# Piletskii-Oleg/chunkfs

Measured on AMD Instinct MI355X. Metric: GiB/s chunked device-resident, FastCDC 4/8/16 KiB avg, at 1/2/4/8 MI355X, higher is better.
Workload: dtype u8

## Files before the change

### chunkfs_amd/build.py

```python
import os
import subprocess
import sys

HERE = os.path.dirname(os.path.abspath(__file__))
ROOT = os.path.dirname(HERE)
CSRC = os.path.join(HERE, "csrc")
BUILD = os.path.join(HERE, "_build")
LIB = os.path.join(HERE, "libchunkfs_amd.so")
SOURCES = ["fastcdc.hip", "fastcdc_ovl.hip", "small.hip", "walk.hip", "util_kernels.hip", "sha256.hip", "index.hip", "engine.cpp", "hostpath.cpp", "capi.cpp",
           "index_host.cpp"]
HEADERS = ["fastcdc.hpp", "small.hpp", "walk.hpp", "cdc_kernels.hpp", "sha256.hpp", "index.hpp", "engine.hpp"]
ARCH = "gfx950"
HIPCC = os.environ.get("HIPCC", "/opt/rocm/bin/hipcc")
CFLAGS = ["-O3", "-std=c++17", "-fPIC", f"--offload-arch={ARCH}", "-Wall", "-Wno-unused-result"]


def source_digest():
    import hashlib
    h = hashlib.sha256()
    files = [os.path.join(CSRC, f) for f in SOURCES + HEADERS] + [
        os.path.join(ROOT, "include", f) for f in ("chunkfs_amd.h", "chunkfs_amd_tables.h", "chunkfs_amd_debug.h", "chunkfs_amd_cdc_params.h")]
    for f in files:
        h.update(os.path.basename(f).encode())
        with open(f, "rb") as fh:
            h.update(fh.read())
    return h.hexdigest()[:16]


def _newer(target, deps):
    if not os.path.exists(target):
        return True
    t = os.path.getmtime(target)
    return any(os.path.getmtime(d) > t for d in deps)


def _run(cmd):
    print("+", " ".join(cmd), flush=True)
    subprocess.check_call(cmd)


def build(force=False, defines=(), lib=None, build_dir=None):
    bdir = build_dir or BUILD
    out_lib = lib or LIB
    os.makedirs(bdir, exist_ok=True)
    common = [os.path.join(CSRC, h) for h in HEADERS] + [
        os.path.join(ROOT, "include", "chunkfs_amd.h"),
        os.path.join(ROOT, "include", "chunkfs_amd_tables.h"),
        os.path.join(ROOT, "include", "chunkfs_amd_debug.h"),
        os.path.join(ROOT, "include", "chunkfs_amd_cdc_params.h"),
    ]
    objs = []
    for src in SOURCES:
        s = os.path.join(CSRC, src)
        o = os.path.join(bdir, src + ".o")
        objs.append(o)
        deps = [s] + common + ([os.path.join(CSRC, "fastcdc.hip")] if src == "fastcdc_ovl.hip" else [])
        if force or _newer(o, deps):
            lang = ["-x", "hip"] if src.endswith(".hip") else []
            _run([HIPCC] + CFLAGS + [f"-D{d}" for d in defines] + lang + ["-c", s, "-o", o])
    if force or _newer(out_lib, objs):
        _run([HIPCC, f"--offload-arch={ARCH}", "-shared", "-fPIC", "-o", out_lib] + objs)
    return out_lib


if __name__ == "__main__":
    build(force="--force" in sys.argv)
```

### chunkfs_amd/csrc/engine.cpp

```cpp
#include "engine.hpp"

#include <algorithm>
#include <atomic>
#include <chrono>
#include <cmath>
#include <cstdio>
#include <cstdlib>
#include <cstring>

#include "../../include/chunkfs_amd_cdc_params.h"
#include "../../include/chunkfs_amd_tables.h"
#include "fastcdc.hpp"
#include "sha256.hpp"

namespace cdc {

namespace {
thread_local std::string g_last_error;

#ifndef CDC_MIN_SPAN_LOG2
#define CDC_MIN_SPAN_LOG2 16
#endif
constexpr uint32_t kMinSpanLog2 = CDC_MIN_SPAN_LOG2;
constexpr uint32_t kMaxSpanLog2 = 17;

constexpr uint32_t kMinimumMin = 64, kMinimumMax = 1048576;
constexpr uint32_t kAverageMin = 256, kAverageMax = 4194304;
constexpr uint32_t kMaximumMin = 1024, kMaximumMax = 16777216;

size_t align_up(size_t x, size_t a) { return (x + a - 1) / a * a; }

uint32_t ceil_log2(uint64_t x) {
    uint32_t r = 0;
    while ((1ull << r) < x) ++r;
    return r;
}
}

void set_error(const std::string &msg) { g_last_error = msg; }
const char *last_error() { return g_last_error.c_str(); }

#define HIP_TRY(expr)                                                          \
    do {                                                                       \
        hipError_t e_ = (expr);                                                \
        if (e_ != hipSuccess) {                                                \
            set_error(std::string(#expr) + ": " + hipGetErrorString(e_));      \
            return CDC_EDEVICE;                                                \
        }                                                                      \
    } while (0)

int Engine::create(cdc_algo_t algo, uint32_t min, uint32_t avg, uint32_t max,
                   int device, Engine **out) {
    if (!out) {
        set_error("cdc_create: out is NULL");
        return CDC_EINVAL;
    }
    *out = nullptr;
    if (algo == CDC_ALGO_RABIN || algo == CDC_ALGO_ULTRA || algo == CDC_ALGO_LEAP || algo == CDC_ALGO_SEQ) {
        const uint32_t seq[4] = {0, CDC_SEQ_LENGTH, CDC_SEQ_JUMP_TRIGGER, CDC_SEQ_JUMP_SIZE};
        return create_walk(algo, seq, min, avg, max, device, out);
    }
    if (algo != CDC_ALGO_FASTCDC && algo != CDC_ALGO_FIXED) {
        set_error("SuperCDC is not implemented on MI355X: its chunk records (supercdc.rs:10, 37-50) "
                  "follow cdc-chunkers 0.1.3, absent offline (SURVEY.md §8c)");
        return CDC_ENOTSUP;
    }
    Engine *e = new Engine();
    e->algo_ = algo;
    e->min_ = min;
    e->avg_ = avg;
    e->max_ = max;
    e->device_ = device;
    if (algo == CDC_ALGO_FASTCDC) {
        if (min < kMinimumMin || min > kMinimumMax || avg < kAverageMin ||
            avg > kAverageMax || max < kMaximumMin || max > kMaximumMax) {
            set_error("FastCDC sizes out of range (fastcdc v2020 asserts: min 64..1MiB, "
                      "avg 256..4MiB, max 1KiB..16MiB)");
            delete e;
            return CDC_EINVAL;
        }
        const unsigned bits = (unsigned)std::lround(std::log2((double)avg));
        FastParams &fp = e->fp_;
        fp.min = min;
        fp.avg = avg;
        fp.max = max;
        fp.mask_s = CHUNKFS_AMD_MASKS[bits + 1];
        fp.mask_l = CHUNKFS_AMD_MASKS[bits - 1];
        fp.cmask = fp.mask_s & fp.mask_l;
        const uint64_t all = fp.mask_s | fp.mask_l;
        const uint32_t top = 63 - (uint32_t)__builtin_clzll(all);
        if (top > 47) {
            set_error("mask tests bit >= 48: unsupported");
            delete e;
            return CDC_EINVAL;
        }
        fp.trunc = top;
        const uint32_t wlo = (uint32_t)__builtin_ctzll(all);
        fp.cm_align = (wlo <= 32 && (all >> wlo) <= 0xFFFFFFFFull) ? 1u : 0u;
        fp.tshift = fp.cm_align ? 32 - wlo : 0;
        fp.cm32 = (uint32_t)((fp.cmask << fp.tshift) >> 32);
        fp.cm_lo = (uint32_t)fp.cmask;
        fp.cm_hi = (uint32_t)(fp.cmask >> 32);
        fp.mask_s_sh = fp.mask_s << fp.tshift;
        fp.mask_l_sh = fp.mask_l << fp.tshift;
        if (const char *d = std::getenv("CHUNKFS_AMD_DIAG")) fp.diag = (uint32_t)std::atoi(d);
        if (const char *v = std::getenv("CHUNKFS_AMD_EVENT_EVERY")) e->event_every_ = std::max(1, std::atoi(v));
        if (const char *v = std::getenv("CHUNKFS_AMD_OVERLAP")) {
            e->ovl_on_ = std::atoi(v) != 0;
            e->ovl_std_ = std::atoi(v) != 1;
        }
        uint32_t l2 = ceil_log2(max);
        e->span_log2_ = l2 > kMinSpanLog2 ? l2 : kMinSpanLog2;
        {
            const uint32_t pcm = (uint32_t)__builtin_popcountll(fp.cmask);
            while (e->span_log2_ < kMaxSpanLog2 && 11 * ((2ull << e->span_log2_) >> (pcm < 63 ? pcm : 63)) <= 384)
                ++e->span_log2_;
        }
        if (const char *v = std::getenv("CHUNKFS_AMD_SPAN"))
            e->span_log2_ = (uint32_t)std::max<int>(std::atoi(v), (int)std::max(l2, 14u));
        e->small_span_log2_ = l2 > 14 ? l2 : 14;
        if (const char *v = std::getenv("CHUNKFS_AMD_SMALL_SPAN")) {
            const int x = std::atoi(v);
            e->small_span_log2_ = x == 0 ? e->span_log2_ : (uint32_t)std::max<int>(x, (int)std::max(l2, 14u));
        }
        if (e->small_span_log2_ > e->span_log2_) e->small_span_log2_ = e->span_log2_;
        const uint64_t span = 1ull << e->span_log2_;
        const uint32_t pc = (uint32_t)__builtin_popcountll(fp.cmask);
        uint64_t cap = 8 * (span >> (pc < 63 ? pc : 63));
        if (cap < 64) cap = 64;
        if (cap > 256) cap = 256;
        e->cap_ = (uint32_t)cap;
        e->smax_ = (uint32_t)(span / ((min / 2) * 2) + 2);
        if (11 * (span >> (pc < 63 ? pc : 63)) > 256 && !e->ovl_std_) e->ovl_on_ = false;
        const uint32_t pmin = (uint32_t)std::min(__builtin_popcountll(fp.mask_s), __builtin_popcountll(fp.mask_l));
        e->small_on_ = pmin >= 10;
        e->small_pmin_ = pmin;
        if (const char *v = std::getenv("CHUNKFS_AMD_SMALL")) e->small_on_ = e->small_on_ && std::atoi(v) != 0;
        if (const char *v = std::getenv("CHUNKFS_AMD_SMALL_ZC")) e->small_zc_ = std::atoi(v) != 0;
        if (const char *v = std::getenv("CHUNKFS_AMD_SMALL_FEED")) e->small_feed_ = std::atoi(v);
        if (const char *v = std::getenv("CHUNKFS_AMD_SMALL_FEED_POOL")) e->small_feed_pool_ = std::atoi(v) != 0;
        char buf[256];
        std::snprintf(buf, sizeof buf,
                      "FastCDC (2020), sizes: SizeParams { min: %u, avg: %u, max: %u } "
                      "[MI355X gfx950]",
                      min, avg, max);
        e->describe_ = buf;
    } else {
        if (min == 0) {
            set_error("FSChunker chunk size must be > 0");
            delete e;
            return CDC_EINVAL;
        }
        char buf[128];
        std::snprintf(buf, sizeof buf, "Fixed size chunking, chunk size: %u [MI355X gfx950]", min);
        e->describe_ = buf;
    }
    const int rc = e->init();
    if (rc != CDC_OK) {
        delete e;
        return rc;
    }
    *out = e;
    return CDC_OK;
}

int Engine::init() {
    int count = 0;
    HIP_TRY(hipGetDeviceCount(&count));
    if (device_ < 0 || device_ >= count) {
        set_error("device index out of range");
        return CDC_EDEVICE;
    }
    HIP_TRY(hipSetDevice(device_));
    hipDeviceProp_t prop;
    HIP_TRY(hipGetDeviceProperties(&prop, device_));
    if (std::strncmp(prop.gcnArchName, "gfx950", 6) != 0) {
        set_error(std::string("chunkfs_amd kernels are built for gfx950 only; device is ") +
                  prop.gcnArchName);
        return CDC_EDEVICE;
    }
    num_cus_ = prop.multiProcessorCount;
    HIP_TRY(hipStreamCreateWithFlags(&own_stream_, hipStreamNonBlocking));
    for (auto &ev : ev_) HIP_TRY(hipEventCreate(&ev));
    for (auto &slot : tev_)
        for (auto &ev : slot) HIP_TRY(hipEventCreate(&ev));
    HIP_TRY(hipMalloc(&d_gear_, 256 * sizeof(uint64_t)));
    HIP_TRY(hipMalloc(&d_counter_, (1 + kShaBuckets) * sizeof(unsigned long long)));
    HIP_TRY(hipMemcpy(d_gear_, CHUNKFS_AMD_GEAR, 256 * sizeof(uint64_t), hipMemcpyHostToDevice));
    return CDC_OK;
}

struct Engine::WalkWorker {
    Engine *ctx = nullptr;
    int device = 0;
    std::thread th;
    std::mutex m;
    std::condition_variable cv;
    bool has_job = false, stop = false;
    bool done = true;
    bool fresh = false;
    uint64_t seq = 0;
    std::vector<const uint8_t *> ptrs;
    std::vector<uint64_t> lens;
    cdc_chunk_t *out = nullptr;
    size_t cap = 0;
    uint64_t *first = nullptr;
    int64_t rc = 0;
    std::string err;

    void loop() {
        (void)hipSetDevice(device);
        std::unique_lock<std::mutex> lk(m);
        for (;;) {
            cv.wait(lk, [&] { return stop || has_job; });
            if (has_job) {
                has_job = false;
                lk.unlock();
                const int64_t r =
                    ctx->chunk_batch_device(ptrs.size(), ptrs.data(), lens.data(), out, cap, first, nullptr);
                std::string e = r < 0 ? std::string(last_error()) : std::string();
                lk.lock();
                rc = r;
                err = std::move(e);
                done = true;
                cv.notify_all();
                continue;
            }
            return;
        }
    }
    void wait_done(std::unique_lock<std::mutex> &lk) {
        cv.wait(lk, [&] { return done; });
    }
    ~WalkWorker() {
        {
            std::lock_guard<std::mutex> g(m);
            stop = true;
        }
        cv.notify_all();
        if (th.joinable()) th.join();
        delete ctx;
    }
};

Engine::~Engine() {
    if (device_ >= 0) (void)hipSetDevice(device_);
    if (fb_any_) (void)fast_drain();
    for (auto &w : ww_) w.reset();
    if (own_stream_) (void)hipStreamSynchronize(own_stream_);
    if (res_stream_) (void)hipStreamSynchronize(res_stream_);
    (void)hipFree(ws_);
    (void)hipFree(small_mem_);
    (void)hipFree(d_gear_);
    (void)hipFree(d_data_);
    (void)hipFree(d_out_);
    (void)hipFree(d_dig_);
    (void)hipFree(d_sha_tab_);
    (void)hipHostFree(h_sha_tab_);
    (void)hipFree(d_sha_order_);
    (void)hipFree(d_counter_);
    (void)hipFree(d_wtabs_);
    (void)hipFree(wws_);
    (void)hipHostFree(h_stage_);
    if (copy_stream_) (void)hipStreamSynchronize(copy_stream_);
    (void)hipHostFree(h_ring_);
    (void)hipHostFree(h_ready_);
    (void)hipHostFree(h_out_);
    for (auto &w : ws_win_) (void)hipFree(w);
    for (auto &e : ring_ev_)
        if (e) (void)hipEventDestroy(e);
    if (copy_done_) (void)hipEventDestroy(copy_done_);
    if (ws_ev_) (void)hipEventDestroy(ws_ev_);
    if (copy_stream_) (void)hipStreamDestroy(copy_stream_);
    for (auto &ev : ev_)
        if (ev) (void)hipEventDestroy(ev);
    for (auto &slot : tev_)
        for (auto &ev : slot)
            if (ev) (void)hipEventDestroy(ev);
    if (own_stream_) (void)hipStreamDestroy(own_stream_);
    for (auto &ev : scan_ev_)
        if (ev) (void)hipEventDestroy(ev);
    if (res_ev_) (void)hipEventDestroy(res_ev_);
    for (auto &ev : res_done_)
        if (ev) (void)hipEventDestroy(ev);
    if (res_stream_) (void)hipStreamDestroy(res_stream_);
}

int Engine::set_gear(const uint64_t *gear) {
    if (!gear) {
        set_error("gear is NULL");
        return CDC_EINVAL;
    }
    if (fb_any_) {
        const int64_t r = drain_implicit();
        if (r < 0) return (int)r;
    }
    if (wr_.active) {
        set_error("cdc_set_gear: a streaming write is in progress (cdc_write_finish it first)");
        return CDC_EINVAL;
    }
    HIP_TRY(hipSetDevice(device_));
    HIP_TRY(hipMemcpy(d_gear_, gear, 256 * sizeof(uint64_t), hipMemcpyHostToDevice));
    return CDC_OK;
}

size_t Engine::estimate(size_t len) const {
    if (algo_ == CDC_ALGO_FIXED) return len / min_ + 1;
    if (algo_ == CDC_ALGO_SEQ) return len / avg_;
    return len / min_;
}

size_t Engine::batch_max_chunks(size_t n, const uint64_t *lens) const {
    size_t t = 0;
    for (size_t i = 0; i < n; ++i) t += lens[i] / min_chunk() + 1;
    return t;
}

int Engine::ensure_host_staging(size_t n) {
    if (h_stage_ && h_stage_streams_ >= n) return CDC_OK;
    if (fb_any_) {
        set_error("internal: host staging regrown with FastCDC batches in flight");
        return CDC_EINVAL;
    }
    (void)hipHostFree(h_stage_);
    h_stage_ = nullptr;
    const size_t want = n + 64;
    h_stage_per_ = 5 * want + 36 + 4 * walk::kMaxFixRounds;
    HIP_TRY(placement().host_malloc(&h_stage_, kHostSlots * h_stage_per_ * sizeof(uint64_t), hipHostMallocCoherent));
    h_stage_streams_ = want;
    for (int k = 0; k < kSlots; ++k) fs_[k].tables.clear();
    return CDC_OK;
}

int Engine::ensure_workspace(uint64_t spans, size_t n) {
    if (ws_ && spans <= ws_spans_ && n <= ws_streams_) return CDC_OK;
    const uint64_t S = spans > ws_spans_ ? spans + spans / 4 + 16 : ws_spans_;
    const size_t N = n > ws_streams_ ? n + 64 : ws_streams_;
    const uint64_t cap = algo_ == CDC_ALGO_FASTCDC ? cap_ : 0;
    const uint64_t smax = algo_ == CDC_ALGO_FASTCDC ? smax_ : 0;
    const size_t A = 256;
    size_t off = 0;
    auto take = [&](size_t bytes) {
        const size_t o = off;
        off = align_up(off + bytes, A);
        return o;
    };
    if (fb_any_) {
        set_error("internal: workspace regrown with FastCDC batches in flight");
        return CDC_EINVAL;
    }
    size_t o_count[kSlots], o_pos[kSlots], o_ptrs[kSlots], o_lens[kSlots], o_sb[kSlots], o_stats[kSlots],
        o_tails[kSlots];
    for (int k = 0; k < kSlots; ++k) {
        o_count[k] = take(S * 4);
        o_pos[k] = take(S * cap * 4);
        o_ptrs[k] = take(N * 8);
        o_lens[k] = take(N * 8);
        o_sb[k] = take((N + 1) * 8);
        o_stats[k] = take(p3::kStatWords * 8);
        o_tails[k] = take(N * 8);
    }
    const size_t o_starts = take(S * smax * 8);
    const size_t o_first = take((N + 1) * 8);
    const uint64_t nb = std::max(p3::resolve_blocks(S), p3::ovl::resolve_blocks(S)) + 2;
    const size_t o_desc = take(6 * nb * 8);
    (void)hipFree(ws_);
    ws_ = nullptr;
    ws_spans_ = 0;
    ws_streams_ = 0;
    HIP_TRY(hipMalloc(&ws_, off));
    ++ws_gen_;
    ws_bytes_ = off;
    ws_spans_ = S;
    ws_streams_ = N;
    char *b = static_cast<char *>(ws_);
    for (int k = 0; k < kSlots; ++k) {
        FastSlot &f = fs_[k];
        f.cand.cap = (uint32_t)cap;
        f.cand.count = reinterpret_cast<uint32_t *>(b + o_count[k]);
        f.cand.pos = reinterpret_cast<uint32_t *>(b + o_pos[k]);
        f.d_ptrs = reinterpret_cast<const uint8_t **>(b + o_ptrs[k]);
        f.d_lens = reinterpret_cast<uint64_t *>(b + o_lens[k]);
        f.d_sb = reinterpret_cast<uint64_t *>(b + o_sb[k]);
        f.d_tails = reinterpret_cast<uint64_t *>(b + o_tails[k]);
        f.stats = reinterpret_cast<uint64_t *>(b + o_stats[k]);
        f.tables.clear();
    }
    cand_ = fs_[0].cand;
    d_first_ = reinterpret_cast<uint64_t *>(b + o_first);
    d_ptrs_ = fs_[0].d_ptrs;
    d_lens_ = fs_[0].d_lens;
    d_span_base_ = fs_[0].d_sb;
    ch3_.smax = (uint32_t)smax;
    ch3_.starts = reinterpret_cast<uint64_t *>(b + o_starts);
    uint64_t *desc = reinterpret_cast<uint64_t *>(b + o_desc);
    rs3_ = p3::Resolve{desc, desc + nb, desc + 2 * nb, desc + 3 * nb, desc + 4 * nb, desc + 5 * nb, 0};
    HIP_TRY(hipMemset(desc, 0, 6 * nb * 8));
    d_tails_ = fs_[0].d_tails;
    return CDC_OK;
}

int64_t Engine::chunk_batch_device(size_t n, const uint8_t *const *d_streams,
                                   const uint64_t *lens, cdc_chunk_t *d_out,
                                   size_t out_cap, uint64_t *first,
                                   hipStream_t stream) {
    return batch_device(n, d_streams, lens, d_out, out_cap, first, stream, false);
}

int64_t Engine::chunk_batch_device_async(size_t n, const uint8_t *const *d_streams, const uint64_t *lens,
                                         cdc_chunk_t *d_out, size_t out_cap, uint64_t *first,
                                         hipStream_t stream) {
    return batch_device(n, d_streams, lens, d_out, out_cap, first, stream, true);
}

int64_t Engine::batch_sync() {
    HIP_TRY(hipSetDevice(device_));
    if (fb_any_) {
        held_valid_ = false;
        return fast_drain();
    }
    if (held_valid_) {
        held_valid_ = false;
        return held_;
    }
    return 0;
}

int64_t Engine::drain_implicit() {
    if (!fb_any_) return 0;
    held_ = fast_drain();
    held_valid_ = true;
    return held_;
}

int64_t Engine::walk_submit(size_t n, const uint8_t *const *d_streams, const uint64_t *lens, cdc_chunk_t *d_out,
                            size_t out_cap, uint64_t *first) {
    const int c = (int)(wk_seq_ % (uint64_t)walk_ctx_);
    if (!ww_[c]) {
        Engine *e = nullptr;
        int rc = create_walk(algo_, seq_cfg_, min_, avg_, max_, device_, &e);
        if (rc) return rc;
        e->walk_async_ = false;
        if (rabin_poly_) rc = e->set_rabin_poly(rabin_poly_);
        if (rc) {
            delete e;
            return rc;
        }
        std::unique_ptr<WalkWorker> w(new WalkWorker());
        w->ctx = e;
        w->device = device_;
        WalkWorker *wp = w.get();
        w->th = std::thread([wp] { wp->loop(); });
        ww_[c] = std::move(w);
    }
    WalkWorker &w = *ww_[c];
    {
        std::unique_lock<std::mutex> lk(w.m);
        w.wait_done(lk);
        if (w.fresh && w.rc < 0) {
            const int64_t rc = w.rc;
            const std::string msg = w.err;
            lk.unlock();
            (void)walk_drain();
            set_error(msg);
            return rc;
        }
        w.ptrs.assign(d_streams, d_streams + n);
        w.lens.assign(lens, lens + n);
        w.out = d_out;
        w.cap = out_cap;
        w.first = first;
        w.seq = wk_seq_;
        w.rc = 0;
        w.err.clear();
        w.done = false;
        w.fresh = true;
        w.has_job = true;
    }
    w.cv.notify_all();
    ++wk_seq_;
    wk_any_ = true;
    fb_any_ = true;
    return 0;
}

int64_t Engine::walk_drain() {
    int64_t res = 0, err = 0;
    std::string msg;
    uint64_t last = 0;
    bool any = false;
    for (auto &wp : ww_) {
        if (!wp) continue;
        WalkWorker &w = *wp;
        std::unique_lock<std::mutex> lk(w.m);
        w.wait_done(lk);
        if (!w.fresh) continue;
        w.fresh = false;
        if (w.rc < 0 && !err) {
            err = w.rc;
            msg = w.err;
        }
        if (!any || w.seq > last) {
            any = true;
            last = w.seq;
            res = w.rc;
            timing_ = w.ctx->timing_;
        }
    }
    wk_any_ = false;
    fb_any_ = false;
    if (err) {
        set_error(msg);
        return err;
    }
    return res;
}

int64_t Engine::batch_device(size_t n, const uint8_t *const *d_streams, const uint64_t *lens, cdc_chunk_t *d_out,
                             size_t out_cap, uint64_t *first, hipStream_t stream, bool async) {
    if (n && (!d_streams || !lens || !first)) {
        set_error("cdc_chunk_batch_device: NULL argument");
        return CDC_EINVAL;
    }
    if (n > 0xFFFFFFFEull) {
        set_error("too many streams");
        return CDC_EINVAL;
    }
    HIP_TRY(hipSetDevice(device_));
    hipStream_t s = stream ? stream : own_stream_;
    uint64_t bytes = 0, need = 0;
    for (size_t i = 0; i < n; ++i) {
        bytes += lens[i];
        need += lens[i] / min_chunk() + 1;
        if (lens[i] && !d_streams[i]) {
            set_error("NULL stream pointer with non-zero length");
            return CDC_EINVAL;
        }
        if (lens[i] && algo_ != CDC_ALGO_FIXED && (reinterpret_cast<uintptr_t>(d_streams[i]) & 15)) {
            set_error("device stream pointers must be 16-byte aligned");
            return CDC_EINVAL;
        }
    }
    if (need > out_cap) {
        set_error("out_cap < cdc_batch_max_chunks()");
        return CDC_EINVAL;
    }
    if (async && is_walk() && walk_async_ && n > 0 && bytes > kSmallBatch)
        return walk_submit(n, d_streams, lens, d_out, out_cap, first);
    const bool pipe = algo_ == CDC_ALGO_FASTCDC && n > 0 && bytes > kSmallBatch;
    if (!pipe && fb_any_) {
        const int64_t r = drain_implicit();
        if (r < 0) return r;
    }
    if (pipe) {
        const int64_t r = fast_submit(n, d_streams, lens, d_out, out_cap, first, bytes, s,
                                      !async || fb_seq_ % event_every_ == 0, async && ovl_on_);
        if (r < 0 || async) return r;
        return fast_drain();
    }
    const double hash_ms = timing_.hash_ms;
    timing_pending_ = false;
    timing_ = cdc_timing_t{};
    timing_.hash_ms = hash_ms;
    timing_.bytes = bytes;
    timing_.path = CDC_PATH_EMPTY;
    out_cap_ = out_cap;
    if (n == 0) {
        if (first) first[0] = 0;
        return 0;
    }
    int rc = ensure_host_staging(n);
    if (rc) return rc;
    if (algo_ == CDC_ALGO_FASTCDC && n == 1 && !small_skip_ && small_ok(lens[0])) {
        rc = run_small(d_streams[0], lens[0], d_out, out_cap, first, s);
        if (rc == CDC_OK) {
            timing_.path = CDC_PATH_SMALL;
            return (int64_t)first[1];
        }
        if (rc < 0) return rc;
    }
    if (algo_ == CDC_ALGO_FASTCDC) {
        const int64_t r = fast_submit(n, d_streams, lens, d_out, out_cap, first, bytes, s, true, false);
        if (r < 0) return r;
        return fast_drain();
    }
    uint64_t *h = static_cast<uint64_t *>(h_stage_);
    uint64_t *h_ptrs = h, *h_lens = h + h_stage_streams_, *h_sb = h + 2 * h_stage_streams_;
    const uint32_t sl2 = is_walk() ? seg_log2_ : 0;
    uint64_t spans = 0;
    for (size_t i = 0; i < n; ++i) {
        h_ptrs[i] = reinterpret_cast<uint64_t>(d_streams[i]);
        h_lens[i] = lens[i];
        h_sb[i] = spans;
        if (is_walk()) spans += (lens[i] + (1ull << sl2) - 1) >> sl2;
    }
    h_sb[n] = spans;
    if (algo_ != CDC_ALGO_FIXED && spans == 0) {
        for (size_t i = 0; i <= n; ++i) first[i] = 0;
        return 0;
    }
    rc = is_walk() ? ensure_walk_workspace(spans, n) : ensure_workspace(spans, n);
    if (rc) return rc;
    const bool zero_copy = bytes <= kSmallBatch && n <= kZeroCopyStreams;
    const bool same = zero_copy || (ws_gen_ == tables_gen_ && tables_.size() == 2 * n &&
                                    std::memcmp(tables_.data(), h_ptrs, n * 8) == 0 &&
                                    std::memcmp(tables_.data() + n, h_lens, n * 8) == 0);
    if (!same) {
        HIP_TRY(hipMemcpyAsync(d_ptrs_, h_ptrs, n * 8, hipMemcpyHostToDevice, s));
        HIP_TRY(hipMemcpyAsync(d_lens_, h_lens, n * 8, hipMemcpyHostToDevice, s));
        HIP_TRY(hipMemcpyAsync(d_span_base_, h_sb, (n + 1) * 8, hipMemcpyHostToDevice, s));
        tables_.assign(h_ptrs, h_ptrs + n);
        tables_.insert(tables_.end(), h_lens, h_lens + n);
        tables_gen_ = ws_gen_;
    }
    StreamTable st{};
    st.ptrs = zero_copy ? reinterpret_cast<const uint8_t *const *>(h_ptrs) : d_ptrs_;
    st.lens = zero_copy ? h_lens : d_lens_;
    st.span_base = zero_copy ? h_sb : d_span_base_;
    st.n = (uint32_t)n;
    st.span_log2 = sl2;
    st.total_spans = spans;
    rc = is_walk() ? run_walk(st, d_out, n, first, s) : run_fixed(st, n, lens, d_out, first, s);
    if (rc) return rc;
    return (int64_t)first[n];
}

int64_t Engine::fast_submit(size_t n, const uint8_t *const *d_streams, const uint64_t *lens, cdc_chunk_t *d_out,
                            size_t out_cap, uint64_t *first, uint64_t bytes, hipStream_t s, bool timed, bool ovl) {
    if (fb_any_ && (s != fb_stream_ || ovl != fb_ovl_)) {
        const int64_t r = drain_implicit();
        if (r < 0) return r;
    }
    if (ovl && !res_stream_) {
        HIP_TRY(hipStreamCreateWithFlags(&res_stream_, hipStreamNonBlocking));
        for (auto &ev : scan_ev_) HIP_TRY(hipEventCreateWithFlags(&ev, hipEventDisableTiming));
        HIP_TRY(hipEventCreateWithFlags(&res_ev_, hipEventDisableTiming));
        for (auto &ev : res_done_) HIP_TRY(hipEventCreateWithFlags(&ev, hipEventDisableTiming));
        if (!std::getenv("CHUNKFS_AMD_NO_PREWARM")) {
            void *d = nullptr;
            HIP_TRY(hipMalloc(&d, 256));
            for (int i = 0; i < 256; ++i) {
                HIP_TRY(hipMemsetAsync(d, i, 4, s));
                HIP_TRY(hipEventRecord(scan_ev_[i % kSlots], s));
                HIP_TRY(hipStreamWaitEvent(res_stream_, scan_ev_[i % kSlots], 0));
                HIP_TRY(hipMemsetAsync(static_cast<char *>(d) + 128, i, 4, res_stream_));
                HIP_TRY(hipEventRecord(res_done_[i % 3], res_stream_));
            }
            HIP_TRY(hipStreamSynchronize(res_stream_));
            HIP_TRY(hipStreamSynchronize(s));
            HIP_TRY(hipFree(d));
        }
    }
    const uint32_t sl2 = bytes <= kSmallBatch ? small_span_log2_ : span_log2_;
    uint64_t spans = 0;
    for (size_t i = 0; i < n; ++i) spans += (lens[i] + (1ull << sl2) - 1) >> sl2;
    const bool zero_copy = bytes <= kSmallBatch && n <= kZeroCopyStreams;
    const bool grow = !(h_stage_ && h_stage_streams_ >= n) || !(ws_ && spans <= ws_spans_ && n <= ws_streams_);
    if (fb_any_ && (zero_copy || grow)) {
        const int64_t r = drain_implicit();
        if (r < 0) return r;
    }
    const uint64_t seq = fb_seq_;
    if (fb_[seq % 3].live) {
        const int rc = fast_collect((int)(seq % 3));
        if (rc) {
            (void)fast_drain();
            return rc;
        }
    }
    int rc = ensure_host_staging(n);
    if (rc) return rc;
    rc = ensure_workspace(spans ? spans : 1, n);
    if (rc) return rc;
    const int slot = (int)(seq % kSlots);
    FastSlot &f = fs_[slot];
    uint64_t *hb = static_cast<uint64_t *>(h_stage_) + (seq % kHostSlots) * h_stage_per_;
    uint64_t *h_ptrs = hb, *h_lens = hb + h_stage_streams_, *h_sb = hb + 2 * h_stage_streams_;
    uint64_t *h_tails = hb + 3 * h_stage_streams_;
    bool same = !zero_copy && f.tables_gen == ws_gen_ && f.tables.size() == 2 * n;
    for (size_t i = 0; same && i < n; ++i)
        same = f.tables[i] == reinterpret_cast<uint64_t>(d_streams[i]) && f.tables[n + i] == lens[i];
    {
        uint64_t sp = 0;
        uint32_t nt = 0;
        for (size_t i = 0; i < n; ++i) {
            h_ptrs[i] = reinterpret_cast<uint64_t>(d_streams[i]);
            h_lens[i] = lens[i];
            h_sb[i] = sp;
            sp += (lens[i] + (1ull << sl2) - 1) >> sl2;
            if (lens[i] & ((1ull << sl2) - 1)) h_tails[nt++] = sp - 1;
        }
        h_sb[n] = sp;
        if (same && nt != f.n_tails) same = false;
        f.n_tails = nt;
    }
    if (!same) {
        f.tables.clear();
        if (!zero_copy) {
            HIP_TRY(hipMemcpyAsync(f.d_ptrs, h_ptrs, n * 8, hipMemcpyHostToDevice, s));
            HIP_TRY(hipMemcpyAsync(f.d_lens, h_lens, n * 8, hipMemcpyHostToDevice, s));
            HIP_TRY(hipMemcpyAsync(f.d_sb, h_sb, (n + 1) * 8, hipMemcpyHostToDevice, s));
            if (f.n_tails) HIP_TRY(hipMemcpyAsync(f.d_tails, h_tails, f.n_tails * 8, hipMemcpyHostToDevice, s));
            f.tables.assign(h_ptrs, h_ptrs + n);
            f.tables.insert(f.tables.end(), h_lens, h_lens + n);
            f.tables_gen = ws_gen_;
        }
    }
    StreamTable st{};
    st.ptrs = zero_copy ? reinterpret_cast<const uint8_t *const *>(h_ptrs) : f.d_ptrs;
    st.lens = zero_copy ? h_lens : f.d_lens;
    st.span_base = zero_copy ? h_sb : f.d_sb;
    st.n = (uint32_t)n;
    st.span_log2 = sl2;
    st.total_spans = spans;
    uint64_t *h_misc = hb + 4 * h_stage_streams_;
    const p3::Compact cp{f.stats, h_misc, h_misc + p3::kStatWords};
    h_misc[p3::kStatDone] = ~0ull;
    if (!spans) {
        h_misc[p3::kStatDone] = 1;
        h_misc[p3::kStatError] = 0;
        for (size_t i = 0; i <= n; ++i) cp.h_first[i] = 0;
    }
    p3::Resolve rs = rs3_;
    rs.gen = ++res_gen_;
    FastBatch &rec = fb_[seq % 3];
    rec = FastBatch{};
    rec.resolved = true;
    rec.ovl = ovl;
    rec.slot = slot;
    rec.h = hb;
    rec.n = n;
    rec.first = first;
    rec.seq = seq;
    rec.bytes = bytes;
    rec.spans = spans;
    hipEvent_t *ev = tev_[seq % kTimeRing];
    tev_timed_[seq % kTimeRing] = timed;
    rec.timed = timed;
    if (timed) HIP_TRY(hipEventRecord(ev[0], s));
    if (!ovl) {
        if (spans)
            HIP_TRY(p3::launch_scan(st, fp_, d_gear_, f.cand, cp, zero_copy ? h_tails : f.d_tails, f.n_tails,
                                    num_cus_, s));
        if (timed) HIP_TRY(hipEventRecord(ev[1], s));
        if (spans) HIP_TRY(p3::launch_resolve(st, fp_, d_gear_, f.cand, ch3_, cp, rs, d_out, out_cap, s));
        if (timed) HIP_TRY(hipEventRecord(ev[2], s));
    } else {
        static_assert(kSlots > kHostSlots, "device slots must outlast the host blocks");
        if (spans && ovl_std_)
            HIP_TRY(p3::launch_scan(st, fp_, d_gear_, f.cand, cp, zero_copy ? h_tails : f.d_tails, f.n_tails,
                                    num_cus_, s));
        else if (spans)
            HIP_TRY(p3::ovl::launch_scan(st, fp_, d_gear_, f.cand, cp, zero_copy ? h_tails : f.d_tails, f.n_tails,
                                         num_cus_, s));
        if (timed) HIP_TRY(hipEventRecord(ev[1], s));
        HIP_TRY(hipEventRecord(scan_ev_[slot], s));
        HIP_TRY(hipStreamWaitEvent(res_stream_, scan_ev_[slot], 0));
        if (spans && ovl_std_)
            HIP_TRY(p3::launch_resolve(st, fp_, d_gear_, f.cand, ch3_, cp, rs, d_out, out_cap, res_stream_));
        else if (spans)
            HIP_TRY(p3::ovl::launch_resolve(st, fp_, d_gear_, f.cand, ch3_, cp, rs, d_out, out_cap, res_stream_));
        if (timed) HIP_TRY(hipEventRecord(ev[2], res_stream_));
        else HIP_TRY(hipEventRecord(res_done_[seq % 3], res_stream_));
    }
    rec.live = true;
    fb_seq_ = seq + 1;
    fast_batches_ = fb_seq_;
    fb_any_ = true;
    fb_stream_ = s;
    fb_ovl_ = ovl;
    cand_ = f.cand;
    last_spans_ = spans;
    return 0;
}

int64_t Engine::fast_drain() {
    if (!fb_any_) return 0;
    if (wk_any_) return walk_drain();
    const uint64_t last = fb_seq_ - 1;
    int rc = CDC_OK;
    int64_t total = 0;
    for (uint64_t q = last >= 2 ? last - 2 : 0; q <= last; ++q) {
        FastBatch &b = fb_[q % 3];
        if (!b.live || b.seq != q) continue;
        const int r = rc ? rc : fast_collect((int)(q % 3));
        b.live = false;
        if (r && !rc) rc = r;
        if (q == last && !rc) total = (int64_t)b.first[b.n];
    }
    if (fb_ovl_) {
        if (!rc && hipEventRecord(res_ev_, res_stream_) == hipSuccess)
            (void)hipStreamWaitEvent(fb_stream_, res_ev_, 0);
        else
            (void)hipStreamSynchronize(res_stream_);
    }
    if (rc) (void)hipStreamSynchronize(fb_stream_);
    fb_any_ = false;
    return rc ? rc : total;
}

int Engine::fast_collect(int k) {
    FastBatch &b = fb_[k];
    if (!b.resolved) {
        set_error("internal: FastCDC batch collected before its resolve was enqueued");
        return CDC_EDEVICE;
    }
    uint64_t *h_misc = b.h + 4 * h_stage_streams_;
    {
        const volatile uint64_t *done = h_misc + p3::kStatDone;
        const uint64_t us = b.ovl ? std::min<uint64_t>(4000, std::max<uint64_t>(200, b.bytes / 1000000))
                                  : std::min<uint64_t>(2000, std::max<uint64_t>(100, b.bytes / 2000000));
        const auto budget = std::chrono::microseconds(us);
        const auto t_spin = std::chrono::steady_clock::now();
        while (*done == ~0ull && std::chrono::steady_clock::now() - t_spin < budget) __builtin_ia32_pause();
    }
    if (h_misc[p3::kStatDone] == ~0ull) {
        if (b.timed) HIP_TRY(hipEventSynchronize(tev_[b.seq % kTimeRing][2]));
        else if (b.ovl) HIP_TRY(hipEventSynchronize(res_done_[b.seq % 3]));
        else HIP_TRY(hipStreamSynchronize(fb_stream_));
    }
    b.live = false;
    if (h_misc[p3::kStatDone] != 1 || h_misc[p3::kStatError] != 0) {
        set_error(h_misc[p3::kStatDone] != 1 ? "resolve kernel did not report back"
                                             : "chain overflow, output bound or look-back timeout (internal error)");
        return CDC_EDEVICE;
    }
    if (fp_.diag & 64) {
        const uint64_t *d = h_misc + p3::kStatDiag0;
        const uint64_t s0 = ~d[0], s1 = d[1], e1 = d[2], e0 = ~d[3];
        const double blocks =
            (double)(b.ovl && !ovl_std_ ? p3::ovl::resolve_blocks(b.spans) : p3::resolve_blocks(b.spans));
        std::fprintf(stderr, "resolve blocks, us: scan's last block end -> first start %.2f  starts spread %.2f  "
                             "first start -> first end %.2f  -> last end %.2f  longest block %.2f  mean block %.2f\n",
                     ((double)s0 - (double)d[6]) / 100.0, (s1 - s0) / 100.0, (e0 - s0) / 100.0, (e1 - s0) / 100.0,
                     d[4] / 100.0, d[5] / 100.0 / (blocks ? blocks : 1.0));
    } else if (fp_.diag & 128) {
        const double waves = b.ovl && !ovl_std_ ? (double)p3::ovl::resolve_blocks(b.spans) * 4
                                                : (double)p3::resolve_blocks(b.spans) * 8;
        std::fprintf(stderr, (fp_.diag & 8192) ? "resolve link passes, us per wave (records: issue trunc link; "
                                                 "virtual: issue trunc link; -; -):"
                                               : "resolve phases, us per wave (meta recs settle+wait virtual-links "
                                                 "record-links walk lookback(w0) out):");
        for (int i = 0; i < p3::kStatDiagN; ++i)
            std::fprintf(stderr, " %.2f", (double)h_misc[p3::kStatDiag0 + i] / 100.0 / (waves ? waves : 1.0));
        std::fprintf(stderr, "\n");
    }
    const uint64_t *lens = b.h + h_stage_streams_;
    uint64_t *hf = h_misc + p3::kStatWords;
    for (size_t i = b.n; i-- > 0;)
        if (lens[i] == 0) hf[i] = hf[i + 1];
    std::memcpy(b.first, hf, (b.n + 1) * 8);
    const double hash_ms = timing_.hash_ms;
    timing_ = cdc_timing_t{};
    timing_.hash_ms = hash_ms;
    timing_.bytes = b.bytes;
    timing_.candidates = h_misc[p3::kStatCand];
    timing_.overflow_spans = (uint32_t)h_misc[p3::kStatOvf];
    timing_.fixup_iterations = (uint32_t)h_misc[p3::kStatRewalk];
    timing_.walk_fallback_steps = h_misc[p3::kStatOnDemand];
    timing_.path = CDC_PATH_PIPELINE;
    timing_.timed = b.timed ? 1u : 0u;
    timing_pending_ = true;
    timing_seq_ = b.seq;
    return CDC_OK;
}

bool Engine::small_ok(uint64_t len) const {
    return small_on_ && len > 0 && len <= small::kMaxBytes && (len >> small_pmin_) <= small::kRecCap * 5 / 8;
}

int Engine::run_small(const uint8_t *data, uint64_t len, cdc_chunk_t *d_out, size_t out_cap, uint64_t *first,
                      hipStream_t s, bool host_input, const uint8_t *feed_src, uint8_t *feed_dst,
                      uint32_t feed_slot) {
    if (!small_mem_) {
        HIP_TRY(hipMalloc(&small_mem_, small::scratch_bytes() + small::copy_bytes() + small::bstamp_bytes()));
        HIP_TRY(hipMemset(small_mem_, 0, small::scratch_bytes()));
        uint32_t *b = static_cast<uint32_t *>(small_mem_);
        small_ws_.brec = reinterpret_cast<uint64_t *>(b);
        small_ws_.bcnt = b + 2 * small::kMaxBlocks * small::kBlockRecCap;
        small_ws_.ticket = small_ws_.bcnt + small::kMaxBlocks;
        small_ws_.stamp = reinterpret_cast<uint64_t *>(static_cast<char *>(small_mem_) + small::scratch_bytes() - 64);
        small_ws_.bpub = small_ws_.stamp - small::kMaxBlocks;
        small_ws_.copy = static_cast<uint8_t *>(small_mem_) + small::scratch_bytes();
        small_ws_.bstamp = reinterpret_cast<uint64_t *>(small_ws_.copy + small::copy_bytes());
    }
    uint64_t *h = static_cast<uint64_t *>(h_stage_);
    uint64_t *h_misc = h + 4 * h_stage_streams_;
    uint64_t *h_first = h_misc + p3::kStatWords;
    volatile uint64_t *done = h_misc + small::kWordDone;
    *done = 0;
    small_seq_ = small_seq_ % 0xFFFFFFFEull + 1;
    const small::Feed feed{feed_src ? h_ready_dev_ + (size_t)feed_slot * small::kFeedPieces : nullptr, small_seq_};
    auto feed_copy = [&]() {
        const auto tc = std::chrono::steady_clock::now();
        volatile uint64_t *ready = h_ready_ + (size_t)feed_slot * small::kFeedPieces;
        if (small_feed_pool_) {
            pool_->copy_feed(feed_dst, feed_src, len, size_t(1) << small::kFeedLog2, ready, small_seq_);
        } else {
            const uint64_t piece = 1ull << small::kFeedLog2;
            for (uint64_t off = 0; off < len; off += piece) {
                std::memcpy(feed_dst + off, feed_src + off, std::min(piece, len - off));
                std::atomic_thread_fence(std::memory_order_release);
                ready[off >> small::kFeedLog2] = small_seq_;
            }
        }
        small_copy_s_ = std::chrono::duration<double>(std::chrono::steady_clock::now() - tc).count();
    };
    if (feed_src && small_feed_ == 2) feed_copy();
    HIP_TRY(small::launch_small(data, len, fp_, d_gear_, small_ws_, d_out, out_cap, h_misc, h_first, host_input,
                                feed, s));
    ++small_calls_;
    if (feed_src && small_feed_ != 2) {
        feed_copy();
    }
    const auto t_spin = std::chrono::steady_clock::now();
    while (*done == 0 && std::chrono::steady_clock::now() - t_spin < std::chrono::microseconds(2000))
        __builtin_ia32_pause();
    if (*done == 0) HIP_TRY(hipStreamSynchronize(s));
    if (*done != 1) {
        set_error("small FastCDC kernel did not report back");
        return CDC_EDEVICE;
    }
    timing_pending_ = false;
    timing_.candidates = h_misc[small::kWordRecords];
    timing_.overflow_spans = 0;
    timing_.fixup_iterations = 0;
    timing_.walk_fallback_steps = 0;
    if (fp_.diag & small::kDiagStamps) {
        const uint64_t *t = h_misc + small::kWordStamp0;
        std::fprintf(stderr, "small: %llu B, us from block 0's start: last block %.2f, records %.2f, links %.2f "
                             "(%llu rounds), walk %.2f, output %.2f\n",
                     (unsigned long long)len, (t[1] - t[0]) / 100.0, (t[2] - t[0]) / 100.0, (t[3] - t[0]) / 100.0,
                     (unsigned long long)t[7], (t[4] - t[0]) / 100.0, (t[5] - t[0]) / 100.0);
        std::fprintf(stderr, "  round 0 max cycles per lane: load+trunc %llu, link %llu, successor %llu; rounds end at",
                     (unsigned long long)(t[6] & 0x1FFFFF), (unsigned long long)((t[6] >> 21) & 0x1FFFFF),
                     (unsigned long long)(t[6] >> 42));
        for (int k = 0; k < 4; ++k)
            if (h_first[2 + k]) std::fprintf(stderr, " %.2f", (h_first[2 + k] - t[0]) / 100.0);
        if (feed_src) std::fprintf(stderr, "; block 0 fed at %.2f; host copy %.2f us", (h_first[6] - t[0]) / 100.0,
                                   small_copy_s_ * 1e6);
        std::fprintf(stderr, "; round 0 added %llu entries, round 1 worked on %llu", (unsigned long long)(h_first[7] & 0xFFFF),
                     (unsigned long long)(h_first[7] >> 16));
        std::fprintf(stderr, "\n");
        const uint32_t G = (uint32_t)((len + small::kBlockBytes - 1) / small::kBlockBytes);
        std::vector<uint64_t> bs((size_t)G * 8);
        HIP_TRY(hipStreamSynchronize(s));
        HIP_TRY(hipMemcpy(bs.data(), small_ws_.bstamp, bs.size() * 8, hipMemcpyDeviceToHost));
        const char *nm[6] = {"fed", "loaded", "hashed(w0)", "tinfo(w0)", "drained", "ticket"};
        std::fprintf(stderr, "  blocks (%u):", G);
        for (int k = 0; k < 6; ++k) {
            std::vector<double> v;
            for (uint32_t b = 0; b < G; ++b) v.push_back(((double)bs[b * 8 + k] - (double)t[0]) / 100.0);
            std::sort(v.begin(), v.end());
            std::fprintf(stderr, " %s %.2f/%.2f/%.2f", nm[k], v.front(), v[v.size() / 2], v.back());
        }
        std::fprintf(stderr, "\n");
    }
    if (h_misc[small::kWordFallback]) {
        ++small_fallbacks_;
        return kSmallFallback;
    }
    first[0] = 0;
    first[1] = h_first[1];
    return CDC_OK;
}

const cdc_timing_t &Engine::timing() {
    if (fb_any_) (void)drain_implicit();
    if (timing_pending_) {
        timing_pending_ = false;
        (void)timing_back((uint32_t)(fast_batches_ - 1 - timing_seq_), timing_);
    }
    return timing_;
}

int Engine::timing_back(uint32_t back, cdc_timing_t &out) {
    if (fb_any_) (void)drain_implicit();
    if (algo_ != CDC_ALGO_FASTCDC || back >= kTimeRing || back >= fast_batches_) {
        set_error("cdc_debug_timing_back: no such FastCDC batch in the event ring");
        return CDC_EINVAL;
    }
    if (&out != &timing_) out = timing_;
    hipEvent_t *ev = tev_[(fast_batches_ - 1 - back) % kTimeRing];
    float t01 = 0, t12 = 0, t02 = 0;
    HIP_TRY(hipSetDevice(device_));
    out.path = CDC_PATH_PIPELINE;
    out.timed = tev_timed_[(fast_batches_ - 1 - back) % kTimeRing] ? 1u : 0u;
    if (!out.timed) {
        out.scan_ms = out.resolve_ms = out.total_ms = 0;
        return CDC_OK;
    }
    HIP_TRY(hipEventSynchronize(ev[2]));
    HIP_TRY(hipEventElapsedTime(&t01, ev[0], ev[1]));
    HIP_TRY(hipEventElapsedTime(&t12, ev[1], ev[2]));
    HIP_TRY(hipEventElapsedTime(&t02, ev[0], ev[2]));
    out.scan_ms = t01;
    out.resolve_ms = t12;
    out.total_ms = t02;
    return CDC_OK;
}

int Engine::run_fixed(const StreamTable &st, size_t n, const uint64_t *lens,
                      cdc_chunk_t *d_out, uint64_t *first, hipStream_t s) {
    uint64_t *h = static_cast<uint64_t *>(h_stage_);
    uint64_t *h_first = h + 4 * h_stage_streams_;
    uint64_t t = 0;
    for (size_t i = 0; i < n; ++i) {
        h_first[i] = t;
        t += (lens[i] + min_ - 1) / min_;
    }
    h_first[n] = t;
    HIP_TRY(hipEventRecord(ev_[0], s));
    HIP_TRY(hipMemcpyAsync(d_first_, h_first, (n + 1) * 8, hipMemcpyHostToDevice, s));
    HIP_TRY(launch_fixed(st, min_, d_first_, d_out, t, s));
    HIP_TRY(hipEventRecord(ev_[3], s));
    HIP_TRY(hipStreamSynchronize(s));
    std::memcpy(first, h_first, (n + 1) * 8);
    float t03 = 0;
    HIP_TRY(hipEventElapsedTime(&t03, ev_[0], ev_[3]));
    timing_.total_ms = t03;
    timing_.scan_ms = t03;
    timing_.path = CDC_PATH_FIXED;
    timing_.timed = 1;
    return CDC_OK;
}

int64_t Engine::fs_write(const uint8_t *data, size_t len, size_t seg_size, std::vector<uint64_t> &spans,
                         double *seconds) {
    spans.clear();
    if (seg_size == 0) {
        set_error("cdc_fs_write: seg_size must be > 0");
        return CDC_EINVAL;
    }
    if (len && !data) {
        set_error("cdc_fs_write: data is NULL");
        return CDC_EINVAL;
    }
    int rc = write_begin();
    if (rc) return rc;
    for (size_t off = 0; !rc && off < len; off += seg_size)
        rc = write_segment(data + off, std::min(seg_size, len - off));
    if (rc) {
        wr_.active = false;
        return rc;
    }
    return write_finish(spans, seconds);
}

int Engine::sha256_device(const uint8_t *d_data, const cdc_chunk_t *d_chunks, size_t n,
                          uint8_t *d_digests, hipStream_t s) {
    const uint64_t first[2] = {0, n};
    return sha256_batch(1, &d_data, first, d_chunks, d_digests, s);
}

int Engine::sha256_batch(size_t n, const uint8_t *const *d_streams, const uint64_t *first,
                         const cdc_chunk_t *d_chunks, uint8_t *d_digests, hipStream_t s) {
    if (n == 0) return CDC_OK;
    if (!d_streams || !first) {
        set_error("cdc_sha256_batch_device: NULL stream table");
        return CDC_EINVAL;
    }
    if (first[0] != 0) {
        set_error("cdc_sha256_batch_device: first[0] must be 0");
        return CDC_EINVAL;
    }
    for (size_t i = 0; i < n; ++i) {
        if (first[i + 1] < first[i]) {
            set_error("cdc_sha256_batch_device: first[] must be non-decreasing");
            return CDC_EINVAL;
        }
        if (first[i + 1] > first[i] && !d_streams[i]) {
            set_error("cdc_sha256_batch_device: NULL stream with chunks");
            return CDC_EINVAL;
        }
    }
    const uint64_t total = first[n];
    if (total >= (1ull << 32)) {
        set_error("cdc_sha256_batch_device: more than 2^32 - 1 chunks in one batch");
        return CDC_EINVAL;
    }
    if (total && (!d_chunks || !d_digests)) {
        set_error("cdc_sha256_chunks_device: NULL argument");
        return CDC_EINVAL;
    }
    HIP_TRY(hipSetDevice(device_));
    if (fb_any_) {
        const int64_t r = drain_implicit();
        if (r < 0) return (int)r;
    }
    hipStream_t st = s ? s : own_stream_;
    (void)timing();
    if (total == 0) {
        timing_.hash_ms = 0;
        return CDC_OK;
    }
    const size_t words = 2 * n + 1;
    if (sha_tab_cap_ < words) {
        (void)hipFree(d_sha_tab_);
        (void)hipHostFree(h_sha_tab_);
        d_sha_tab_ = h_sha_tab_ = nullptr;
        sha_tab_cap_ = 0;
        const size_t want = words + 64;
        HIP_TRY(hipMalloc(&d_sha_tab_, want * 8));
        HIP_TRY(hipHostMalloc(&h_sha_tab_, want * 8, hipHostMallocDefault));
        sha_tab_cap_ = want;
    }
    std::memcpy(h_sha_tab_, first, (n + 1) * 8);
    for (size_t i = 0; i < n; ++i) h_sha_tab_[n + 1 + i] = reinterpret_cast<uint64_t>(d_streams[i]);
    HIP_TRY(hipMemcpyAsync(d_sha_tab_, h_sha_tab_, words * 8, hipMemcpyHostToDevice, st));
    ShaBatch b{};
    b.chunks = reinterpret_cast<const cdc_chunk_pod *>(d_chunks);
    b.n_chunks = total;
    b.first = d_sha_tab_;
    b.base = d_sha_tab_ + n + 1;
    b.n_streams = (uint32_t)n;
    b.digests = reinterpret_cast<uint32_t *>(d_digests);
    b.counter = d_counter_;
    if (sha_order_cap_ < total) {
        (void)hipFree(d_sha_order_);
        d_sha_order_ = nullptr;
        sha_order_cap_ = 0;
        const uint64_t want = total + total / 8 + 1024;
        HIP_TRY(hipMalloc(&d_sha_order_, want * sizeof(uint32_t)));
        sha_order_cap_ = want;
    }
    b.order = d_sha_order_;
    HIP_TRY(hipEventRecord(ev_[3], st));
    HIP_TRY(launch_sha256(b, num_cus_, st));
    HIP_TRY(hipEventRecord(ev_[2], st));
    HIP_TRY(hipStreamSynchronize(st));
    float ms = 0;
    HIP_TRY(hipEventElapsedTime(&ms, ev_[3], ev_[2]));
    timing_.hash_ms = ms;
    return CDC_OK;
}

int64_t Engine::debug_copy(int what, void *out, size_t max_bytes) {
    if (fb_any_) {
        const int64_t r = drain_implicit();
        if (r < 0) return r;
    }
    if (algo_ != CDC_ALGO_FASTCDC || !ws_) {
        set_error("debug_copy: no FastCDC batch yet");
        return CDC_EINVAL;
    }
    const void *src = nullptr;
    size_t bytes = 0;
    if (what == 0) {
        src = cand_.count;
        bytes = last_spans_ * 4;
    } else if (what == 1) {
        src = cand_.pos;
        bytes = last_spans_ * cap_ * 4;
    } else {
        set_error("debug_copy: unknown array");
        return CDC_EINVAL;
    }
    if (bytes > max_bytes) bytes = max_bytes;
    HIP_TRY(hipSetDevice(device_));
    HIP_TRY(hipStreamSynchronize(own_stream_));
    if (bytes) HIP_TRY(hipMemcpy(out, src, bytes, hipMemcpyDeviceToHost));
    return (int64_t)bytes;
}

int Engine::read_bw(const uint8_t *d_buf, size_t len, int reps, double *ms) {
    HIP_TRY(hipSetDevice(device_));
    if (fb_any_) {
        const int64_t r = drain_implicit();
        if (r < 0) return (int)r;
    }
    uint64_t *d_acc = nullptr;
    const size_t words = (size_t)num_cus_ * 8;
    HIP_TRY(hipMalloc(&d_acc, words * 8));
    hipError_t e = hipMemsetAsync(d_acc, 0, words * 8, own_stream_);
    if (e == hipSuccess) e = launch_read_reduce(d_buf, len, d_acc, num_cus_, own_stream_);
    if (e == hipSuccess) e = hipEventRecord(ev_[0], own_stream_);
    for (int r = 0; e == hipSuccess && r < reps; ++r) e = launch_read_reduce(d_buf, len, d_acc, num_cus_, own_stream_);
    if (e == hipSuccess) e = hipEventRecord(ev_[3], own_stream_);
    if (e == hipSuccess) e = hipEventSynchronize(ev_[3]);
    float t = 0;
    if (e == hipSuccess) e = hipEventElapsedTime(&t, ev_[0], ev_[3]);
    (void)hipFree(d_acc);
    if (e != hipSuccess) {
        set_error(std::string("read_bw: ") + hipGetErrorString(e));
        return CDC_EDEVICE;
    }
    *ms = (double)t / reps;
    return CDC_OK;
}

int Engine::fill_splitmix64(uint8_t *d_buf, size_t len, uint64_t seed, hipStream_t s) {
    HIP_TRY(hipSetDevice(device_));
    hipStream_t st = s ? s : own_stream_;
    HIP_TRY(launch_fill_splitmix64(d_buf, len, seed, st));
    HIP_TRY(hipStreamSynchronize(st));
    return CDC_OK;
}


namespace {
uint64_t gf2_mod(uint64_t x, uint64_t p) {
    const int dp = 63 - __builtin_clzll(p);
    while (x) {
        const int dx = 63 - __builtin_clzll(x);
        if (dx < dp) break;
        x ^= p << (dx - dp);
    }
    return x;
}

uint64_t splitmix_word(uint64_t z) {
    z = (z ^ (z >> 30)) * 0xBF58476D1CE4E5B9ull;
    z = (z ^ (z >> 27)) * 0x94D049BB133111EBull;
    return z ^ (z >> 31);
}
}

int Engine::create_seq(const uint32_t seq[4], uint32_t min, uint32_t avg, uint32_t max, int device,
                       Engine **out) {
    if (!seq) {
        set_error("cdc_create_seq: config is NULL");
        return CDC_EINVAL;
    }
    return create_walk(CDC_ALGO_SEQ, seq, min, avg, max, device, out);
}

int Engine::create_walk(cdc_algo_t algo, const uint32_t seq[4], uint32_t min, uint32_t avg, uint32_t max,
                        int device, Engine **out) {
    if (!out) {
        set_error("cdc_create: out is NULL");
        return CDC_EINVAL;
    }
    *out = nullptr;
    if (min == 0 || min > avg || avg > max || (algo == CDC_ALGO_ULTRA && min < 8) ||
        (algo == CDC_ALGO_LEAP && min < 32) || (algo == CDC_ALGO_RABIN && avg < 2)) {
        set_error("invalid sizes: need 0 < min <= avg <= max (UltraCDC min >= 8, LeapCDC min >= 32)");
        return CDC_EINVAL;
    }
    if (algo == CDC_ALGO_SEQ && (seq[0] > 1 || seq[1] == 0 || seq[2] == 0 || seq[3] == 0)) {
        set_error("invalid SeqCDC config: mode 0/1, seq_length > 0, jump_trigger > 0, jump_size > 0");
        return CDC_EINVAL;
    }
    Engine *e = new Engine();
    e->algo_ = algo;
    e->min_ = min;
    e->avg_ = avg;
    e->max_ = max;
    e->device_ = device;
    const char *name = algo == CDC_ALGO_RABIN ? "RabinCDC" : algo == CDC_ALGO_ULTRA ? "UltraCDC"
                     : algo == CDC_ALGO_LEAP ? "LeapCDC" : "SeqCDC";
    char buf[256];
    if (algo == CDC_ALGO_SEQ)
        std::snprintf(buf, sizeof buf, "%s, sizes: SizeParams { min: %u, avg: %u, max: %u }, mode: %s [MI355X gfx950]",
                      name, min, avg, max, seq[0] ? "Decreasing" : "Increasing");
    else
        std::snprintf(buf, sizeof buf, "%s, sizes: SizeParams { min: %u, avg: %u, max: %u } [MI355X gfx950]", name,
                      min, avg, max);
    e->describe_ = buf;
    for (int i = 0; i < 4; ++i) e->seq_cfg_[i] = seq[i];
    if (const char *v = std::getenv("CHUNKFS_AMD_WALK_ASYNC")) e->walk_async_ = std::atoi(v) != 0;
    if (const char *v = std::getenv("CHUNKFS_AMD_WALK_CTX")) e->walk_ctx_ = std::max(2, std::min(kWalkCtxMax, std::atoi(v)));
    int rc = e->init();
    if (rc == CDC_OK) rc = e->init_walk(seq);
    if (rc != CDC_OK) {
        delete e;
        return rc;
    }
    *out = e;
    return CDC_OK;
}

int Engine::init_walk(const uint32_t *seq) {
    walk::WalkParams &wp = wp_;
    wp.algo = (uint32_t)algo_;
    wp.min = min_;
    wp.avg = avg_;
    wp.max = max_;
    wp.rabin_mask = (1ull << cdc_log2_round(avg_)) - 1;

    const uint64_t lspan = avg_ > min_ ? (uint64_t)(avg_ - min_) : 1;
    const uint32_t lb = cdc_log2_round(lspan);
    wp.leap_thr = CDC_LEAP_THRESHOLD[lb > 32 ? 32 : lb];
    wp.seq_mode = seq[0];
    wp.seq_len = seq[1];
    wp.seq_trig = seq[2];
    wp.seq_jump = seq[3];
    wp.nbm = algo_ == CDC_ALGO_RABIN ? (min_ >= CDC_RABIN_WINDOW ? 1u : 0u)
           : algo_ == CDC_ALGO_ULTRA ? 3u : algo_ == CDC_ALGO_LEAP ? 2u
           : (wp.seq_len <= 63 ? 1u : 0u);
    if (const char *b = std::getenv("CHUNKFS_AMD_WALK_BYTES"))
        if (std::atoi(b) != 0) wp.nbm = 0;
    wp.wave = wp.nbm ? 1u : 0u;
    if (const char *v = std::getenv("CHUNKFS_AMD_WAVE")) wp.wave = wp.wave && std::atoi(v) != 0;
    uint64_t warm_mult = !wp.wave ? (algo_ == CDC_ALGO_SEQ ? 16 : 8)
                       : algo_ == CDC_ALGO_RABIN ? 8 : algo_ == CDC_ALGO_LEAP ? 24 : 16;
    seg_log2_ = !wp.wave ? 15 : algo_ == CDC_ALGO_RABIN ? 17 : 18;
    if (wp.wave) {
        const uint32_t wl = ceil_log2(warm_mult * avg_);
        if (wl > seg_log2_) seg_log2_ = wl < 22 ? wl : 22;
    }
    const uint32_t lmin = 63 - (uint32_t)__builtin_clzll((uint64_t)min_) + 12;
    if (seg_log2_ > lmin) seg_log2_ = lmin < 12 ? 12 : lmin;
    if (const char *w = std::getenv("CHUNKFS_AMD_WALK")) {
        unsigned a = 0, b = 0;
        if (std::sscanf(w, "%u,%u", &a, &b) == 2 && a >= 10 && a <= 30) {
            seg_log2_ = a;
            warm_mult = b;
        }
    }
    wp.warm = warm_mult * avg_;
    if (const char *a = std::getenv("CHUNKFS_AMD_AHEAD")) {
        unsigned x = 0, y = 0;
        if (std::sscanf(a, "%u,%u", &x, &y) == 2 && y >= 1) {
            ahead_after_ = x;
            ahead_max_ = y;
        }
    }
    wp.ahead = 1;
    wp.bits_fine = 1;
    if (const char *f = std::getenv("CHUNKFS_AMD_BITS_FINE")) wp.bits_fine = std::atoi(f) != 0 ? 1u : 0u;
    if (const char *f = std::getenv("CHUNKFS_AMD_WALK_FUSED")) walk_fused_ = std::atoi(f) != 0;
    wp.cap = (uint32_t)((1ull << seg_log2_) / min_ + 2);
    const bool linkable = algo_ == CDC_ALGO_RABIN || algo_ == CDC_ALGO_ULTRA || algo_ == CDC_ALGO_LEAP;
    wp.links = algo_ == CDC_ALGO_ULTRA ? 1u : 0u;
    if (const char *l = std::getenv("CHUNKFS_AMD_LINKS")) wp.links = std::atoi(l) != 0 && linkable;
    {
        const uint32_t dens = algo_ == CDC_ALGO_RABIN ? cdc_log2_round(avg_) : algo_ == CDC_ALGO_ULTRA ? 10u : lb;
        const uint64_t expect = ((1ull << seg_log2_) >> dens) + 1;
        uint64_t cc = 16;
        while (cc < 4 * expect && cc < 1024) cc <<= 1;
        wp.ccap = (uint32_t)cc;
    }
    if (!wp.nbm) wp.links = 0;
    if (wp.wave) wp.links = 0;
    wp.seg_words = (uint32_t)((1ull << seg_log2_) / 64);
    wp.piece_log2 = seg_log2_ < 15 ? seg_log2_ : 15;
    wp.bm = nullptr;
    HIP_TRY(hipMalloc(&d_wtabs_, 768 * sizeof(uint64_t)));
    wp.tabs = d_wtabs_;
    return load_walk_tables(CDC_RABIN_POLY);
}

int Engine::load_walk_tables(uint64_t P) {
    uint64_t t[768];
    const int deg = 63 - __builtin_clzll(P);
    for (uint64_t b = 0; b < 256; ++b) {
        t[b] = gf2_mod(b << deg, P) | (b << deg);
        uint64_t h = b;
        for (uint32_t i = 1; i < CDC_RABIN_WINDOW; ++i) h = gf2_mod(h << 8, P);
        t[256 + b] = h;
        t[512 + b] = splitmix_word(CDC_LEAP_SEED + (b + 1) * 0x9E3779B97F4A7C15ull);
    }
    HIP_TRY(hipSetDevice(device_));
    HIP_TRY(hipMemcpy(d_wtabs_, t, sizeof t, hipMemcpyHostToDevice));
    wp_.rabin_shift = (uint32_t)deg - 8;
    return CDC_OK;
}

int Engine::set_rabin_poly(uint64_t P) {
    if (algo_ != CDC_ALGO_RABIN) {
        set_error("cdc_set_rabin_poly: not a RabinChunker handle");
        return CDC_EINVAL;
    }
    const int deg = P ? 63 - __builtin_clzll(P) : -1;
    if (deg < 9 || deg > 56) {
        set_error("cdc_set_rabin_poly: polynomial degree must be 9..56");
        return CDC_EINVAL;
    }
    if (wr_.active) {
        set_error("cdc_set_rabin_poly: a streaming write is in progress (cdc_write_finish it first)");
        return CDC_EINVAL;
    }
    HIP_TRY(hipSetDevice(device_));
    if (fb_any_) {
        const int64_t r = drain_implicit();
        if (r < 0) return (int)r;
    }
    HIP_TRY(hipStreamSynchronize(own_stream_));
    rabin_poly_ = P;
    for (auto &w : ww_) w.reset();
    (void)hipFree(wws_);
    wws_ = nullptr;
    wws_segs_ = 0;
    wws_streams_ = 0;
    return load_walk_tables(P);
}

int Engine::ensure_walk_workspace(uint64_t segs, size_t n) {
    if (wws_ && segs <= wws_segs_ && n <= wws_streams_) return CDC_OK;
    const uint64_t S = segs > wws_segs_ ? segs + segs / 4 + 16 : wws_segs_;
    const size_t N = n > wws_streams_ ? n + 64 : wws_streams_;
    const uint64_t nb = S / walk::kScanBlock + 2;
    const size_t A = 256;
    size_t off = 0;
    auto take = [&](size_t bytes) {
        const size_t o = off;
        off = align_up(off + bytes, A);
        return o;
    };
    const size_t oE = take(S * 8), oX = take(S * 8), oXs = take(S * 8), oEs = take(S * 8), oP = take((S + 1) * 8);
    const size_t oN = take(S * 4), oL = take(S * (size_t)wp_.cap * 8), oB = take((nb + 1) * 8);
    const size_t oF = take((N + 1) * 8), oG = take((4 + 4 * walk::kMaxFixRounds) * 8), oGo = take(16);
    const size_t oBM = take(S * (size_t)wp_.seg_words * wp_.nbm * 8);
    const bool jt = algo_ == CDC_ALGO_LEAP && wp_.wave;
    const size_t oJT = take(jt ? S * (size_t)wp_.seg_words * 24 : 0);
    const size_t oJ8 = take(jt ? S * (size_t)wp_.seg_words * 6 : 0);
    bool rsum = walk::bits_write_summary(wp_);
    if (const char *q = std::getenv("CHUNKFS_AMD_QUIET")) rsum = rsum && std::atoi(q) != 0;
    const size_t oRS = take(rsum ? S * (size_t)wp_.seg_words / 8 * (algo_ == CDC_ALGO_RABIN ? 2 : 1) : 0);
    const size_t oQS = take(rsum ? S : 0);
    const size_t cc = wp_.links ? wp_.ccap : 0;
    const size_t oCN = take(S * 4), oCP = take(S * cc * 4), oLN = take(S * cc * 8), oLI = take(S * cc * 4);
    const size_t vc = wp_.links ? S * 8 : 0;
    const size_t oVC = take((2 * walk::kVirtRounds + 2) * 8), oVP = take(vc * 8), oVS = take(vc * 4),
                 oVN = take(vc * 8), oVI = take(vc * 4);
    const size_t o_ptrs = take(N * 8), o_lens = take(N * 8), o_sb = take((N + 1) * 8);
    (void)hipFree(wws_);
    wws_ = nullptr;
    wws_segs_ = 0;
    wws_streams_ = 0;
    HIP_TRY(hipMalloc(&wws_, off));
    ++ws_gen_;
    wws_segs_ = S;
    wws_streams_ = N;
    char *b = static_cast<char *>(wws_);
    wst_.E = reinterpret_cast<uint64_t *>(b + oE);
    wst_.X = reinterpret_cast<uint64_t *>(b + oX);
    wst_.Xs = reinterpret_cast<uint64_t *>(b + oXs);
    wst_.Es = reinterpret_cast<uint64_t *>(b + oEs);
    wst_.P = reinterpret_cast<uint64_t *>(b + oP);
    wst_.N = reinterpret_cast<uint32_t *>(b + oN);
    wst_.list = reinterpret_cast<uint64_t *>(b + oL);
    wst_.bsum = reinterpret_cast<uint64_t *>(b + oB);
    wst_.first = reinterpret_cast<uint64_t *>(b + oF);
    wst_.flags = reinterpret_cast<unsigned long long *>(b + oG);
    walk_go_ = reinterpret_cast<uint64_t *>(b + oGo);
    walk_flags_clean_ = false;
    wp_.bm = wp_.nbm ? reinterpret_cast<uint64_t *>(b + oBM) : nullptr;
    wp_.jt = jt ? reinterpret_cast<uint8_t *>(b + oJT) : nullptr;
    wp_.jt8 = jt ? reinterpret_cast<uint16_t *>(b + oJ8) : nullptr;
    wp_.rsum = rsum ? reinterpret_cast<uint64_t *>(b + oRS) : nullptr;
    wp_.qseg = rsum ? reinterpret_cast<uint8_t *>(b + oQS) : nullptr;
    wp_.ccnt = reinterpret_cast<uint32_t *>(b + oCN);
    wp_.cpos = reinterpret_cast<uint32_t *>(b + oCP);
    wp_.lnext = reinterpret_cast<uint64_t *>(b + oLN);
    wp_.lidx = reinterpret_cast<uint32_t *>(b + oLI);
    wp_.vcap = (uint32_t)vc;
    wp_.vcnt = reinterpret_cast<unsigned long long *>(b + oVC);
    wp_.vpos = reinterpret_cast<uint64_t *>(b + oVP);
    wp_.vseg = reinterpret_cast<uint32_t *>(b + oVS);
    wp_.vnext = reinterpret_cast<uint64_t *>(b + oVN);
    wp_.vidx = reinterpret_cast<uint32_t *>(b + oVI);
    d_ptrs_ = reinterpret_cast<const uint8_t **>(b + o_ptrs);
    d_lens_ = reinterpret_cast<uint64_t *>(b + o_lens);
    d_span_base_ = reinterpret_cast<uint64_t *>(b + o_sb);
    return CDC_OK;
}

int Engine::run_walk(const StreamTable &st, cdc_chunk_t *d_out, size_t n, uint64_t *first, hipStream_t s) {
    uint64_t *h = static_cast<uint64_t *>(h_stage_);
    uint64_t *h_first = h + 4 * h_stage_streams_ + 4;
    uint64_t *h_flags = h + 5 * h_stage_streams_ + 32;
    uint64_t *h_rf = h_flags + 4;
    const uint32_t R = max_rounds_ < walk::kMaxFixRounds ? max_rounds_ : walk::kMaxFixRounds;
    HIP_TRY(hipEventRecord(ev_[0], s));
    if (!walk_flags_clean_) HIP_TRY(walk::launch_flags_init(wst_.flags, R, s));
    walk_flags_clean_ = false;
    static const bool diag = std::getenv("CHUNKFS_AMD_WALKDIAG") != nullptr;
    auto lap = [&](const char *what) -> int {
        if (!diag) return CDC_OK;
        static auto t_last = std::chrono::steady_clock::now();
        HIP_TRY(hipStreamSynchronize(s));
        const auto t = std::chrono::steady_clock::now();
        std::fprintf(stderr, "  walkdiag %-6s %9.3f ms\n", what,
                     std::chrono::duration<double, std::milli>(t - t_last).count());
        t_last = t;
        return CDC_OK;
    };
    (void)lap("start");
    HIP_TRY(walk::launch_bits(st, wp_, s));
    (void)lap("bits");
    HIP_TRY(walk::launch_links(st, wp_, s));
    (void)lap("links");
    if (diag && wp_.links) {
        std::vector<uint32_t> cn(st.total_spans);
        HIP_TRY(hipMemcpy(cn.data(), wp_.ccnt, cn.size() * 4, hipMemcpyDeviceToHost));
        uint64_t tot = 0, ovf = 0, mx = 0;
        for (uint32_t c : cn) {
            tot += c;
            ovf += c > wp_.ccap;
            mx = c > mx ? c : mx;
        }
        std::fprintf(stderr, "  walkdiag candidates %llu (%.2f per segment, max %llu, cap %u, overflowed %llu of %zu)\n",
                     (unsigned long long)tot, (double)tot / cn.size(), (unsigned long long)mx, wp_.ccap,
                     (unsigned long long)ovf, cn.size());
    }
    HIP_TRY(walk::launch_walk(st, wp_, wst_, s));
    (void)lap("walk");
    HIP_TRY(hipEventRecord(ev_[1], s));
    constexpr uint32_t kGroup = 4;
    unsigned long long *rf = wst_.flags + 4;
    uint64_t rewalked = 0, round_errors = 0;
    bool settled = false, quiet_stop = false, queued = false, fused = false;
    uint32_t launched = 0, last_round = 0;
    while (launched < R && !settled) {
        const uint32_t grp = launched == 0 ? walk::kFirstGroupRounds : kGroup;
        const uint32_t end = launched + grp < R ? launched + grp : R;
        for (uint32_t r = launched; r < end; ++r) {
            wp_.ahead = r < ahead_after_ ? 1u : ahead_max_;
            walk::WalkState ws = wst_;
            ws.flags = rf + 4 * r;
            ws.gate = r ? rf + 4 * (r - 1) : nullptr;
            const auto t0 = std::chrono::steady_clock::now();
            HIP_TRY(walk::launch_fix(st, wp_, ws, s, r != 0));
            if (diag) {
                HIP_TRY(hipStreamSynchronize(s));
                std::fprintf(stderr, "  walkdiag round %u %.3f ms\n", r,
                             std::chrono::duration<double, std::milli>(std::chrono::steady_clock::now() - t0).count());
            }
        }
        queued = launched == 0 && !diag;
        launched = end;
        fused = queued && walk_fused_ && walk::finish_fits(st);
        if (fused) {
            HIP_TRY(walk::launch_finish_emit(st, wp_, wst_, d_out, out_cap_, s, rf, launched, launched, walk_go_,
                                             h_first, h_flags));
        } else {
            if (queued) {
                HIP_TRY(walk::launch_emit(st, wp_, wst_, d_out, out_cap_, s, rf, launched));
                HIP_TRY(hipMemcpyAsync(h_first, wst_.first, (n + 1) * 8, hipMemcpyDeviceToHost, s));
            }
            HIP_TRY(hipMemcpyAsync(h_flags, wst_.flags, (4 + (size_t)launched * 4) * 8, hipMemcpyDeviceToHost, s));
        }
        if (queued) HIP_TRY(hipEventRecord(ev_[2], s));
        HIP_TRY(hipStreamSynchronize(s));
        for (uint32_t r = 0; r < launched; ++r) {
            const int v = walk::round_verdict(h_rf[4 * r], h_rf[4 * r + 3] >> 32);
            if (v == walk::kRoundSettled) {
                settled = true;
                break;
            }
            if (v == walk::kRoundQuiet) {
                last_round = r;
                quiet_stop = true;
                break;
            }
        }
        if (quiet_stop) break;
    }
    for (uint32_t r = 0; r < launched; ++r) {
        round_errors += h_rf[4 * r + 1];
        rewalked += h_rf[4 * r + 3] & 0xFFFFFFFFull;
    }
    if (diag) {
        std::fprintf(stderr, "  walkdiag rounds %u settled %d:", launched, (int)settled);
        for (uint32_t r = 0; r < launched && r < 24; ++r)
            std::fprintf(stderr, " %llu/%llu", (unsigned long long)h_rf[4 * r + 3], (unsigned long long)h_rf[4 * r]);
        std::fprintf(stderr, "\n");
    }
    if (!settled) {
        const uint32_t lr = quiet_stop ? last_round : launched - 1;
        HIP_TRY(hipMemcpyAsync(wst_.flags + 2, rf + 4 * lr + 2, 8, hipMemcpyDeviceToDevice, s));
        HIP_TRY(walk::launch_serial(st, wp_, wst_, s));
    }
    (void)lap("fixup");
    const bool gated_ran = queued && settled && launched == walk::kFirstGroupRounds;
    walk_flags_clean_ = gated_ran && fused;
    if (!gated_ran) {
        HIP_TRY(walk::launch_emit(st, wp_, wst_, d_out, out_cap_, s));
        HIP_TRY(hipMemcpyAsync(h_flags, wst_.flags, 4 * 8, hipMemcpyDeviceToHost, s));
        HIP_TRY(hipMemcpyAsync(h_first, wst_.first, (n + 1) * 8, hipMemcpyDeviceToHost, s));
        HIP_TRY(hipEventRecord(ev_[2], s));
        HIP_TRY(hipStreamSynchronize(s));
    }
    if (h_flags[1] + round_errors != 0) {
        set_error("segment walk: chunk list or output bound exceeded (internal error)");
        return CDC_EDEVICE;
    }
    std::memcpy(first, h_first, (n + 1) * 8);
    float t01 = 0, t12 = 0, t02 = 0;
    HIP_TRY(hipEventElapsedTime(&t01, ev_[0], ev_[1]));
    HIP_TRY(hipEventElapsedTime(&t12, ev_[1], ev_[2]));
    HIP_TRY(hipEventElapsedTime(&t02, ev_[0], ev_[2]));
    timing_.scan_ms = t01;
    timing_.resolve_ms = t12;
    timing_.total_ms = t02;
    timing_.fixup_iterations = (uint32_t)rewalked;
    timing_.overflow_spans = settled ? 0u : 1u;
    timing_.path = CDC_PATH_WALK;
    timing_.timed = 1;
    return CDC_OK;
}

}
```

### chunkfs_amd/csrc/engine.hpp

```cpp
#pragma once
#include <hip/hip_runtime.h>

#include <atomic>
#include <condition_variable>
#include <memory>
#include <mutex>
#include <string>
#include <thread>
#include <vector>

#include "../../include/chunkfs_amd.h"
#include "cdc_kernels.hpp"
#include "fastcdc.hpp"
#include "small.hpp"
#include "walk.hpp"

namespace cdc {

struct HostPlacement {
    std::string pci, link, link_max;
    int node = -1;
    int allowed = 0;
    std::vector<int> cpus;
    bool enabled = false;
    static HostPlacement probe(int device);
    hipError_t host_malloc(void **ptr, size_t bytes, unsigned flags) const;
    static int node_of(const void *addr);
};

class CopyPool {
  public:
    CopyPool(unsigned threads, unsigned spin_us, const std::vector<int> &cpus);
    ~CopyPool();
    static CopyPool &for_node(int node, const std::vector<int> &cpus);
    void copy(void *dst, const void *src, size_t n);
    void copy_feed(void *dst, const void *src, size_t n, size_t piece, volatile uint64_t *ready, uint64_t seq);
    unsigned threads() const { return (unsigned)th_.size() + 1; }
    unsigned pinned() const { return pinned_; }

  private:
    void run(unsigned id);
    void work();
    void job(void *dst, const void *src, size_t n, size_t piece, volatile uint64_t *ready, uint64_t seq);
    std::vector<std::thread> th_;
    std::mutex m_, job_m_;
    std::condition_variable cv_;
    unsigned spin_us_ = 200;
    unsigned pinned_ = 0;
    std::atomic<uint64_t> gen_{0};
    std::atomic<bool> stop_{false}, open_{false};
    std::atomic<unsigned> active_{0};
    std::atomic<size_t> next_{0}, done_{0};
    uint8_t *dst_ = nullptr;
    const uint8_t *src_ = nullptr;
    size_t n_ = 0, piece_ = 0, np_ = 0;
    volatile uint64_t *ready_ = nullptr;
    uint64_t seq_ = 0;
};

class Engine {
  public:
    static int create(cdc_algo_t algo, uint32_t min, uint32_t avg, uint32_t max,
                      int device, Engine **out);
    static int create_seq(const uint32_t seq[4], uint32_t min, uint32_t avg, uint32_t max,
                          int device, Engine **out);
    ~Engine();

    int64_t chunk_host(const uint8_t *data, size_t len, cdc_chunk_t *out, size_t cap,
                       uint8_t *digests = nullptr);
    int64_t fs_write(const uint8_t *data, size_t len, size_t seg_size, std::vector<uint64_t> &spans,
                     double *seconds);
    int write_begin();
    int write_segment(const uint8_t *data, size_t len);
    int64_t write_finish(std::vector<uint64_t> &spans, double *seconds);
    int64_t write_drain(uint64_t *out, size_t cap);
    int host_stats(double *v, size_t n) const;
    int64_t host_placement_json(char *out, size_t cap);
    int sha256_device(const uint8_t *d_data, const cdc_chunk_t *d_chunks, size_t n,
                      uint8_t *d_digests, hipStream_t s);
    int sha256_batch(size_t n, const uint8_t *const *d_streams, const uint64_t *first, const cdc_chunk_t *d_chunks,
                     uint8_t *d_digests, hipStream_t s);
    int64_t chunk_batch_device(size_t n, const uint8_t *const *d_streams,
                               const uint64_t *lens, cdc_chunk_t *d_out,
                               size_t out_cap, uint64_t *first, hipStream_t stream);
    int64_t chunk_batch_device_async(size_t n, const uint8_t *const *d_streams, const uint64_t *lens,
                                     cdc_chunk_t *d_out, size_t out_cap, uint64_t *first, hipStream_t stream);
    int64_t batch_sync();
    size_t estimate(size_t len) const;
    size_t min_chunk() const { return algo_ == CDC_ALGO_FASTCDC ? (min_ / 2) * 2 : min_; }
    size_t max_chunks(size_t len) const { return len / min_chunk() + 1; }
    size_t batch_max_chunks(size_t n, const uint64_t *lens) const;
    int set_gear(const uint64_t *gear);
    int set_rabin_poly(uint64_t poly);
    const char *describe() const { return describe_.c_str(); }
    const cdc_timing_t &timing();
    int timing_back(uint32_t back, cdc_timing_t &out);
    cdc_algo_t algo() const { return algo_; }
    int device() const { return device_; }
    int fill_splitmix64(uint8_t *d_buf, size_t len, uint64_t seed, hipStream_t s);
    int read_bw(const uint8_t *d_buf, size_t len, int reps, double *ms);
    int64_t debug_copy(int what, void *out, size_t max_bytes);
    uint32_t record_cap() const { return cap_; }
    int pipeline() const { return 3; }

  private:
    Engine() = default;
    static int create_walk(cdc_algo_t algo, const uint32_t seq[4], uint32_t min, uint32_t avg, uint32_t max,
                           int device, Engine **out);
    int init();
    int ensure_workspace(uint64_t spans, size_t n);
    int ensure_host_staging(size_t n);
    int64_t batch_device(size_t n, const uint8_t *const *d_streams, const uint64_t *lens, cdc_chunk_t *d_out,
                         size_t out_cap, uint64_t *first, hipStream_t stream, bool async);
    int64_t fast_submit(size_t n, const uint8_t *const *d_streams, const uint64_t *lens, cdc_chunk_t *d_out,
                        size_t out_cap, uint64_t *first, uint64_t bytes, hipStream_t s, bool timed, bool ovl);
    int fast_collect(int rec);
    int64_t fast_drain();
    int64_t drain_implicit();
    int64_t walk_submit(size_t n, const uint8_t *const *d_streams, const uint64_t *lens, cdc_chunk_t *d_out,
                        size_t out_cap, uint64_t *first);
    int64_t walk_drain();
    struct WalkWorker;
    static constexpr int kWalkCtxMax = 4;
    std::unique_ptr<WalkWorker> ww_[kWalkCtxMax];
    int walk_ctx_ = 2;
    bool wk_any_ = false;
    uint64_t wk_seq_ = 0;
    bool walk_async_ = true;
    uint32_t seq_cfg_[4] = {0, 0, 0, 0};
    uint64_t rabin_poly_ = 0;
    static constexpr int kSmallFallback = 1;
    bool small_ok(uint64_t len) const;
    int run_small(const uint8_t *data, uint64_t len, cdc_chunk_t *d_out, size_t out_cap, uint64_t *first,
                  hipStream_t s, bool host_input = false, const uint8_t *feed_src = nullptr,
                  uint8_t *feed_dst = nullptr, uint32_t feed_slot = 0);
    int run_fixed(const StreamTable &st, size_t n, const uint64_t *lens,
                  cdc_chunk_t *d_out, uint64_t *first, hipStream_t s);
    bool is_walk() const { return algo_ != CDC_ALGO_FASTCDC && algo_ != CDC_ALGO_FIXED; }
    int init_walk(const uint32_t *seq);
    int load_walk_tables(uint64_t rabin_poly);
    int ensure_walk_workspace(uint64_t segs, size_t n);
    int run_walk(const StreamTable &st, cdc_chunk_t *d_out, size_t n, uint64_t *first, hipStream_t s);
    int ensure_ring();
    int ensure_host_out(size_t chunks);
    int ensure_device_data(size_t len);
    int upload(const uint8_t *src, size_t len, uint8_t *dst, hipStream_t s, size_t piece);
    int write_window(bool final);

    cdc_algo_t algo_ = CDC_ALGO_FASTCDC;
    uint32_t min_ = 0, avg_ = 0, max_ = 0;
    int device_ = 0;
    int num_cus_ = 256;
    FastParams fp_{};
    uint32_t span_log2_ = 16;
    uint32_t small_span_log2_ = 16;
    static constexpr uint64_t kSmallBatch = uint64_t(8) << 20;
    static constexpr size_t kZeroCopyStreams = 64;
    uint32_t cap_ = 0, smax_ = 0;
    std::string describe_;

    hipStream_t own_stream_ = nullptr;
    hipEvent_t ev_[4] = {nullptr, nullptr, nullptr, nullptr};
    static constexpr uint32_t kTimeRing = 64;
    hipEvent_t tev_[kTimeRing][3] = {};
    uint64_t fast_batches_ = 0;
    uint64_t *d_gear_ = nullptr;

    void *ws_ = nullptr;
    size_t ws_bytes_ = 0;
    uint64_t ws_spans_ = 0;
    size_t ws_streams_ = 0;
    Candidates cand_{};
    p3::Chains ch3_{};
    p3::Resolve rs3_{};
    uint64_t res_gen_ = 0;
    uint64_t *d_tails_ = nullptr;
    static constexpr int kSlots = 4, kHostSlots = 3;
    struct FastSlot {
        Candidates cand{};
        const uint8_t **d_ptrs = nullptr;
        uint64_t *d_lens = nullptr, *d_sb = nullptr, *d_tails = nullptr, *stats = nullptr;
        std::vector<uint64_t> tables;
        uint64_t tables_gen = ~0ull;
        uint32_t n_tails = 0;
    } fs_[kSlots];
    struct FastBatch {
        bool live = false, resolved = false, timed = true, ovl = false;
        int slot = 0;
        uint64_t *h = nullptr;
        size_t n = 0;
        uint64_t *first = nullptr;
        uint64_t seq = 0, bytes = 0, spans = 0;
    } fb_[3];
    int event_every_ = 4;
    bool tev_timed_[kTimeRing] = {};
    uint64_t timing_seq_ = 0;
    uint64_t fb_seq_ = 0;
    hipStream_t fb_stream_ = nullptr;
    bool fb_any_ = false;
    bool fb_ovl_ = false;
    bool ovl_on_ = true;
    bool ovl_std_ = true;
    hipStream_t res_stream_ = nullptr;
    hipEvent_t scan_ev_[kSlots] = {};
    hipEvent_t res_ev_ = nullptr;
    hipEvent_t res_done_[3] = {};
    int64_t held_ = 0;
    bool held_valid_ = false;
    const uint64_t *cur_tails_ = nullptr;
    uint32_t n_tails_ = 0;
    uint64_t *d_first_ = nullptr;
    const uint8_t **d_ptrs_ = nullptr;
    uint64_t *d_lens_ = nullptr;
    uint64_t *d_span_base_ = nullptr;

    void *h_stage_ = nullptr;
    size_t h_stage_streams_ = 0, h_stage_per_ = 0;

    static constexpr uint32_t kRingSlots = 4;
    static constexpr size_t kRingSlot = size_t(4) << 20;
    static constexpr size_t kWriteWindow = size_t(256) << 20;
    static constexpr size_t kRingDirect = size_t(16) << 20;
    void *h_ring_ = nullptr;
    uint8_t *h_ring_dev_ = nullptr;
    CopyPool *pool_ = nullptr;
    HostPlacement place_;
    bool place_probed_ = false;
    const HostPlacement &placement();
    hipEvent_t ring_ev_[kRingSlots] = {};
    uint32_t ring_next_ = 0;
    uint64_t *h_ready_ = nullptr, *h_ready_dev_ = nullptr;
    hipStream_t copy_stream_ = nullptr;
    hipEvent_t copy_done_ = nullptr, ws_ev_ = nullptr;
    cdc_chunk_t *h_out_ = nullptr, *d_hout_ = nullptr;
    size_t h_out_cap_ = 0;
    uint8_t *ws_win_[2] = {nullptr, nullptr};
    struct WriteState {
        bool active = false, failed = false;
        int cur = 0;
        size_t drained = 0;
        size_t reserve = 0, carry = 0, fill = 0;
        uint64_t bytes = 0, segments = 0;
        double t0 = 0, chunk_s = 0;
        std::vector<uint64_t> spans;
    } wr_;
    struct HostStats {
        uint64_t calls = 0;
        double upload_s = 0, total_s = 0;
    } host_;
    uint8_t *d_data_ = nullptr;
    size_t d_data_bytes_ = 0;
    cdc_chunk_t *d_out_ = nullptr;
    size_t d_out_cap_ = 0;
    uint8_t *d_dig_ = nullptr;
    size_t d_dig_cap_ = 0;
    unsigned long long *d_counter_ = nullptr;
    uint64_t *d_sha_tab_ = nullptr, *h_sha_tab_ = nullptr;
    size_t sha_tab_cap_ = 0;
    uint32_t *d_sha_order_ = nullptr;
    uint64_t sha_order_cap_ = 0;

    cdc_timing_t timing_{};
    bool timing_pending_ = false;

    std::vector<uint64_t> tables_;
    uint64_t ws_gen_ = 0, tables_gen_ = ~0ull;
    bool small_on_ = false, small_zc_ = true;
    int small_feed_ = 1;
    bool small_feed_pool_ = true;
    uint32_t small_pmin_ = 0;
    bool small_skip_ = false;
    void *small_mem_ = nullptr;
    small::Scratch small_ws_{};
    uint64_t small_calls_ = 0, small_fallbacks_ = 0;
    uint64_t small_seq_ = 0;
    double small_copy_s_ = 0;
    uint64_t last_spans_ = 0;
    uint64_t out_cap_ = 0;

    walk::WalkParams wp_{};
    uint32_t seg_log2_ = 14;
    uint32_t max_rounds_ = 16;
    uint32_t ahead_after_ = 8;
    uint32_t ahead_max_ = 64;
    uint64_t *d_wtabs_ = nullptr;
    void *wws_ = nullptr;
    uint64_t wws_segs_ = 0;
    size_t wws_streams_ = 0;
    walk::WalkState wst_{};
    uint64_t *walk_go_ = nullptr;
    bool walk_flags_clean_ = false;
    bool walk_fused_ = true;
};

void set_error(const std::string &msg);
const char *last_error();

}
```

### chunkfs_amd/csrc/fastcdc.hip

```cpp
#include "fastcdc.hpp"

#include <cstdlib>
#include <type_traits>

namespace cdc {
namespace p3 {
namespace {


constexpr uint32_t kCandPosMask = 0x00FFFFFFu;
constexpr uint32_t kCandHitL = 1u << 30;
constexpr uint32_t kCandHitS = 1u << 31;

typedef unsigned int u32x4 __attribute__((ext_vector_type(4)));
typedef const __attribute__((address_space(1))) u32x4 g_u32x4;
typedef const __attribute__((address_space(1))) uint8_t g_u8;
typedef const __attribute__((address_space(1))) uint32_t g_u32;
typedef __attribute__((address_space(1))) uint64_t g_u64;
__device__ __forceinline__ g_u32x4 *as_global4(const void *p) { return (g_u32x4 *)(p); }
__device__ __forceinline__ g_u8 *as_global1(const void *p) { return (g_u8 *)(p); }
__device__ __forceinline__ uint4 ld16(g_u32x4 *p) {
    const u32x4 v = *p;
    return make_uint4(v.x, v.y, v.z, v.w);
}
__device__ __forceinline__ uint4 ld16_nt(g_u32x4 *p) {
    const u32x4 v = __builtin_nontemporal_load(p);
    return make_uint4(v.x, v.y, v.z, v.w);
}

#ifndef CDC_SCAN_NOFENCE
#define SCHED_FENCE() __builtin_amdgcn_sched_barrier(0)
#else
#define SCHED_FENCE() do {} while (0)
#endif
#ifndef CDC_SCAN_WAVES
#define CDC_SCAN_WAVES 12
#endif
#ifndef CDC_SCAN_NT_ODD
#define CDC_SCAN_NT_ODD 1
#endif
#ifndef CDC_SCAN_WAVE_MAJOR
#define CDC_SCAN_WAVE_MAJOR 1
#endif
#ifndef CDC_SCAN_LOOK
#define CDC_SCAN_LOOK 1
#endif
#ifndef CDC_SCAN_TRUNC
#define CDC_SCAN_TRUNC 0
#endif

__device__ __forceinline__ void wave_sync_lds() {
    __builtin_amdgcn_fence(__ATOMIC_RELEASE, "wavefront");
    __builtin_amdgcn_wave_barrier();
    __builtin_amdgcn_fence(__ATOMIC_ACQUIRE, "wavefront");
}

__device__ __forceinline__ void locate(const StreamTable &st, uint64_t g, uint32_t &si, uint64_t &off) {
    uint32_t lo = 0, hi = st.n;
    while (hi - lo > 1) {
        const uint32_t mid = (lo + hi) >> 1;
        if (st.span_base[mid] <= g) lo = mid; else hi = mid;
    }
    si = lo;
    off = (g - st.span_base[lo]) << st.span_log2;
}

template <bool kAlign>
__device__ __forceinline__ uint32_t cand_test(uint64_t h, const FastParams &fp) {
    if constexpr (kAlign) {
        return (uint32_t)(h >> 32) & fp.cm32;
    } else {
        return ((uint32_t)h & fp.cm_lo) | ((uint32_t)(h >> 32) & fp.cm_hi);
    }
}

__device__ __forceinline__ uint64_t shl1_add(uint64_t h, uint64_t g) {
    return (h << 1) + g;
}

__device__ __forceinline__ uint64_t wave_shr1(uint64_t v, uint64_t fill) {
    const uint32_t lo = (uint32_t)__builtin_amdgcn_update_dpp(
        (int)(uint32_t)fill, (int)(uint32_t)v, 0x138, 0xF, 0xF, false);
    const uint32_t hi = (uint32_t)__builtin_amdgcn_update_dpp(
        (int)(uint32_t)(fill >> 32), (int)(uint32_t)(v >> 32), 0x138, 0xF, 0xF, false);
    return ((uint64_t)hi << 32) | lo;
}

__device__ __forceinline__ uint64_t readlane_u64(uint64_t v, int l) {
    const uint32_t lo = (uint32_t)__builtin_amdgcn_readlane((int)(uint32_t)v, l);
    const uint32_t hi = (uint32_t)__builtin_amdgcn_readlane((int)(uint32_t)(v >> 32), l);
    return ((uint64_t)hi << 32) | lo;
}

__device__ __forceinline__ uint64_t gear_prefix(uint64_t g, uint32_t lane) {
#pragma unroll
    for (int k = 1; k < 64; k <<= 1) {
        const uint64_t t = __shfl_up(g, k);
        if (lane >= (uint32_t)k) g += t << k;
    }
    return g;
}

constexpr uint32_t kTruncMax = 47;
constexpr uint32_t kTruncNone = 63;
constexpr uint32_t kTruncUnknown = 62;
constexpr int kRecTShift = 24;

struct Regime {
    uint64_t rem, a0, ce, re, tl;
};

__device__ __forceinline__ Regime regime(const FastParams &fp, uint64_t s, uint64_t n) {
    Regime R;
    uint64_t rem = n - s, center = fp.avg;
    if (rem > fp.max) rem = fp.max; else if (rem < center) center = rem;
    R.rem = rem;
    R.a0 = (fp.min / 2) * 2;
    R.ce = (center / 2) * 2;
    R.re = (rem / 2) * 2;
    R.tl = min(R.a0 + (uint64_t)fp.trunc, R.re);
    return R;
}


constexpr int kCopies = 32;
constexpr uint32_t kEntCap = 64;
constexpr uint32_t kStep = 64;

__device__ __forceinline__ uint64_t gear_of(const uint64_t *tab, uint32_t rep_off, uint32_t w, int b) {
    const uint32_t addr = __builtin_amdgcn_perm(rep_off, w, 0x0c0c0004u | ((uint32_t)b << 8));
    return *reinterpret_cast<const uint64_t *>(reinterpret_cast<const char *>(tab) + addr);
}

struct G4 {
    uint64_t v[4];
};

__device__ __forceinline__ void look4(G4 &g, const uint64_t *tab, uint32_t rep, uint32_t w) {
#pragma unroll
    for (int b = 0; b < 4; ++b) g.v[b] = gear_of(tab, rep, w, b);
}

template <bool kAlign>
__device__ __forceinline__ void chain4_test(uint64_t &h, uint32_t &acc, const G4 &g, const FastParams &fp) {
#pragma unroll
    for (int i = 0; i < 4; ++i) {
        h = shl1_add(h, g.v[i]);
        acc = min(acc, cand_test<kAlign>(h, fp));
    }
}

__device__ __forceinline__ uint32_t word_of(const uint4 &v, int w) {
    return w == 0 ? v.x : w == 1 ? v.y : w == 2 ? v.z : v.w;
}

__device__ __forceinline__ uint4 ld16_guarded(const uint8_t *base, uint32_t p, uint32_t limit) {
    if (p + 16 <= limit) return ld16(as_global4(base + p));
    uint32_t w[4] = {0, 0, 0, 0};
    if (p < limit) {
        g_u8 *gb = as_global1(base);
        for (uint32_t j = 0; p + j < limit; ++j) w[j >> 2] |= (uint32_t)gb[p + j] << (8 * j);
    }
    return make_uint4(w[0], w[1], w[2], w[3]);
}

struct EntryList {
    uint32_t *pos, *hlo, *hhi, *cnt;
};

constexpr uint32_t kEntFix = 1u << 31;
constexpr uint32_t kEntPos = kEntFix - 1;

__device__ __forceinline__ void append_hits(bool hit, uint32_t pos, uint64_t h0, uint32_t &ne,
                                            const EntryList &E) {
    const uint64_t m = __ballot(hit);
    if (m) {
        if (hit) {
            const uint32_t below = __builtin_amdgcn_mbcnt_hi((uint32_t)(m >> 32),
                                                             __builtin_amdgcn_mbcnt_lo((uint32_t)m, 0u));
            const uint32_t slot = ne + below;
            if (slot < kEntCap) {
                E.pos[slot] = pos;
                E.hlo[slot] = (uint32_t)h0;
                E.hhi[slot] = (uint32_t)(h0 >> 32);
            }
        }
        ne += (uint32_t)__popcll(m);
    }
}

__device__ __forceinline__ void append_hits_d(bool hit, uint32_t pos, uint64_t h0, const uint4 &q, uint32_t &ne,
                                              const EntryList &E, uint4 *edat) {
    const uint64_t m = __ballot(hit);
    if (m) {
        if (hit) {
            const uint32_t below = __builtin_amdgcn_mbcnt_hi((uint32_t)(m >> 32),
                                                             __builtin_amdgcn_mbcnt_lo((uint32_t)m, 0u));
            const uint32_t slot = ne + below;
            if (slot < kEntCap) {
                E.pos[slot] = pos;
                E.hlo[slot] = (uint32_t)h0;
                E.hhi[slot] = (uint32_t)(h0 >> 32);
                edat[slot] = q;
            }
        }
        ne += (uint32_t)__popcll(m);
    }
}

template <bool kAlign>
__device__ __forceinline__ uint32_t quarter(uint64_t &h, const uint4 &v, const uint64_t *tab, uint32_t rep,
                                            const FastParams &fp) {
    G4 ga, gb;
    uint32_t acc = 0xffffffffu;
    look4(ga, tab, rep, v.x);
    SCHED_FENCE();
    look4(gb, tab, rep, v.y);
    SCHED_FENCE();
    chain4_test<kAlign>(h, acc, ga, fp);
    SCHED_FENCE();
    look4(ga, tab, rep, v.z);
    SCHED_FENCE();
    chain4_test<kAlign>(h, acc, gb, fp);
    SCHED_FENCE();
    look4(gb, tab, rep, v.w);
    SCHED_FENCE();
    chain4_test<kAlign>(h, acc, ga, fp);
    SCHED_FENCE();
    chain4_test<kAlign>(h, acc, gb, fp);
    SCHED_FENCE();
    return acc;
}

struct Q4 {
    uint4 q[4];
};

template <bool kAlign, int kLook>
__device__ __forceinline__ void process_step(const Q4 &C, uint64_t &h, uint32_t pos0, uint32_t &ne,
                                             const EntryList &E, const uint64_t *tab, uint32_t rep,
                                             const FastParams &fp) {
    if constexpr (kLook == 1) {
        G4 ga, gb;
        look4(ga, tab, rep, C.q[0].x);
        SCHED_FENCE();
#pragma unroll
        for (int q = 0; q < 4; ++q) {
            const uint64_t h0 = h;
            uint32_t acc = 0xffffffffu;
#pragma unroll
            for (int w = 0; w < 4; w += 2) {
                look4(gb, tab, rep, word_of(C.q[q], w + 1));
                SCHED_FENCE();
                chain4_test<kAlign>(h, acc, ga, fp);
                SCHED_FENCE();
                if (q < 3 || w < 2) {
                    look4(ga, tab, rep, w < 2 ? word_of(C.q[q], w + 2) : word_of(C.q[q + 1], 0));
                    SCHED_FENCE();
                }
                chain4_test<kAlign>(h, acc, gb, fp);
                SCHED_FENCE();
            }
            append_hits(acc == 0, pos0 + 16 * q, h0, ne, E);
        }
    } else {
        G4 ga0, ga1, gb0, gb1;
        look4(ga0, tab, rep, C.q[0].x);
        look4(ga1, tab, rep, C.q[0].y);
        SCHED_FENCE();
#pragma unroll
        for (int q = 0; q < 4; ++q) {
            const uint64_t h0 = h;
            uint32_t acc = 0xffffffffu;
            look4(gb0, tab, rep, C.q[q].z);
            look4(gb1, tab, rep, C.q[q].w);
            SCHED_FENCE();
            chain4_test<kAlign>(h, acc, ga0, fp);
            chain4_test<kAlign>(h, acc, ga1, fp);
            SCHED_FENCE();
            if (q < 3) {
                look4(ga0, tab, rep, C.q[q + 1].x);
                look4(ga1, tab, rep, C.q[q + 1].y);
                SCHED_FENCE();
            }
            chain4_test<kAlign>(h, acc, gb0, fp);
            chain4_test<kAlign>(h, acc, gb1, fp);
            SCHED_FENCE();
            append_hits(acc == 0, pos0 + 16 * q, h0, ne, E);
        }
    }
}

template <bool kAlign>
__device__ __forceinline__ void process_step_d(const Q4 &C, uint64_t &h, uint32_t pos0, uint32_t &ne,
                                               const EntryList &E, uint4 *edat, const uint64_t *tab, uint32_t rep,
                                               const FastParams &fp) {
    G4 ga, gb;
    look4(ga, tab, rep, C.q[0].x);
    SCHED_FENCE();
#pragma unroll
    for (int q = 0; q < 4; ++q) {
        const uint64_t h0 = h;
        uint32_t acc = 0xffffffffu;
#pragma unroll
        for (int w = 0; w < 4; w += 2) {
            look4(gb, tab, rep, word_of(C.q[q], w + 1));
            SCHED_FENCE();
            chain4_test<kAlign>(h, acc, ga, fp);
            SCHED_FENCE();
            if (q < 3 || w < 2) {
                look4(ga, tab, rep, w < 2 ? word_of(C.q[q], w + 2) : word_of(C.q[q + 1], 0));
                SCHED_FENCE();
            }
            chain4_test<kAlign>(h, acc, gb, fp);
            SCHED_FENCE();
        }
        append_hits_d(acc == 0, pos0 + 16 * q, h0, C.q[q], ne, E, edat);
    }
}

template <bool kNt = false>
__device__ __forceinline__ void gload_step(Q4 &X, const uint8_t *gp, uint64_t istride, uint32_t t) {
#pragma unroll
    for (int i = 0; i < 4; ++i)
        X.q[i] = kNt ? ld16_nt(as_global4(gp + i * istride + t * kStep)) : ld16(as_global4(gp + i * istride + t * kStep));
}

__device__ __forceinline__ void stage_step(Q4 &C, const Q4 &X, uint4 *wrow, const uint4 *rrow) {
#pragma unroll
    for (int i = 0; i < 4; ++i) wrow[i * 16 * 5] = X.q[i];
    __builtin_amdgcn_wave_barrier();
#pragma unroll
    for (int k = 0; k < 4; ++k) C.q[k] = rrow[k];
    __builtin_amdgcn_wave_barrier();
}

typedef const __attribute__((address_space(3))) uint64_t lds_u64;
typedef const __attribute__((address_space(3))) char lds_char;

#if CDC_SCAN_TRUNC
__device__ __noinline__ uint32_t scan_trunc(const uint8_t *base, uint32_t c, uint64_t avail, lds_u64 *ltab,
                                            uint32_t rep, uint32_t mn, uint32_t avg, uint32_t mx, uint32_t trunc,
                                            uint64_t mask_s, uint64_t mask_l) {
    const uint32_t a0 = (mn / 2) * 2, ce = (avg / 2) * 2, re = (mx / 2) * 2;
    if (avail - c < (uint64_t)mx || (uint64_t)a0 + 52 > avail - c) return kTruncUnknown;
    const uint32_t tl = min(a0 + trunc, re);
    if (tl <= a0) return kTruncNone;
    const uint32_t len = tl - a0;
    const uint64_t w0 = (uint64_t)c + a0;
    const uint64_t al = w0 & ~3ull;
    const uint32_t sh = (uint32_t)(w0 - al);
    uint32_t w[13];
#pragma unroll
    for (int i = 0; i < 13; ++i) w[i] = *(g_u32 *)(base + al + 4 * i);
    uint64_t h = 0;
    uint32_t t = kTruncNone;
#pragma unroll
    for (int k = 0; k < 12; ++k) {
        const uint32_t a = __builtin_amdgcn_alignbyte(w[k + 1], w[k], sh);
#pragma unroll
        for (int j = 0; j < 4; ++j) {
            const uint32_t d = 4 * k + j;
            if (d >= kTruncMax) break;
            const uint32_t addr = __builtin_amdgcn_perm(rep, a, 0x0c0c0004u | ((uint32_t)j << 8));
            h = shl1_add(h, *reinterpret_cast<lds_u64 *>(reinterpret_cast<lds_char *>(ltab) + addr));
            const bool hit = d < len && !(h & ((a0 + d) < ce ? mask_s : mask_l));
            t = (hit && t == kTruncNone) ? d : t;
        }
    }
    return t;
}

#endif

__device__ __forceinline__ void flush_span(uint64_t g, const uint8_t *base, uint32_t span_len, uint64_t avail,
                                           uint32_t sub_mask, uint32_t ne, const EntryList &E, const uint64_t *tab,
                                           uint32_t rep, const FastParams &fp, const Candidates &cand,
                                           uint32_t lane, const uint4 *edat = nullptr) {
    wave_sync_lds();
    uint32_t *cpos = cand.pos + g * cand.cap;
    if (ne > kEntCap) {
        if (lane == 0) cand.count[g] = cand.cap + 1;
        wave_sync_lds();
        return;
    }
    uint32_t hs = 0, hl = 0, my_pos = 0;
    const uint32_t wd = lane < ne ? E.pos[lane] : 0u;
    const bool keep = lane < ne && ((wd & kEntFix) || (wd & sub_mask) >= 48);
    if (lane < ne) E.cnt[lane] = 0;
    if (keep) {
        my_pos = wd & kEntPos;
        uint64_t hh = ((uint64_t)E.hhi[lane] << 32) | E.hlo[lane];
        const uint4 v = edat ? edat[lane] : ld16_guarded(base, my_pos, span_len);
#pragma unroll
        for (int w = 0; w < 4; ++w)
#pragma unroll
            for (int b = 0; b < 4; ++b) {
                const int j = 4 * w + b;
                hh = (hh << 1) + gear_of(tab, rep, word_of(v, w), b);
                if (my_pos + j < span_len) {
                    hs |= (uint32_t)((hh & fp.mask_s_sh) == 0) << j;
                    hl |= (uint32_t)((hh & fp.mask_l_sh) == 0) << j;
                }
            }
        E.cnt[lane] = __popc(hs | hl);
    }
    wave_sync_lds();
    uint32_t slot = 0, total = 0;
    for (uint32_t k = 0; k < ne; ++k) {
        const uint32_t c = E.cnt[k];
        total += c;
        if ((E.pos[k] & kEntPos) < my_pos) slot += c;
    }
    if (keep) {
        for (uint32_t m = hs | hl; m; m &= m - 1) {
            const uint32_t j = __builtin_ctz(m);
            uint32_t t = kTruncUnknown;
#if CDC_SCAN_TRUNC
            t = scan_trunc(base, my_pos + j, avail, (lds_u64 *)tab, rep, fp.min, fp.avg, fp.max, fp.trunc,
                           fp.mask_s_sh, fp.mask_l_sh);
#endif
            if (slot < cand.cap)
                cpos[slot] = (my_pos + j) | (t << kRecTShift) | (((hs >> j) & 1u) << 31) | (((hl >> j) & 1u) << 30);
            ++slot;
        }
    }
    if (lane == 0) cand.count[g] = total;
    wave_sync_lds();
}

template <int kW>
struct ScanLds {
    uint64_t tab[256 * kCopies];
    uint4 stage[kW][64 * 5];
    uint32_t epos[kW][kEntCap];
    uint32_t ehlo[kW][kEntCap];
    uint32_t ehhi[kW][kEntCap];
    uint32_t ecnt[kW][kEntCap];
};

#ifndef CDC_SCAN_DYN
#define CDC_SCAN_DYN 0
#endif
#ifdef CDC_SCAN_MAXW
#define CDC_SCAN_VGPR_ATTR __attribute__((amdgpu_flat_work_group_size(1, kW * 64), amdgpu_waves_per_eu(CDC_SCAN_MAXW)))
#else
#define CDC_SCAN_VGPR_ATTR __launch_bounds__(kW * 64, 1)
#endif
template <bool kAlign, int kW, int kLook, int kMode>
__global__ CDC_SCAN_VGPR_ATTR void scan_kernel(const StreamTable st, const FastParams fp,
                                                           const uint64_t *__restrict__ gear,
                                                           const Candidates cand, const Compact cp) {
#if CDC_SCAN_DYN
    extern __shared__ uint4 scan_dyn[];
    ScanLds<kW> &L = *reinterpret_cast<ScanLds<kW> *>(scan_dyn);
#else
    __shared__ ScanLds<kW> L;
#endif
    const uint64_t *tab = L.tab;
    for (int i = threadIdx.x; i < 256 * kCopies; i += kW * 64)
        L.tab[i] = gear[i / kCopies] << fp.tshift;
    if (blockIdx.x == 0 && threadIdx.x < kStatWords) cp.stats[threadIdx.x] = 0;
    __syncthreads();

    const uint32_t lane = threadIdx.x & 63;
    const uint32_t wave = threadIdx.x >> 6;
    const uint32_t rep = (lane & 31) * 8;
    const uint64_t span = 1ull << st.span_log2;
    const uint32_t sub_log2 = st.span_log2 - 6;
    const uint32_t sub = 1u << sub_log2;
    const uint32_t steps = sub / kStep;
    const uint32_t lo = lane << sub_log2;
    const uint64_t istride = 16ull * sub;
    const EntryList E{L.epos[wave], L.ehlo[wave], L.ehhi[wave], L.ecnt[wave]};
    const uint32_t rsel = ((lane >> 3) & 3) + 8 * (lane >> 5) + 4 * ((lane >> 2) & 1);
    uint4 *wrow = &L.stage[wave][rsel * 5 + (lane & 3)];
    const uint4 *rrow = &L.stage[wave][lane * 5];

    const uint64_t gstride = (uint64_t)gridDim.x * kW;
    auto next_full = [&](uint64_t g, uint32_t &si, uint64_t &off) {
        for (; g < st.total_spans; g += gstride) {
            locate(st, g, si, off);
            if (st.lens[si] - off >= span) break;
        }
        return g;
    };
    Q4 A, B, C;
    uint32_t si, wb = 0;
    uint64_t off;
    uint64_t g = next_full(CDC_SCAN_WAVE_MAJOR ? (uint64_t)wave * gridDim.x + blockIdx.x
                                               : (uint64_t)blockIdx.x * kW + wave, si, off);
    const uint8_t *base = nullptr, *gp = nullptr;
    auto prefetch = [&]() {
        base = st.ptrs[si] + off;
        gp = base + (uint64_t)rsel * sub + (lane & 3) * 16;
        wb = 0;
        if (off != 0 && lane < 48) wb = as_global1(base)[(int)lane - 48];
        gload_step(A, gp, istride, 0);
        SCHED_FENCE();
        gload_step<(bool)CDC_SCAN_NT_ODD>(B, gp, istride, 1);
        SCHED_FENCE();
    };
    if (g < st.total_spans) prefetch();
    while (g < st.total_spans) {
        uint32_t ne = 0;
        uint64_t h = 0;
        uint4 F0, F1, F2;
        stage_step(C, A, wrow, rrow);
        F0 = C.q[0];
        F1 = C.q[1];
        F2 = C.q[2];
        gload_step(A, gp, istride, 2);
        SCHED_FENCE();
#define CDC_PROC(POS)                                                                          \
    do {                                                                                       \
        if constexpr (kMode == 1) h ^= (uint64_t)(C.q[0].x ^ C.q[1].y ^ C.q[2].z ^ C.q[3].w);   \
        else process_step<kAlign, kLook>(C, h, POS, ne, E, tab, rep, fp);                      \
    } while (0)
#define CDC_SCAN_PAIR(T, LOAD_B, STAGE_A, LOAD_A)                                              \
    do {                                                                                       \
        CDC_PROC(lo + (T) * kStep);                                                            \
        SCHED_FENCE();                                                                         \
        stage_step(C, B, wrow, rrow);                                                          \
        if (LOAD_B && kMode != 2) gload_step<(bool)CDC_SCAN_NT_ODD>(B, gp, istride, (T) + 3);  \
        SCHED_FENCE();                                                                         \
        CDC_PROC(lo + ((T) + 1) * kStep);                                                      \
        SCHED_FENCE();                                                                         \
        if (STAGE_A) stage_step(C, A, wrow, rrow);                                             \
        if (LOAD_A && kMode != 2) gload_step(A, gp, istride, (T) + 4);                         \
        SCHED_FENCE();                                                                         \
    } while (0)
        uint32_t t = 0;
        for (; t + 4 < steps; t += 2) CDC_SCAN_PAIR(t, true, true, true);
        CDC_SCAN_PAIR(t, true, true, false);
        CDC_SCAN_PAIR(t + 2, false, false, false);
#undef CDC_SCAN_PAIR
#undef CDC_PROC
        const uint64_t g_cur = g, off_cur = off;
        const uint64_t avail_cur = st.lens[si] - off;
        const uint32_t wb_cur = wb;
        const uint8_t *base_cur = base;
        g = next_full(g + gstride, si, off);
        if (g < st.total_spans) prefetch();
        const uint64_t gw = lane < 48 ? L.tab[wb_cur * kCopies + (lane & 31)] : 0;
        const uint64_t hw = readlane_u64(gear_prefix(gw, lane), 47);
        h = wave_shr1(h, off_cur != 0 ? hw : 0);
        {
            uint64_t h0 = h;
            append_hits(quarter<kAlign>(h, F0, tab, rep, fp) == 0, lo | kEntFix, h0, ne, E);
            h0 = h;
            append_hits(quarter<kAlign>(h, F1, tab, rep, fp) == 0, (lo + 16) | kEntFix, h0, ne, E);
            h0 = h;
            append_hits(quarter<kAlign>(h, F2, tab, rep, fp) == 0, (lo + 32) | kEntFix, h0, ne, E);
        }
        flush_span(g_cur, base_cur, (uint32_t)span, avail_cur, sub - 1, ne, E, tab, rep, fp, cand, lane);
    }
    if (fp.diag & 64) {
        __syncthreads();
        if (threadIdx.x == 0)
            atomicMax((unsigned long long *)&cp.stats[kStatDiag0 + 6],
                      (unsigned long long)__builtin_amdgcn_s_memrealtime());
    }
}


constexpr int kDmaW = 8;
constexpr uint32_t kDiagDmaScan = 1024;

struct ScanDmaLds {
    uint64_t tab[256 * kCopies];
    uint4 ring[kDmaW][2][256];
    uint32_t epos[kDmaW][kEntCap];
    uint32_t ehlo[kDmaW][kEntCap];
    uint32_t ehhi[kDmaW][kEntCap];
    uint32_t ecnt[kDmaW][kEntCap];
    uint4 edat[kDmaW][kEntCap];
    uint32_t carry[kDmaW][64];
    uint4 recs[kDmaW][64];
};

typedef const __attribute__((address_space(4))) uint64_t c_u64;
typedef const __attribute__((address_space(4))) uint32_t c_u32;

__device__ __forceinline__ uint64_t cld(const uint64_t *p) { return *(c_u64 *)p; }

__device__ __forceinline__ void glds16(const uint8_t *gsrc, uint32_t lds_dst) {
    uint32_t keep;
    asm volatile("s_mov_b32 %0, m0\n\ts_mov_b32 m0, %2\n\ts_nop 0\n\tglobal_load_lds_dwordx4 %1, off\n\ts_mov_b32 m0, %0"
                 : "=&s"(keep)
                 : "v"(gsrc), "s"(lds_dst)
                 : "memory");
}

template <int N>
__device__ __forceinline__ void wait_vm() {
    asm volatile("s_waitcnt vmcnt(%0)" ::"i"(N) : "memory");
}

__device__ __forceinline__ void glds4(const uint8_t *gsrc, uint32_t lds_dst) {
    uint32_t keep;
    asm volatile("s_mov_b32 %0, m0\n\ts_mov_b32 m0, %2\n\ts_nop 0\n\tglobal_load_lds_dword %1, off\n\ts_mov_b32 m0, %0"
                 : "=&s"(keep)
                 : "v"(gsrc), "s"(lds_dst)
                 : "memory");
}

template <int kCtrl, int kRowMask>
__device__ __forceinline__ uint64_t dpp64(uint64_t v) {
    const uint32_t lo = (uint32_t)__builtin_amdgcn_update_dpp(0, (int)(uint32_t)v, kCtrl, kRowMask, 0xF, false);
    const uint32_t hi = (uint32_t)__builtin_amdgcn_update_dpp(0, (int)(uint32_t)(v >> 32), kCtrl, kRowMask, 0xF, false);
    return ((uint64_t)hi << 32) | lo;
}

__device__ __forceinline__ uint64_t wave_total_dpp(uint64_t v) {
    v += dpp64<0x111, 0xF>(v);
    v += dpp64<0x112, 0xF>(v);
    v += dpp64<0x114, 0xF>(v);
    v += dpp64<0x118, 0xF>(v);
    v += dpp64<0x142, 0xA>(v);
    v += dpp64<0x143, 0xC>(v);
    return readlane_u64(v, 63);
}

__device__ __forceinline__ void flush_span_d(uint64_t g, uint32_t sub_mask, uint32_t ne, const EntryList &E,
                                             const uint4 *edat, uint4 *recs, const uint64_t *tab, uint32_t rep,
                                             const FastParams &fp, const Candidates &cand, uint32_t lane) {
    wave_sync_lds();
    uint32_t hs = 0, hl = 0, my_pos = 0xFFFFFFFFu, cnt = 0;
    const bool ovf = ne > kEntCap;
    const uint32_t wd = lane < ne && !ovf ? E.pos[lane] : 0u;
    const bool keep = lane < ne && !ovf && ((wd & kEntFix) || (wd & sub_mask) >= 48);
    if (keep) {
        my_pos = wd & kEntPos;
        uint64_t hh = ((uint64_t)E.hhi[lane] << 32) | E.hlo[lane];
        const uint4 v = edat[lane];
#pragma unroll
        for (int w = 0; w < 4; ++w)
#pragma unroll
            for (int b = 0; b < 4; ++b) {
                const int j = 4 * w + b;
                hh = (hh << 1) + gear_of(tab, rep, word_of(v, w), b);
                hs |= (uint32_t)((hh & fp.mask_s_sh) == 0) << j;
                hl |= (uint32_t)((hh & fp.mask_l_sh) == 0) << j;
            }
        cnt = __popc(hs | hl);
    }
    uint32_t slot = 0, total = 0;
    const uint32_t nk = ovf ? 0u : ne;
    for (uint32_t k = 0; k < nk; ++k) {
        const uint32_t pk = (uint32_t)__builtin_amdgcn_readlane((int)my_pos, (int)k);
        const uint32_t ck = (uint32_t)__builtin_amdgcn_readlane((int)cnt, (int)k);
        total += ck;
        slot += pk < my_pos ? ck : 0u;
    }
    uint32_t *const rec = reinterpret_cast<uint32_t *>(recs);
    if (keep) {
        for (uint32_t m = hs | hl; m; m &= m - 1) {
            const uint32_t j = __builtin_ctz(m);
            if (slot < cand.cap)
                rec[slot] = (my_pos + j) | (kTruncUnknown << kRecTShift) | (((hs >> j) & 1u) << 31) |
                            (((hl >> j) & 1u) << 30);
            ++slot;
        }
    }
    wave_sync_lds();
    if (lane < cand.cap / 4)
        *reinterpret_cast<uint4 *>(cand.pos + g * cand.cap + 4 * lane) = recs[lane];
    if (lane == 0) cand.count[g] = ovf ? cand.cap + 1 : total;
    wave_sync_lds();
}

__device__ __forceinline__ void locate_c(const StreamTable &st, uint64_t g, uint32_t &si, uint64_t &off) {
    uint32_t lo = 0, hi = st.n;
    while (hi - lo > 1) {
        const uint32_t mid = (lo + hi) >> 1;
        if (cld(st.span_base + mid) <= g) lo = mid; else hi = mid;
    }
    si = lo;
    off = (g - cld(st.span_base + lo)) << st.span_log2;
}

template <bool kAlign>
__global__ __launch_bounds__(kDmaW * 64, 1) void scan_dma_kernel(const StreamTable st, const FastParams fp,
                                                                 const uint64_t *__restrict__ gear,
                                                                 const Candidates cand, const Compact cp) {
    __shared__ ScanDmaLds L;
    const uint64_t *tab = L.tab;
    for (int i = threadIdx.x; i < 256 * kCopies; i += kDmaW * 64)
        L.tab[i] = gear[i / kCopies] << fp.tshift;
    if (blockIdx.x == 0 && threadIdx.x < kStatWords) cp.stats[threadIdx.x] = 0;
    __syncthreads();

    const uint32_t lane = threadIdx.x & 63;
    const uint32_t wave = __builtin_amdgcn_readfirstlane(threadIdx.x >> 6);
    const uint32_t rep = (lane & 31) * 8;
    const uint64_t span = 1ull << st.span_log2;
    const uint32_t sub_log2 = st.span_log2 - 6;
    const uint32_t sub = 1u << sub_log2;
    const uint32_t steps = sub / kStep;
    const uint32_t lo = lane << sub_log2;
    const EntryList E{L.epos[wave], L.ehlo[wave], L.ehhi[wave], L.ecnt[wave]};
    uint4 *const edat = L.edat[wave];
    const uint64_t src_lane = (uint64_t)(lane & 15) * sub + (lane >> 4) * 16;
    const uint64_t istride = 16ull * sub;
    const uint32_t ring0 = (uint32_t)(uintptr_t)&L.ring[wave][0][0];
    const uint4 *rd0 = &L.ring[wave][0][(lane >> 4) * 64 + (lane & 15)];
    const uint64_t gstride = (uint64_t)gridDim.x * kDmaW;
    auto next_full = [&](uint64_t g, uint32_t &si, uint64_t &off) {
        for (; g < st.total_spans; g += gstride) {
            locate_c(st, g, si, off);
            if (cld(st.lens + si) - off >= span) break;
        }
        return g;
    };
    auto stream_ptr = [&](uint32_t si) {
        return reinterpret_cast<const uint8_t *>(cld(reinterpret_cast<const uint64_t *>(st.ptrs) + si));
    };
    auto issue = [&](const uint8_t *src, uint32_t slot) {
#pragma unroll
        for (int i = 0; i < 4; ++i) glds16(src + i * istride, ring0 + slot * 4096 + i * 1024);
    };
    const uint32_t carry0 = (uint32_t)(uintptr_t)&L.carry[wave][0];
    auto issue_carry = [&](const uint8_t *b, uint64_t o) {
        glds4(o != 0 ? b - 48 + 4 * (lane % 12) : b, carry0);
    };
    uint32_t si;
    uint64_t off;
    uint64_t g = next_full(CDC_SCAN_WAVE_MAJOR ? (uint64_t)wave * gridDim.x + blockIdx.x
                                               : (uint64_t)blockIdx.x * kDmaW + wave, si, off);
    const uint8_t *base = nullptr;
    if (g < st.total_spans) {
        base = stream_ptr(si) + off;
        issue_carry(base, off);
        issue(base + src_lane, 0);
        issue(base + src_lane + kStep, 1);
    }
    uint32_t slot = 0;
    bool first = true;
    while (g < st.total_spans) {
        const uint64_t g_cur = g, off_cur = off;
        const uint8_t *const base_cur = base;
        g = next_full(g + gstride, si, off);
        const bool more = g < st.total_spans;
        const uint8_t *const base_next = more ? stream_ptr(si) + off : base_cur;
        const uint64_t off_next = more ? off : 0;
        uint32_t ne = 0;
        uint64_t h = 0;
        uint32_t wb = 0;
        uint4 F0, F1, F2;
        for (uint32_t t = 0; t < steps; ++t) {
            if (t == 0) {
                if (first) wait_vm<4>(); else wait_vm<6>();
            } else if (t + 1 == steps) {
                wait_vm<5>();
            } else {
                wait_vm<4>();
            }
            Q4 C;
            const uint4 *rd = rd0 + slot * 256;
#pragma unroll
            for (int k = 0; k < 4; ++k) C.q[k] = rd[k * 16];
            if (t == 0 && lane < 48) wb = L.carry[wave][lane >> 2];
            asm volatile("s_waitcnt lgkmcnt(0)" ::: "memory");
            if (t + 2 < steps) {
                issue(base_cur + src_lane + (t + 2) * kStep, slot);
            } else if (t + 2 == steps) {
                issue_carry(base_next, off_next);
                issue(base_next + src_lane, slot);
            } else {
                issue(base_next + src_lane + kStep, slot);
            }
            if (t == 0) {
                F0 = C.q[0];
                F1 = C.q[1];
                F2 = C.q[2];
            }
            process_step_d<kAlign>(C, h, lo + t * kStep, ne, E, edat, tab, rep, fp);
            slot ^= 1;
        }
        first = false;
        base = base_next;
        wb = (wb >> (8 * (lane & 3))) & 0xFFu;
        const uint64_t gw = lane < 48 ? L.tab[wb * kCopies + (lane & 31)] << (47 - lane) : 0;
        const uint64_t hw = wave_total_dpp(gw);
        h = wave_shr1(h, off_cur != 0 ? hw : 0);
        {
            uint64_t h0 = h;
            append_hits_d(quarter<kAlign>(h, F0, tab, rep, fp) == 0, lo | kEntFix, h0, F0, ne, E, edat);
            h0 = h;
            append_hits_d(quarter<kAlign>(h, F1, tab, rep, fp) == 0, (lo + 16) | kEntFix, h0, F1, ne, E, edat);
            h0 = h;
            append_hits_d(quarter<kAlign>(h, F2, tab, rep, fp) == 0, (lo + 32) | kEntFix, h0, F2, ne, E, edat);
        }
        flush_span_d(g_cur, sub - 1, ne, E, edat, L.recs[wave], tab, rep, fp, cand, lane);
    }
    wait_vm<0>();
}

template <bool kAlign>
__global__ __launch_bounds__(64) void scan_tail_kernel(const StreamTable st, const FastParams fp,
                                                       const uint64_t *__restrict__ gear, const Candidates cand,
                                                       const uint64_t *__restrict__ tails) {
    __shared__ uint64_t tab[256 * kCopies];
    __shared__ uint32_t e_pos[kEntCap], e_hlo[kEntCap], e_hhi[kEntCap], e_cnt[kEntCap];
    for (int i = threadIdx.x; i < 256 * kCopies; i += 64) tab[i] = gear[i / kCopies] << fp.tshift;
    __syncthreads();
    const uint32_t lane = threadIdx.x;
    const uint32_t rep = (lane & 31) * 8;
    const uint64_t g = tails[blockIdx.x];
    const EntryList E{e_pos, e_hlo, e_hhi, e_cnt};
    uint32_t si;
    uint64_t off;
    locate(st, g, si, off);
    const uint8_t *base = st.ptrs[si] + off;
    const uint32_t span_len = (uint32_t)(st.lens[si] - off);
    const uint32_t sub_log2 = st.span_log2 - 6;
    const uint32_t sub = 1u << sub_log2;
    const uint32_t lo = lane << sub_log2;
    uint32_t ne = 0;
    uint64_t h = 0;
    const bool active = lo < span_len;
    if (active && off + lo != 0) {
        (void)quarter<kAlign>(h, ld16(as_global4(base + lo - 48)), tab, rep, fp);
        (void)quarter<kAlign>(h, ld16(as_global4(base + lo - 32)), tab, rep, fp);
        (void)quarter<kAlign>(h, ld16(as_global4(base + lo - 16)), tab, rep, fp);
    }
    for (uint32_t it = 0; it < sub / 16; ++it) {
        const uint32_t p = lo + 16 * it;
        bool hit = false;
        const uint64_t h0 = h;
        if (active && p < span_len) hit = quarter<kAlign>(h, ld16_guarded(base, p, span_len), tab, rep, fp) == 0;
        append_hits(hit, p | kEntFix, h0, ne, E);
    }
    flush_span(g, base, span_len, span_len, 0, ne, E, tab, rep, fp, cand, lane);
}



#ifndef CDC_RES_WAVES
#define CDC_RES_WAVES 8
#endif
#ifndef CDC_WALK_SPANS
#define CDC_WALK_SPANS 8
#endif
#ifndef CDC_WIN_RECS
#define CDC_WIN_RECS 768
#endif
constexpr int kResWaves = CDC_RES_WAVES;
#ifndef CDC_RES_LINK_DIAG
#define CDC_RES_LINK_DIAG 0
#endif
#ifndef CDC_RES_HOSTREL
#define CDC_RES_HOSTREL 1
#endif
#ifndef CDC_WALK_COOP
#define CDC_WALK_COOP 1
#endif
#ifndef CDC_RES_FASTTRUNC
#define CDC_RES_FASTTRUNC 1
#endif
constexpr int kResThreads = kResWaves * 64;

__device__ __forceinline__ uint32_t trunc_words(const uint8_t *data, uint64_t w0, uint32_t len, uint64_t a0,
                                                uint64_t ce, uint64_t mask_s, uint64_t mask_l, lds_u64 *tab) {
    const uint64_t al = w0 & ~3ull;
    const uint32_t sh = (uint32_t)(w0 - al);
    uint32_t w[13];
#pragma unroll
    for (int i = 0; i < 13; ++i) w[i] = *(g_u32 *)(data + al + 4 * i);
    uint64_t h = 0;
    uint32_t t = kTruncNone;
#pragma unroll
    for (int k = 0; k < 12; ++k) {
        const uint32_t a = __builtin_amdgcn_alignbyte(w[k + 1], w[k], sh);
#pragma unroll
        for (int j = 0; j < 4; ++j) {
            const uint32_t d = 4 * k + j;
            if (d >= kTruncMax) break;
            h = shl1_add(h, tab[(a >> (8 * j)) & 255]);
            const bool hit = d < len && !(h & ((a0 + d) < ce ? mask_s : mask_l));
            t = (hit && t == kTruncNone) ? d : t;
        }
    }
    return t;
}

#ifndef CDC_RES_CALLS
#define CDC_RES_CALLS __forceinline__
#endif
__device__ CDC_RES_CALLS uint32_t trunc_at(const uint8_t *data, uint64_t n, uint64_t c, uint64_t mask_s,
                                          uint64_t mask_l, uint32_t mn, uint32_t avg, uint32_t mx, uint32_t trunc,
                                          lds_u64 *tab) {
    if (n - c <= mn) return kTruncNone;
    uint64_t rem = n - c, center = avg;
    if (rem > mx) rem = mx; else if (rem < center) center = rem;
    const uint64_t a0 = (mn / 2) * 2, ce = (center / 2) * 2, re = (rem / 2) * 2;
    const uint64_t tl = min(a0 + (uint64_t)trunc, re);
    if (tl <= a0) return kTruncNone;
    const uint32_t len = (uint32_t)(tl - a0);
    const uint64_t w0 = c + a0;
    if ((w0 & ~3ull) + 52 <= n) return trunc_words(data, w0, len, a0, ce, mask_s, mask_l, tab);
    uint64_t h = 0;
    for (uint32_t d = 0; d < len; ++d) {
        h = (h << 1) + tab[as_global1(data)[w0 + d]];
        if (!(h & ((a0 + d) < ce ? mask_s : mask_l))) return d;
    }
    return kTruncNone;
}

__device__ __forceinline__ uint32_t trunc_call(const uint8_t *data, uint64_t n, uint64_t c, const FastParams &fp,
                                               const uint64_t *tab) {
    return trunc_at(data, n, c, fp.mask_s, fp.mask_l, fp.min, fp.avg, fp.max, fp.trunc, (lds_u64 *)tab);
}

__device__ CDC_RES_CALLS uint64_t coop_next_bytes(uint32_t mn, uint32_t avg, uint32_t mx, uint64_t mask_s,
                                                 uint64_t mask_l, const uint64_t *tab, const uint8_t *data,
                                                 uint64_t n, uint64_t s, uint32_t lane) {
    if (n - s <= mn) return n;
    FastParams fp{};
    fp.min = mn;
    fp.avg = avg;
    fp.max = mx;
    const Regime R = regime(fp, s, n);
    uint64_t h = 0;
    for (uint64_t b = R.a0; b < R.re; b += 64) {
        const uint64_t p1 = min(b + 64, R.re);
        const uint64_t p = b + lane;
        const bool in = p < p1;
        const uint64_t gv = in ? tab[as_global1(data)[s + p]] : 0;
        const uint64_t x = gear_prefix(gv, lane) + ((h << lane) << 1);
        const bool hit = in && !(x & (p < R.ce ? mask_s : mask_l));
        const uint64_t m = __ballot(hit);
        if (m) return s + b + (uint64_t)(__ffsll((long long)m) - 1);
        h = __shfl(x, (int)(p1 - b - 1));
    }
    return s + R.rem;
}

__device__ __forceinline__ void load_tab1(uint64_t *tab, const uint64_t *gear) {
    for (int i = threadIdx.x; i < 256; i += blockDim.x) tab[i] = gear[i];
    __syncthreads();
}

__device__ __forceinline__ uint64_t wave_sum(uint64_t v) {
#pragma unroll
    for (int k = 1; k < 64; k <<= 1) v += __shfl_xor(v, k);
    return v;
}

__device__ __forceinline__ uint64_t lane_next_global(const StreamTable &st, const FastParams &fp,
                                                     const Candidates &cand, const uint64_t *tab,
                                                     const uint8_t *data, uint64_t n, uint64_t gbase, uint64_t s) {
    if (n - s <= fp.min) return n;
    const Regime R = regime(fp, s, n);
    const uint32_t t = trunc_call(data, n, s, fp, tab);
    if (t != kTruncNone) return s + R.a0 + t;
    if (R.tl >= R.re) return s + R.rem;
    const uint64_t lo = s + R.tl, hi = s + R.re;
    for (uint64_t sp = lo >> st.span_log2; (sp << st.span_log2) < hi; ++sp) {
        const uint64_t g = gbase + sp;
        const uint32_t cnt = cand.count[g];
        if (cnt > cand.cap) return ~0ull;
        const uint32_t *P = cand.pos + g * cand.cap;
        const uint64_t sp0 = sp << st.span_log2;
        const uint32_t lo_rel = lo > sp0 ? (uint32_t)(lo - sp0) : 0u;
        uint32_t a = 0, b = cnt;
        while (a < b) {
            const uint32_t m = (a + b) >> 1;
            if ((P[m] & kCandPosMask) < lo_rel) a = m + 1; else b = m;
        }
        for (uint32_t j = a; j < cnt; ++j) {
            const uint32_t r = P[j];
            const uint64_t c = sp0 + (r & kCandPosMask);
            if (c >= hi) return s + R.rem;
            if (r & ((c - s) < R.ce ? kCandHitS : kCandHitL)) return c;
        }
    }
    return s + R.rem;
}

struct LaneSpan {
    bool act, first;
    uint32_t si;
    uint64_t g, off, span_end, n, gbase;
    const uint8_t *data;
};

struct ChainWin;
__device__ __forceinline__ void emit_start(ChainWin &W, const Chains &ch, const LaneSpan &L, uint32_t l, uint64_t s,
                                           uint32_t &cnt, uint64_t &entry);
__device__ __forceinline__ void walk_lanes(const StreamTable &st, const FastParams &fp, const Candidates &cand,
                                           const uint64_t *tab, ChainWin &W, const Chains &ch, const LaneSpan &L,
                                           uint32_t lane, bool go, uint64_t s, uint32_t &cnt, uint64_t &entry,
                                           uint64_t &exit, uint64_t &steps) {
    cnt = 0;
    entry = ~0ull;
    go = go && s < L.span_end;
    for (;;) {
        bool need = false;
        if (go) {
            emit_start(W, ch, L, lane, s, cnt, entry);
            ++steps;
            const uint64_t nx = lane_next_global(st, fp, cand, tab, L.data, L.n, L.gbase, s);
            if (nx == ~0ull) need = true; else s = nx;
            go = !need && s < L.span_end;
        }
        for (uint64_t m = __ballot(need); m; m &= m - 1) {
            const int l = __ffsll((long long)m) - 1;
            const uint64_t sl = readlane_u64(s, l), nl = readlane_u64(L.n, l);
            const uint8_t *dl = reinterpret_cast<const uint8_t *>(readlane_u64(reinterpret_cast<uint64_t>(L.data), l));
            const uint64_t nx = coop_next_bytes(fp.min, fp.avg, fp.max, fp.mask_s, fp.mask_l, tab, dl, nl, sl, lane);
            if ((int)lane == l) {
                s = nx;
                go = s < L.span_end;
            }
        }
        if (__ballot(go) == 0) break;
    }
    if (cnt == 0) entry = s;
    exit = s;
}

constexpr int kWalkSpans = CDC_WALK_SPANS;
#ifndef CDC_WARM_SPANS
#define CDC_WARM_SPANS 2
#endif
constexpr int kWarmSpans = CDC_WARM_SPANS;
constexpr int kWinSlots = kWarmSpans + kWalkSpans + 1;
constexpr int kReach = kWarmSpans + kWalkSpans;
constexpr uint32_t kWinRecs = CDC_WIN_RECS;
constexpr uint32_t kVirt = 128;
constexpr int kBlockSpans = kResWaves * kWalkSpans;
constexpr uint64_t kNoDep = ~0ull;
constexpr uint64_t kAgg = 1, kInc = 2;
constexpr uint32_t kSpinMax = 1u << 26;

constexpr uint32_t kLdsStarts = 24;
constexpr int kKeyShift = 40;
constexpr uint64_t kKeyPos = (1ull << kKeyShift) - 1;

struct ChainWin {
    uint64_t key[kWinRecs];
    uint32_t rec[kWinRecs];
    uint32_t link[kWinRecs + kVirt];
    uint16_t lrec[kWinRecs + kVirt];
    uint8_t rslot[kWinRecs];
    uint8_t vslot[kVirt];
    uint64_t vpos[kVirt];
    uint32_t st[kWalkSpans][kLdsStarts];
    uint64_t soff[kWinSlots];
    uint64_t slen[kWinSlots];
    const uint8_t *sptr[kWinSlots];
    uint32_t ssi[kWinSlots];
    uint32_t scnt[kWinSlots];
    uint32_t pre[kWinSlots + 1];
    uint32_t wpre[kWalkSpans + 1];
    uint32_t nrec, nvirt;
};

struct BlockState {
    uint64_t E[kBlockSpans];
    uint64_t X[kBlockSpans];
    uint32_t N[kBlockSpans];
    uint8_t F[kBlockSpans];
    uint64_t b, base, pred;
    uint64_t t0;
    uint32_t rewalk;
    uint64_t stat[kResWaves][3];
    uint64_t diag[kResWaves][kStatDiagN];
};

__device__ __forceinline__ uint64_t skey(uint32_t si) { return (uint64_t)si << kKeyShift; }

__device__ __forceinline__ uint32_t win_lower(const ChainWin &W, uint64_t k) {
    uint32_t a = 0, b = W.nrec;
    while (a < b) {
        const uint32_t m = (a + b) >> 1;
        if (W.key[m] < k) a = m + 1; else b = m;
    }
    return a;
}

__device__ __forceinline__ uint32_t win_entry_at(const ChainWin &W, uint32_t si, uint64_t p) {
    const uint64_t k = skey(si) | p;
    const uint32_t f = win_lower(W, k);
    if (f < W.nrec && W.key[f] == k) return f + 1;
    for (uint32_t v = 0; v < W.nvirt; ++v)
        if (W.vpos[v] == p && W.ssi[W.vslot[v]] == si) return kWinRecs + v + 1;
    return 0;
}

__device__ __forceinline__ uint64_t win_search(const ChainWin &W, uint32_t si, uint64_t c, const Regime &R,
                                               uint32_t i0, uint32_t *lr) {
    *lr = 0;
    const uint64_t s = skey(si);
    const uint64_t lo = s | (c + R.tl), hi = s | (c + R.re), ce = s | (c + R.ce);
    for (uint32_t i = i0; i < W.nrec; ++i) {
        const uint64_t k = W.key[i];
        if (k >= hi) break;
        if (k >= lo && (W.rec[i] & (k < ce ? kCandHitS : kCandHitL))) {
            *lr = i + 1;
            return k & kKeyPos;
        }
    }
    return c + R.rem;
}

template <bool kTrKnown>
__device__ __forceinline__ uint64_t win_next(const ChainWin &W, const FastParams &fp, const uint64_t *tab,
                                             const uint8_t *data, uint64_t n, uint32_t si, uint64_t c,
                                             uint32_t i0, uint32_t tr, uint32_t *lr) {
    *lr = 0;
    if (n - c <= fp.min) return n;
    const Regime R = regime(fp, c, n);
    if (R.tl > R.a0) {
        const uint32_t t = kTrKnown ? tr : trunc_call(data, n, c, fp, tab);
        if (t != kTruncNone) return c + R.a0 + t;
    }
    if (R.tl >= R.re) return c + R.rem;
    if (fp.diag & 8) return c + R.rem;
    return win_search(W, si, c, R, i0, lr);
}

__device__ __forceinline__ uint32_t virt_alloc(bool mk, uint32_t &nv) {
    const uint64_t m = __ballot(mk);
    const uint32_t below = __builtin_amdgcn_mbcnt_hi((uint32_t)(m >> 32), __builtin_amdgcn_mbcnt_lo((uint32_t)m, 0u));
    const uint32_t v = nv + below;
    nv += (uint32_t)__popcll(m);
    return v < kVirt ? v : kVirt;
}

__device__ __forceinline__ void emit_start(ChainWin &W, const Chains &ch, const LaneSpan &L, uint32_t l, uint64_t s,
                                           uint32_t &cnt, uint64_t &entry) {
    if (s >= L.off) {
        if (cnt < kLdsStarts) W.st[l][cnt] = (uint32_t)(s - L.off);
        else if (cnt < ch.smax) ch.starts[L.g * ch.smax + cnt] = s;
        if (cnt == 0) entry = s;
        ++cnt;
    }
}

__device__ __forceinline__ void walk_window(ChainWin &W, const FastParams &fp, const uint64_t *tab,
                                            const LaneSpan &L, const Chains &ch, uint32_t lane, bool go, uint64_t s,
                                            uint32_t wr, uint32_t &cnt, uint64_t &entry, uint64_t &exit,
                                            uint64_t &steps) {
    cnt = 0;
    entry = ~0ull;
    go = go && s < L.span_end;
    for (;;) {
        while (go) {
            emit_start(W, ch, L, lane, s, cnt, entry);
            if (wr == 0) break;
            const uint32_t d = W.link[wr - 1];
            if (d == 0) break;
            wr = W.lrec[wr - 1];
            s += d;
            go = s < L.span_end;
        }
        if (!__ballot(go)) break;
#if CDC_WALK_COOP
        static_assert(kWalkSpans == 8, "walkers are lanes 0..7");
        {
            const int wl = (int)(lane & 7);
            const uint32_t jj = lane >> 3;
            const uint64_t c0 = __shfl(s, wl);
            const bool g0 = __shfl(go ? 1 : 0, wl) != 0;
            const uint64_t nw = __shfl(L.n, wl);
            const uint32_t siw = (uint32_t)__shfl((int)L.si, wl);
            const uint8_t *dw = reinterpret_cast<const uint8_t *>(__shfl(reinterpret_cast<uint64_t>(L.data), wl));
            const uint64_t cj = c0 + (uint64_t)jj * fp.max;
            uint64_t nx = 0;
            uint32_t lrj = 0;
            if (g0 && cj < nw) nx = win_next<false>(W, fp, tab, dw, nw, siw, cj, win_lower(W, skey(siw) | cj), 0, &lrj);
            bool run = go;
            uint64_t cur = s;
#pragma unroll
            for (int j = 0; j < 8; ++j) {
                const uint64_t n_j = __shfl(nx, wl + 8 * j);
                const uint32_t l_j = (uint32_t)__shfl((int)lrj, wl + 8 * j);
                if (run) {
                    ++steps;
                    const uint64_t c_next = cur + fp.max;
                    if (j < 7 && l_j == 0 && n_j == c_next && c_next < L.span_end) {
                        emit_start(W, ch, L, lane, c_next, cnt, entry);
                        cur = c_next;
                    } else {
                        s = n_j;
                        wr = l_j;
                        go = s < L.span_end;
                        run = false;
                    }
                }
            }
        }
#else
        if (go) {
            ++steps;
            uint32_t lr;
            s = win_next<false>(W, fp, tab, L.data, L.n, L.si, s, win_lower(W, skey(L.si) | s), 0, &lr);
            wr = lr;
            go = s < L.span_end;
        }
#endif
    }
    if (cnt == 0) entry = s;
    exit = s;
}

__device__ __forceinline__ void wave_settle(const StreamTable &st, const FastParams &fp, const Candidates &cand,
                                            const uint64_t *tab, const Chains &ch, ChainWin &W, bool dense,
                                            const LaneSpan &L, uint32_t lane, uint32_t k0, bool has0,
                                            uint64_t pred0, BlockState &B, uint64_t &rewalks, uint64_t &steps) {
    const bool mine = lane < kWalkSpans && L.act;
    uint64_t E = mine ? B.E[k0 + lane] : 0, X = mine ? B.X[k0 + lane] : 0;
    for (;;) {
        uint64_t pred = __shfl_up(X, 1);
        if (lane == 0) pred = pred0;
        const bool mism = mine && !L.first && (lane > 0 || has0) && E != pred;
        const uint64_t m = __ballot(mism);
        if (m == 0) break;
        const bool ready = mism && !(lane > 0 && ((m >> (lane - 1)) & 1ull));
        uint32_t cnt = 0;
        uint64_t entry = 0, exit = 0;
        if (dense)
            walk_lanes(st, fp, cand, tab, W, ch, L, lane, ready, pred, cnt, entry, exit, steps);
        else
            walk_window(W, fp, tab, L, ch, lane, ready, pred, ready ? win_entry_at(W, L.si, pred) : 0u, cnt, entry,
                        exit, steps);
        if (ready) {
            B.E[k0 + lane] = E = entry;
            B.X[k0 + lane] = X = exit;
            B.N[k0 + lane] = cnt;
            ++rewalks;
        }
    }
}

struct LinkItem {
    bool act, fast;
    int j;
    uint32_t e, i0, si, len;
    uint32_t known;
    uint64_t c, n, a0, ce, w0;
    const uint8_t *data;
};

__device__ __forceinline__ LinkItem link_item(const ChainWin &W, const FastParams &fp, bool virt, uint32_t x,
                                              uint32_t e1) {
    LinkItem it{};
    it.known = kTruncUnknown;
    it.act = x < e1;
    if (!it.act) return it;
    if (virt) {
        it.e = kWinRecs + x;
        it.j = W.vslot[x];
        it.c = W.vpos[x];
        it.i0 = win_lower(W, skey(W.ssi[it.j]) | it.c);
    } else {
        it.e = x;
        it.j = W.rslot[x];
        it.c = W.key[x] & kKeyPos;
        it.i0 = x + 1;
        it.known = (W.rec[x] >> kRecTShift) & 63u;
    }
    it.si = W.ssi[it.j];
    it.n = W.slen[it.j];
    it.data = W.sptr[it.j];
    if (it.n - it.c > fp.min) {
        const Regime R = regime(fp, it.c, it.n);
        if (R.tl > R.a0) {
            it.len = (uint32_t)(R.tl - R.a0);
            it.a0 = R.a0;
            it.ce = R.ce;
            it.w0 = it.c + R.a0;
            it.fast = (it.w0 & ~3ull) + 52 <= it.n && it.known == kTruncUnknown;
        }
    }
    return it;
}

__device__ __forceinline__ void item_load(const LinkItem &it, const void *safe, uint32_t (&w)[13]) {
    if (!__ballot(it.fast)) return;
    const uint8_t *src = it.fast ? it.data + (it.w0 & ~3ull) : static_cast<const uint8_t *>(safe);
#pragma unroll
    for (int i = 0; i < 13; ++i) w[i] = *(g_u32 *)(src + 4 * i);
}

__device__ __forceinline__ uint32_t item_trunc(const LinkItem &it, const uint32_t (&w)[13], const FastParams &fp,
                                               const uint64_t *tab, const uint64_t *tabs) {
    if (!it.act || it.len == 0) return kTruncNone;
    if (it.known != kTruncUnknown) return it.known;
    if (!it.fast) return trunc_call(it.data, it.n, it.c, fp, tab);
    const uint32_t r = (uint32_t)(it.w0 & 3);
    const uint32_t ns = it.ce > it.a0 ? (uint32_t)min(it.ce - it.a0, (uint64_t)64) : 0u;
    if (CDC_RES_FASTTRUNC && fp.cm_align && it.len == kTruncMax && ns >= kTruncMax) {
        const uint32_t ms = (uint32_t)(fp.mask_s_sh >> 32);
        uint64_t h = 0;
        uint32_t acc = 0xFFFFFFFFu;
#pragma unroll
        for (int k0 = 0; k0 < 12; k0 += 3) {
            uint64_t g[12];
#pragma unroll
            for (int k = 0; k < 3; ++k) {
                const uint32_t a = __builtin_amdgcn_alignbyte(w[k0 + k + 1], w[k0 + k], r);
#pragma unroll
                for (int b = 0; b < 4; ++b) g[4 * k + b] = tabs[(a >> (8 * b)) & 255];
            }
#pragma unroll
            for (int i = 0; i < 12; ++i) {
                if (4 * k0 + i >= (int)kTruncMax) break;
                h = shl1_add(h, g[i]);
                acc = min(acc, (uint32_t)(h >> 32) & ms);
            }
        }
        if (acc != 0) return kTruncNone;
    }
    uint64_t h = 0, hits = 0;
#pragma unroll
    for (int k0 = 0; k0 < 12; k0 += 3) {
        uint64_t g[12];
#pragma unroll
        for (int k = 0; k < 3; ++k) {
            const uint32_t a = __builtin_amdgcn_alignbyte(w[k0 + k + 1], w[k0 + k], r);
#pragma unroll
            for (int b = 0; b < 4; ++b) g[4 * k + b] = tab[(a >> (8 * b)) & 255];
        }
#pragma unroll
        for (int i = 0; i < 12; ++i) {
            const uint32_t d = 4 * k0 + i;
            if (d >= kTruncMax) break;
            h = shl1_add(h, g[i]);
            hits |= (uint64_t)((h & (d < ns ? fp.mask_s : fp.mask_l)) == 0) << d;
        }
    }
    hits &= it.len >= 64 ? ~0ull : (1ull << it.len) - 1;
    return hits ? (uint32_t)__builtin_ctzll(hits) : kTruncNone;
}

__device__ __forceinline__ void item_link(ChainWin &W, const FastParams &fp, const uint64_t *tab,
                                          const LinkItem &it, uint32_t tr, uint32_t sl2, uint32_t &nv) {
    bool mk = false;
    uint64_t nx = 0;
    uint32_t lr = 0;
    int jt = 0;
    if (it.act) {
        nx = win_next<true>(W, fp, tab, nullptr, it.n, it.si, it.c, it.i0, tr, &lr);
        W.link[it.e] = (uint32_t)(nx - it.c);
        jt = it.j + (int)((nx - W.soff[it.j]) >> sl2);
        mk = lr == 0 && nx < it.n && jt < kReach && W.ssi[jt] == it.si;
    }
    const uint32_t v = virt_alloc(mk, nv);
    if (mk && v < kVirt) {
        W.vpos[v] = nx;
        W.vslot[v] = (uint8_t)jt;
        lr = kWinRecs + v + 1;
    }
    if (it.act) W.lrec[it.e] = (uint16_t)lr;
}

__device__ __forceinline__ uint64_t ld_agent(const uint64_t *p) {
    return __hip_atomic_load((g_u64 *)const_cast<uint64_t *>(p), __ATOMIC_RELAXED, __HIP_MEMORY_SCOPE_AGENT);
}
__device__ __forceinline__ void st_agent(uint64_t *p, uint64_t v) {
    __hip_atomic_store((g_u64 *)p, v, __ATOMIC_RELAXED, __HIP_MEMORY_SCOPE_AGENT);
}

__device__ __forceinline__ void publish(const Resolve &rs, uint64_t b, uint64_t status, uint64_t cnt, uint64_t E,
                                        uint64_t X, uint32_t lane) {
    if (lane == 0) {
        if (status == kAgg) {
            st_agent(&rs.dagg[b], cnt);
            st_agent(&rs.dE[b], E);
            st_agent(&rs.dXa[b], X);
        } else {
            st_agent(&rs.dinc[b], cnt);
            st_agent(&rs.dXi[b], X);
        }
        asm volatile("s_waitcnt vmcnt(0)" ::: "memory");
        st_agent(&rs.dstat[b], (rs.gen << 2) | status);
    }
}

__device__ __forceinline__ bool wait_final(const Resolve &rs, uint64_t j) {
    const uint64_t inc = (rs.gen << 2) | kInc;
    for (uint32_t k = 0; k < kSpinMax; ++k) {
        if (ld_agent(&rs.dstat[j]) == inc) {
            __builtin_amdgcn_fence(__ATOMIC_ACQUIRE, "wavefront");
            return true;
        }
        __builtin_amdgcn_s_sleep(2);
    }
    return false;
}

constexpr int kLbGroups = 4;

__device__ int lookback(const Resolve &rs, uint64_t b, uint64_t Eb, uint32_t lane, uint64_t &acc, uint64_t &pred) {
    const uint64_t agg_w = (rs.gen << 2) | kAgg, inc_w = (rs.gen << 2) | kInc;
    for (uint32_t attempt = 0; attempt < 1024; ++attempt) {
        acc = 0;
        uint64_t expect = Eb;
        int64_t j0 = (int64_t)b - 1;
        int64_t stale = -1;
        for (;;) {
            int64_t j[kLbGroups];
            uint64_t w[kLbGroups];
#pragma unroll
            for (int k = 0; k < kLbGroups; ++k) {
                j[k] = j0 - (int64_t)lane - 64 * k;
                w[k] = j[k] >= 0 ? 0 : inc_w;
            }
            int kl = kLbGroups - 1;
            uint32_t ll = 63;
            uint64_t mi[kLbGroups];
            for (uint32_t spins = 0;; ++spins) {
#pragma unroll
                for (int k = 0; k < kLbGroups; ++k)
                    if (w[k] != agg_w && w[k] != inc_w) w[k] = ld_agent(&rs.dstat[j[k]]);
                bool ready = true, found = false;
#pragma unroll
                for (int k = 0; k < kLbGroups; ++k) {
                    mi[k] = __ballot(w[k] == inc_w);
                    const uint64_t mp = __ballot(w[k] == agg_w || w[k] == inc_w);
                    if (found) continue;
                    if (mi[k]) {
                        found = true;
                        kl = k;
                        ll = (uint32_t)__ffsll((long long)mi[k]) - 1;
                        const uint64_t need = (2ull << ll) - 1;
                        if ((mp & need) != need) ready = false;
                    } else if (mp != ~0ull) {
                        ready = false;
                    }
                }
                if (!found) {
                    kl = kLbGroups - 1;
                    ll = 63;
                }
                if (ready) break;
                if (spins >= kSpinMax) return -1;
                __builtin_amdgcn_s_sleep(2);
            }
            __builtin_amdgcn_fence(__ATOMIC_ACQUIRE, "wavefront");
            uint64_t cnt[kLbGroups], E[kLbGroups], X[kLbGroups];
#pragma unroll
            for (int k = 0; k < kLbGroups; ++k) {
                const bool in = k < kl || (k == kl && lane <= ll);
                const bool inc = w[k] == inc_w;
                cnt[k] = 0;
                E[k] = kNoDep;
                X[k] = 0;
                if (j[k] >= 0 && in) {
                    cnt[k] = ld_agent(inc ? &rs.dinc[j[k]] : &rs.dagg[j[k]]);
                    X[k] = ld_agent(inc ? &rs.dXi[j[k]] : &rs.dXa[j[k]]);
                    if (!inc) E[k] = ld_agent(&rs.dE[j[k]]);
                }
            }
            int64_t bad = -1;
#pragma unroll
            for (int k = 0; k < kLbGroups; ++k) {
                if (k > kl) break;
                uint64_t En = __shfl_up(E[k], 1);
                if (lane == 0) En = k == 0 ? expect : readlane_u64(E[k - 1], 63);
                const bool in = k < kl || lane <= ll;
                const uint64_t mb = __ballot(in && En != kNoDep && X[k] != En);
                if (mb && bad < 0) bad = 64 * k + (__ffsll((long long)mb) - 1);
            }
            if (bad >= 0) {
                stale = j0 - bad + 1;
                break;
            }
            uint64_t part = 0;
#pragma unroll
            for (int k = 0; k < kLbGroups; ++k)
                if (k < kl || (k == kl && lane <= ll)) part += cnt[k];
            acc += wave_sum(part);
            if (mi[kl]) return 1;
            expect = readlane_u64(E[kLbGroups - 1], 63);
            j0 -= 64 * kLbGroups;
        }
        if (stale == (int64_t)b) {
            if (!wait_final(rs, b - 1)) return -1;
            acc = ld_agent(&rs.dinc[b - 1]);
            pred = ld_agent(&rs.dXi[b - 1]);
            return pred == Eb ? 1 : 0;
        }
        if (!wait_final(rs, (uint64_t)stale)) return -1;
    }
    return -1;
}

__device__ __forceinline__ uint64_t ld_nt(const uint64_t *p) {
    return __builtin_nontemporal_load((const g_u64 *)p);
}

#define CDC_DIAG_T(k)                                                  \
    do {                                                               \
        if ((fp.diag & 128) && !(CDC_RES_LINK_DIAG && (fp.diag & 8192))) { \
            const uint64_t t_ = __builtin_amdgcn_s_memrealtime();       \
            dt[k] += t_ - t_prev;                                      \
            t_prev = t_;                                               \
        }                                                              \
    } while (0)

#ifndef CDC_RES_ATTR
#define CDC_RES_ATTR __launch_bounds__(kResThreads, 2)
#endif
__global__ CDC_RES_ATTR void resolve_kernel(const StreamTable st, const FastParams fp,
                                                              const uint64_t *__restrict__ gear,
                                                              const Candidates cand, const Chains ch,
                                                              const Compact cp, const Resolve rs,
                                                              cdc_chunk_pod *out, uint64_t out_cap) {
    __shared__ uint64_t tab[256];
    __shared__ uint64_t tabs[256];
    __shared__ ChainWin win[kResWaves];
    __shared__ BlockState B;
    if (threadIdx.x == 0) {
        if (fp.diag & 64) B.t0 = __builtin_amdgcn_s_memrealtime();
        B.b = atomicAdd((unsigned long long *)&cp.stats[kStatOrder], 1ull);
        B.base = B.pred = 0;
        B.rewalk = 0;
    }
    for (int i = threadIdx.x; i < 256; i += blockDim.x) tabs[i] = gear[i] << fp.tshift;
    load_tab1(tab, gear);
    const uint64_t b = B.b;
    const uint32_t lane = threadIdx.x & 63, wave = threadIdx.x >> 6;
    const uint32_t sl2 = st.span_log2;
    const uint64_t span = 1ull << sl2;
    const uint64_t g0 = b * kBlockSpans;
    const uint32_t nsp = (uint32_t)min((uint64_t)kBlockSpans, st.total_spans - g0);
    const uint32_t k0 = wave * kWalkSpans;
    const uint64_t G0 = g0 + k0;
    const uint32_t cap = cand.cap;
    ChainWin &W = win[wave];
    uint64_t t_prev = (fp.diag & 128) ? __builtin_amdgcn_s_memrealtime() : 0;
    uint64_t dt[kStatDiagN] = {};
    uint64_t steps = 0, rewalks = 0, cstat = 0;
    LaneSpan L{};
    bool dense = false;

    if (k0 < nsp) {
        const int64_t gfirst = (int64_t)G0 - kWarmSpans;
        if (lane < kWinSlots) {
            const int64_t g = gfirst + lane;
            uint32_t si = ~0u, c = 0;
            uint64_t off = 0, n = 0;
            const uint8_t *p = nullptr;
            if (g >= 0 && (uint64_t)g < st.total_spans) {
                locate(st, (uint64_t)g, si, off);
                c = cand.count[g];
                n = st.lens[si];
                p = st.ptrs[si];
            }
            W.ssi[lane] = si;
            W.soff[lane] = off;
            W.scnt[lane] = c;
            W.slen[lane] = n;
            W.sptr[lane] = p;
        }
        wave_sync_lds();
        if (lane == 0) {
            uint32_t acc = 0;
            bool dn = (fp.diag & 2) != 0;
#pragma unroll 1
            for (int j = 0; j < kWinSlots; ++j) {
                W.pre[j] = acc;
                const uint32_t c = W.scnt[j];
                if (c > cap) dn = true; else acc += c;
            }
            if (acc > kWinRecs) dn = true;
            W.pre[kWinSlots] = dn ? 0 : acc;
            W.nrec = dn ? 0 : acc;
            W.nvirt = dn ? 1u : 0u;
        }
        wave_sync_lds();
        dense = W.nvirt != 0;
        if (lane < kWalkSpans && k0 + lane < nsp) {
            const int j = kWarmSpans + (int)lane;
            L.act = true;
            L.g = G0 + lane;
            L.si = W.ssi[j];
            L.off = W.soff[j];
            L.n = W.slen[j];
            L.data = W.sptr[j];
            L.gbase = L.g - (L.off >> sl2);
            L.span_end = min(L.off + span, L.n);
            L.first = L.off == 0;
            const uint32_t c = W.scnt[j];
            cstat = c > cap ? 1ull : (uint64_t)c << 24;
        }
        CDC_DIAG_T(0);
        uint32_t cnt = 0;
        uint64_t entry = 0, exit = 0;
        if (dense) {
            uint64_t s0 = 0;
            if (L.act && !L.first) s0 = L.off > kWarmSpans * span ? L.off - kWarmSpans * span : 0;
            if (L.act && !L.first && (fp.diag & 1)) s0 = L.off;
            walk_lanes(st, fp, cand, tab, W, ch, L, lane, L.act, s0, cnt, entry, exit, steps);
        } else {
            const uint32_t nrec = W.nrec;
            {
                uint32_t v[kWinSlots];
#pragma unroll
                for (int j = 0; j < kWinSlots; ++j) {
                    const uint32_t c = W.scnt[j];
                    v[j] = cand.pos[lane < c ? (uint64_t)(gfirst + j) * cap + lane : 0];
                }
#pragma unroll 1
                for (int j = 0; j < kWinSlots; ++j) {
                    const uint64_t kb = skey(W.ssi[j]) | W.soff[j];
                    const uint32_t c = W.scnt[j], p0 = W.pre[j];
                    for (uint32_t k = lane; k < c; k += 64) {
                        const uint32_t r = k < 64 ? v[0] : cand.pos[(uint64_t)(gfirst + j) * cap + k];
                        W.rec[p0 + k] = r;
                        W.key[p0 + k] = kb + (r & kCandPosMask);
                        W.rslot[p0 + k] = (uint8_t)j;
                    }
#pragma unroll
                    for (int q = 0; q + 1 < kWinSlots; ++q) v[q] = v[q + 1];
                }
            }
            wave_sync_lds();
            CDC_DIAG_T(1);
            const uint32_t nlink = W.pre[kReach];
            for (uint32_t i = nlink + lane; i < nrec; i += 64) W.link[i] = 0;
            uint32_t nv = 0, e0 = 0, e1 = nlink;
            bool virt = false;
            for (;;) {
                LinkItem A = link_item(W, fp, virt, e0 + lane, e1);
                uint32_t wa[13];
                item_load(A, gear, wa);
                for (uint32_t base = e0; base < e1; base += 64) {
                    constexpr bool kLinkDiag = CDC_RES_LINK_DIAG;
                    uint64_t f0 = (kLinkDiag && (fp.diag & 8192)) ? __builtin_amdgcn_s_memrealtime() : 0;
                    const LinkItem B2 = link_item(W, fp, virt, base + 64 + lane, e1);
                    uint32_t wb[13];
                    item_load(B2, gear, wb);
                    uint64_t f1 = (kLinkDiag && (fp.diag & 8192)) ? __builtin_amdgcn_s_memrealtime() : 0;
                    const uint32_t tr = (fp.diag & 4) ? kTruncNone : item_trunc(A, wa, fp, tab, tabs);
                    if (kLinkDiag && (fp.diag & 8192)) __builtin_amdgcn_s_waitcnt(0);
                    uint64_t f2 = (kLinkDiag && (fp.diag & 8192)) ? __builtin_amdgcn_s_memrealtime() : 0;
                    item_link(W, fp, tab, A, tr, sl2, nv);
                    if (kLinkDiag && (fp.diag & 8192)) {
                        const uint64_t f3 = __builtin_amdgcn_s_memrealtime();
                        const int o = virt ? 3 : 0;
                        dt[o] += f1 - f0;
                        dt[o + 1] += f2 - f1;
                        dt[o + 2] += f3 - f2;
                    }
                    A = B2;
#pragma unroll
                    for (int i = 0; i < 13; ++i) wa[i] = wb[i];
                }
                wave_sync_lds();
                if (!virt) CDC_DIAG_T(4);
                const uint32_t vend = min(nv, kVirt);
                if (virt ? e1 >= vend : vend == 0) break;
                e0 = virt ? e1 : 0;
                e1 = vend;
                virt = true;
            }
            if (lane == 0) W.nvirt = min(nv, kVirt);
            wave_sync_lds();
            CDC_DIAG_T(3);
            uint64_t s = 0;
            uint32_t wr = 0;
            if (L.act && !L.first && L.off >= kWarmSpans * span) {
                const int jw = (int)lane;
                if (W.pre[jw + 1] > W.pre[jw]) {
                    wr = W.pre[jw] + 1;
                    s = W.key[W.pre[jw]] & kKeyPos;
                } else {
                    s = W.soff[jw];
                }
            }
            if (L.act && !L.first && (fp.diag & 1)) {
                s = L.off;
                wr = 0;
            }
            walk_window(W, fp, tab, L, ch, lane, L.act, s, wr, cnt, entry, exit, steps);
        }
        if (L.act) {
            B.E[k0 + lane] = entry;
            B.X[k0 + lane] = exit;
            B.N[k0 + lane] = cnt;
            B.F[k0 + lane] = L.first ? 1 : 0;
        }
        CDC_DIAG_T(5);
    }
    __syncthreads();

#pragma unroll 1
    for (int round = 0; round < 2; ++round) {
        bool need;
        if (round == 0) {
            const uint32_t k = threadIdx.x;
            need = __syncthreads_or(k > 0 && k < nsp && !B.F[k] && B.E[k] != B.X[k - 1]) != 0;
        } else {
            if (wave == 0) {
                uint64_t C = 0;
                for (uint32_t k = lane; k < nsp; k += 64) C += B.N[k];
                C = wave_sum(C);
                const uint64_t Eb = B.F[0] ? kNoDep : B.E[0];
                const uint64_t Xb = B.X[nsp - 1];
                uint64_t acc = 0, pred = 0;
                int ok = 1;
                if (b > 0) {
                    publish(rs, b, kAgg, C, Eb, Xb, lane);
                    ok = lookback(rs, b, Eb, lane, acc, pred);
                }
                if (ok != 0) publish(rs, b, kInc, acc + C, 0, Xb, lane);
                if (lane == 0) {
                    B.base = acc;
                    B.pred = pred;
                    B.rewalk = ok == 0 ? 1u : 0u;
                    if (ok < 0) atomicAdd((unsigned long long *)&cp.stats[kStatError], 1ull);
                }
                CDC_DIAG_T(6);
            }
            __syncthreads();
            need = B.rewalk != 0;
        }
        if (need) {
            for (uint32_t w2 = 0; w2 < (uint32_t)kResWaves; ++w2) {
                if (wave == w2 && k0 < nsp)
                    wave_settle(st, fp, cand, tab, ch, W, dense, L, lane, k0, w2 > 0 || round > 0,
                                w2 > 0 ? B.X[k0 - 1] : B.pred, B, rewalks, steps);
                __syncthreads();
            }
        }
    }
    CDC_DIAG_T(2);
    if (B.rewalk && wave == 0) {
        uint64_t C = 0;
        for (uint32_t k = lane; k < nsp; k += 64) C += B.N[k];
        C = wave_sum(C);
        publish(rs, b, kInc, B.base + C, 0, B.X[nsp - 1], lane);
    }

    if (k0 < nsp) {
        uint32_t wpre0 = 0;
        for (uint32_t k = 0; k < k0; ++k) wpre0 += B.N[k];
        const uint32_t myN = L.act ? B.N[k0 + lane] : 0;
        uint32_t x = myN;
#pragma unroll
        for (int o = 1; o < kWalkSpans; o <<= 1) {
            const uint32_t t = __shfl_up(x, o);
            if (lane >= (uint32_t)o) x += t;
        }
        if (lane < kWalkSpans) W.wpre[lane + 1] = x;
        if (lane == 0) W.wpre[0] = 0;
        const uint32_t wtot = (uint32_t)__shfl(x, kWalkSpans - 1);
        const uint64_t obase = B.base + wpre0;
        const bool bad = __ballot(L.act && myN > ch.smax) != 0 || obase + wtot > out_cap;
        asm volatile("s_waitcnt vmcnt(0)" ::: "memory");
        wave_sync_lds();
        if (!bad) {
            for (uint32_t i = lane; i < wtot; i += 64) {
                int k = 0;
                while (k + 1 < kWalkSpans && W.wpre[k + 1] <= i) ++k;
                const uint32_t r = i - W.wpre[k];
                const uint64_t *list = ch.starts + (G0 + k) * ch.smax;
                const uint64_t off_k = W.soff[kWarmSpans + k];
                const uint64_t s0 = r < kLdsStarts ? off_k + W.st[k][r] : ld_nt(list + r);
                const uint64_t nx = r + 1 >= B.N[k0 + k] ? B.X[k0 + k]
                                    : r + 1 < kLdsStarts ? off_k + W.st[k][r + 1] : ld_nt(list + r + 1);
                out[obase + i] = cdc_chunk_pod{s0, nx - s0};
            }
            if (L.act) {
                if (L.first) cp.h_first[L.si] = obase + x - myN;
                if (L.g + 1 == st.total_spans) cp.h_first[st.n] = obase + x;
            }
        }
        const uint64_t cs = wave_sum(cstat), rw = wave_sum(rewalks), sp = wave_sum(steps);
        if (lane == 0) {
            B.stat[wave][0] = cs;
            B.stat[wave][1] = rw;
            B.stat[wave][2] = sp + (bad ? (1ull << 40) : 0);
        }
        CDC_DIAG_T(7);
    } else if (lane == 0) {
        B.stat[wave][0] = B.stat[wave][1] = B.stat[wave][2] = 0;
    }
    if ((fp.diag & 128) && lane == 0)
        for (int k = 0; k < kStatDiagN; ++k) B.diag[wave][k] = dt[k];
#if CDC_RES_HOSTREL >= 3
    __threadfence_system();
#elif CDC_RES_HOSTREL >= 1
    asm volatile("s_waitcnt vmcnt(0)" ::: "memory");
#endif
    __syncthreads();
    if (threadIdx.x == 0) {
        uint64_t cs = 0, rw = 0, sp = 0;
        for (int w = 0; w < kResWaves; ++w) {
            cs += B.stat[w][0];
            rw += B.stat[w][1];
            sp += B.stat[w][2];
        }
        if (fp.diag & 64) {
            const uint64_t t1 = __builtin_amdgcn_s_memrealtime(), t0 = B.t0;
            unsigned long long *d = (unsigned long long *)&cp.stats[kStatDiag0];
            atomicMax(d + 0, (unsigned long long)~t0);
            atomicMax(d + 1, (unsigned long long)t0);
            atomicMax(d + 2, (unsigned long long)t1);
            atomicMax(d + 3, (unsigned long long)~t1);
            atomicMax(d + 4, (unsigned long long)(t1 - t0));
            atomicAdd(d + 5, (unsigned long long)(t1 - t0));
        } else if (fp.diag & 128)
            for (int k = 0; k < kStatDiagN; ++k) {
                uint64_t d = 0;
                for (int w = 0; w < kResWaves; ++w) d += B.diag[w][k];
                atomicAdd((unsigned long long *)&cp.stats[kStatDiag0 + k], (unsigned long long)d);
            }
        const uint64_t err = sp >> 40;
        sp &= (1ull << 40) - 1;
        if (cs) atomicAdd((unsigned long long *)&cp.stats[kStatCand], (unsigned long long)cs);
        if (rw) atomicAdd((unsigned long long *)&cp.stats[kStatRewalk], (unsigned long long)rw);
        if (sp) atomicAdd((unsigned long long *)&cp.stats[kStatOnDemand], (unsigned long long)sp);
        if (err) atomicAdd((unsigned long long *)&cp.stats[kStatError], (unsigned long long)err);
#if CDC_RES_HOSTREL >= 2
        __threadfence_system();
#else
        __threadfence();
#endif
        if (atomicAdd((unsigned long long *)&cp.stats[kStatTicket], 1ull) + 1 == gridDim.x) {
            __threadfence_system();
            for (int i = 0; i < kStatWords; ++i)
                if (i != kStatDone) cp.h_stats[i] = ld_agent(&cp.stats[i]);
            const uint64_t c = cp.h_stats[kStatCand];
            cp.h_stats[kStatCand] = c >> 24;
            cp.h_stats[kStatOvf] = c & 0xFFFFFF;
            __threadfence_system();
            cp.h_stats[kStatDone] = 1;
        }
    }
}
#undef CDC_DIAG_T

}

#ifdef CDC_OVL
namespace ovl {
#endif

template <bool kAlign, int kW, int kLook, int kMode>
static hipError_t scan_launch(unsigned grid, const StreamTable &st, const FastParams &fp, const uint64_t *d_gear,
                              const Candidates &cand, const Compact &cp, hipStream_t s) {
    size_t lds = 0;
    if (CDC_SCAN_DYN) {
        lds = sizeof(ScanLds<kW>);
        static bool attr = false;
        if (!attr) {
            const hipError_t e = hipFuncSetAttribute(reinterpret_cast<const void *>(&scan_kernel<kAlign, kW, kLook, kMode>),
                                                     hipFuncAttributeMaxDynamicSharedMemorySize, (int)lds);
            if (e != hipSuccess) return e;
            attr = true;
        }
    }
    scan_kernel<kAlign, kW, kLook, kMode><<<grid, kW * 64, lds, s>>>(st, fp, d_gear, cand, cp);
    return hipSuccess;
}

hipError_t launch_scan(const StreamTable &st, const FastParams &fp, const uint64_t *d_gear,
                       const Candidates &cand, const Compact &cp, const uint64_t *d_tails, uint32_t n_tails,
                       int num_cus, hipStream_t s) {
    if (!st.total_spans) return hipSuccess;
    if (n_tails) {
        if (fp.cm_align)
            scan_tail_kernel<true><<<n_tails, 64, 0, s>>>(st, fp, d_gear, cand, d_tails);
        else
            scan_tail_kernel<false><<<n_tails, 64, 0, s>>>(st, fp, d_gear, cand, d_tails);
    }
    constexpr int W = CDC_SCAN_WAVES, K = CDC_SCAN_LOOK;
    const uint32_t mode = (fp.diag >> 8) & 3;
    if (mode == 0 && (fp.diag & kDiagDmaScan)) {
        const uint64_t groups = (st.total_spans + kDmaW - 1) / kDmaW;
        const unsigned grid = (unsigned)(groups < (uint64_t)num_cus ? groups : (uint64_t)num_cus);
        if (fp.cm_align)
            scan_dma_kernel<true><<<grid, kDmaW * 64, 0, s>>>(st, fp, d_gear, cand, cp);
        else
            scan_dma_kernel<false><<<grid, kDmaW * 64, 0, s>>>(st, fp, d_gear, cand, cp);
        return hipGetLastError();
    }
    const uint64_t groups = (st.total_spans + W - 1) / W;
    const unsigned grid = (unsigned)(groups < (uint64_t)num_cus ? groups : (uint64_t)num_cus);
    hipError_t e;
    if (mode == 1 && fp.cm_align)
        e = scan_launch<true, W, K, 1>(grid, st, fp, d_gear, cand, cp, s);
    else if (mode == 2 && fp.cm_align)
        e = scan_launch<true, W, K, 2>(grid, st, fp, d_gear, cand, cp, s);
    else if (fp.cm_align)
        e = scan_launch<true, W, K, 0>(grid, st, fp, d_gear, cand, cp, s);
    else
        e = scan_launch<false, W, K, 0>(grid, st, fp, d_gear, cand, cp, s);
    return e != hipSuccess ? e : hipGetLastError();
}

uint64_t resolve_blocks(uint64_t spans) { return (spans + kBlockSpans - 1) / kBlockSpans; }

hipError_t launch_resolve(const StreamTable &st, const FastParams &fp, const uint64_t *d_gear,
                          const Candidates &cand, const Chains &ch, const Compact &cp, const Resolve &rs,
                          void *d_out, uint64_t out_cap, hipStream_t s) {
    if (!st.total_spans) return hipSuccess;
    resolve_kernel<<<(unsigned)resolve_blocks(st.total_spans), kResThreads, 0, s>>>(
        st, fp, d_gear, cand, ch, cp, rs, reinterpret_cast<cdc_chunk_pod *>(d_out), out_cap);
    return hipGetLastError();
}

#ifdef CDC_OVL
}
#endif
}
}
```

### chunkfs_amd/csrc/fastcdc.hpp

```cpp
#pragma once
#include "cdc_kernels.hpp"

namespace cdc {
namespace p3 {

struct Chains {
    uint32_t smax;
    uint64_t *starts;
};

struct Compact {
    uint64_t *stats;
    uint64_t *h_stats;
    uint64_t *h_first;
};

struct Resolve {
    uint64_t *dstat;
    uint64_t *dagg;
    uint64_t *dinc;
    uint64_t *dE;
    uint64_t *dXa;
    uint64_t *dXi;
    uint64_t gen;
};

constexpr int kStatCand = 0;
constexpr int kStatOvf = 1;
constexpr int kStatRewalk = 2;
constexpr int kStatError = 3;
constexpr int kStatOrder = 4;
constexpr int kStatOnDemand = 5;
constexpr int kStatTicket = 6;
constexpr int kStatDone = 7;
constexpr int kStatDiag0 = 8;
constexpr int kStatDiagN = 8;
constexpr int kStatWords = kStatDiag0 + kStatDiagN;

uint64_t resolve_blocks(uint64_t spans);

hipError_t launch_scan(const StreamTable &st, const FastParams &fp, const uint64_t *d_gear,
                       const Candidates &cand, const Compact &cp, const uint64_t *d_tails, uint32_t n_tails,
                       int num_cus, hipStream_t s);
hipError_t launch_resolve(const StreamTable &st, const FastParams &fp, const uint64_t *d_gear,
                          const Candidates &cand, const Chains &ch, const Compact &cp, const Resolve &rs,
                          void *d_out, uint64_t out_cap, hipStream_t s);

namespace ovl {
uint64_t resolve_blocks(uint64_t spans);
hipError_t launch_scan(const StreamTable &st, const FastParams &fp, const uint64_t *d_gear,
                       const Candidates &cand, const Compact &cp, const uint64_t *d_tails, uint32_t n_tails,
                       int num_cus, hipStream_t s);
hipError_t launch_resolve(const StreamTable &st, const FastParams &fp, const uint64_t *d_gear,
                          const Candidates &cand, const Chains &ch, const Compact &cp, const Resolve &rs,
                          void *d_out, uint64_t out_cap, hipStream_t s);
}

}
}
```

Measured before the change: 4304.

## Template resolve kernel geometry and add runtime-selectable waves and warm spans

```diff
diff --git a/chunkfs_amd/build.py b/chunkfs_amd/build.py
--- a/chunkfs_amd/build.py
+++ b/chunkfs_amd/build.py
@@ -10,6 +10,7 @@
 SOURCES = ["fastcdc.hip", "fastcdc_ovl.hip", "small.hip", "walk.hip", "util_kernels.hip", "sha256.hip", "index.hip", "engine.cpp", "hostpath.cpp", "capi.cpp",
            "index_host.cpp"]
 HEADERS = ["fastcdc.hpp", "small.hpp", "walk.hpp", "cdc_kernels.hpp", "sha256.hpp", "index.hpp", "engine.hpp"]
+REMARKS = ("fastcdc.hip",)
 ARCH = "gfx950"
 HIPCC = os.environ.get("HIPCC", "/opt/rocm/bin/hipcc")
 CFLAGS = ["-O3", "-std=c++17", "-fPIC", f"--offload-arch={ARCH}", "-Wall", "-Wno-unused-result"]
@@ -55,13 +56,42 @@
         o = os.path.join(bdir, src + ".o")
         objs.append(o)
         deps = [s] + common + ([os.path.join(CSRC, "fastcdc.hip")] if src == "fastcdc_ovl.hip" else [])
-        if force or _newer(o, deps):
+        remarks = o + ".remarks.txt" if src in REMARKS else None
+        if force or _newer(o, deps) or (remarks and not os.path.exists(remarks)):
             lang = ["-x", "hip"] if src.endswith(".hip") else []
-            _run([HIPCC] + CFLAGS + [f"-D{d}" for d in defines] + lang + ["-c", s, "-o", o])
+            cmd = [HIPCC] + CFLAGS + [f"-D{d}" for d in defines] + lang + ["-c", s, "-o", o]
+            if remarks:
+                print("+", " ".join(cmd), "-Rpass-analysis=kernel-resource-usage", flush=True)
+                r = subprocess.run(cmd + ["-Rpass-analysis=kernel-resource-usage"], stderr=subprocess.PIPE, text=True)
+                other = [l for l in r.stderr.splitlines() if "remark:" not in l and not l.startswith((" ", "\t"))]
+                if other:
+                    print("\n".join(other), file=sys.stderr, flush=True)
+                if r.returncode:
+                    sys.stderr.write(r.stderr)
+                    raise subprocess.CalledProcessError(r.returncode, cmd)
+                with open(remarks, "w") as fh:
+                    fh.write("\n".join(l for l in r.stderr.splitlines() if "remark:" in l) + "\n")
+            else:
+                _run(cmd)
     if force or _newer(out_lib, objs):
         _run([HIPCC, f"--offload-arch={ARCH}", "-shared", "-fPIC", "-o", out_lib] + objs)
     return out_lib
 
 
+def resource_remarks(src="fastcdc.hip"):
+    import re
+    out, cur = {}, None
+    with open(os.path.join(BUILD, src + ".o.remarks.txt")) as fh:
+        for line in fh:
+            m = re.search(r"remark: +Function Name: (\S+)", line)
+            if m:
+                cur = out.setdefault(m.group(1), {})
+                continue
+            m = re.search(r"remark: +([A-Za-z ]+?)(?: \[[^\]]*\])?: (\d+)", line)
+            if m and cur is not None:
+                cur[m.group(1)] = int(m.group(2))
+    return out
+
+
 if __name__ == "__main__":
     build(force="--force" in sys.argv)
diff --git a/chunkfs_amd/csrc/engine.cpp b/chunkfs_amd/csrc/engine.cpp
--- a/chunkfs_amd/csrc/engine.cpp
+++ b/chunkfs_amd/csrc/engine.cpp
@@ -118,6 +118,28 @@
         }
         if (const char *v = std::getenv("CHUNKFS_AMD_SPAN"))
             e->span_log2_ = (uint32_t)std::max<int>(std::atoi(v), (int)std::max(l2, 14u));
+        {
+            e->res_waves_ = 8;
+            e->res_warm_ = 2;
+            if (const char *v = std::getenv("CHUNKFS_AMD_RES_WAVES")) {
+                const int w = std::atoi(v);
+                if (w != 8 && w != 12) {
+                    set_error("CHUNKFS_AMD_RES_WAVES must be 8 or 12");
+                    delete e;
+                    return CDC_EINVAL;
+                }
+                e->res_waves_ = w;
+            }
+            if (const char *v = std::getenv("CHUNKFS_AMD_WARM_SPANS")) {
+                const int w = std::atoi(v);
+                if (w < 0 || w > 2) {
+                    set_error("CHUNKFS_AMD_WARM_SPANS must be 0, 1 or 2");
+                    delete e;
+                    return CDC_EINVAL;
+                }
+                e->res_warm_ = w;
+            }
+        }
         e->small_span_log2_ = l2 > 14 ? l2 : 14;
         if (const char *v = std::getenv("CHUNKFS_AMD_SMALL_SPAN")) {
             const int x = std::atoi(v);
@@ -362,7 +384,7 @@
     }
     const size_t o_starts = take(S * smax * 8);
     const size_t o_first = take((N + 1) * 8);
-    const uint64_t nb = std::max(p3::resolve_blocks(S), p3::ovl::resolve_blocks(S)) + 2;
+    const uint64_t nb = std::max(p3::resolve_blocks(S, res_waves_), p3::ovl::resolve_blocks(S)) + 2;
     const size_t o_desc = take(6 * nb * 8);
     (void)hipFree(ws_);
     ws_ = nullptr;
@@ -738,12 +760,14 @@
     tev_timed_[seq % kTimeRing] = timed;
     rec.timed = timed;
     if (timed) HIP_TRY(hipEventRecord(ev[0], s));
+    const int warm = res_warm_ ? res_warm_ : p3::resolve_warm_spans(sl2);
     if (!ovl) {
         if (spans)
             HIP_TRY(p3::launch_scan(st, fp_, d_gear_, f.cand, cp, zero_copy ? h_tails : f.d_tails, f.n_tails,
                                     num_cus_, s));
         if (timed) HIP_TRY(hipEventRecord(ev[1], s));
-        if (spans) HIP_TRY(p3::launch_resolve(st, fp_, d_gear_, f.cand, ch3_, cp, rs, d_out, out_cap, s));
+        if (spans)
+            HIP_TRY(p3::launch_resolve(st, fp_, d_gear_, f.cand, ch3_, cp, rs, d_out, out_cap, res_waves_, warm, s));
         if (timed) HIP_TRY(hipEventRecord(ev[2], s));
     } else {
         static_assert(kSlots > kHostSlots, "device slots must outlast the host blocks");
@@ -757,7 +781,8 @@
         HIP_TRY(hipEventRecord(scan_ev_[slot], s));
         HIP_TRY(hipStreamWaitEvent(res_stream_, scan_ev_[slot], 0));
         if (spans && ovl_std_)
-            HIP_TRY(p3::launch_resolve(st, fp_, d_gear_, f.cand, ch3_, cp, rs, d_out, out_cap, res_stream_));
+            HIP_TRY(p3::launch_resolve(st, fp_, d_gear_, f.cand, ch3_, cp, rs, d_out, out_cap, res_waves_, warm,
+                                       res_stream_));
         else if (spans)
             HIP_TRY(p3::ovl::launch_resolve(st, fp_, d_gear_, f.cand, ch3_, cp, rs, d_out, out_cap, res_stream_));
         if (timed) HIP_TRY(hipEventRecord(ev[2], res_stream_));
@@ -829,14 +854,14 @@
         const uint64_t *d = h_misc + p3::kStatDiag0;
         const uint64_t s0 = ~d[0], s1 = d[1], e1 = d[2], e0 = ~d[3];
         const double blocks =
-            (double)(b.ovl && !ovl_std_ ? p3::ovl::resolve_blocks(b.spans) : p3::resolve_blocks(b.spans));
+            (double)(b.ovl && !ovl_std_ ? p3::ovl::resolve_blocks(b.spans) : p3::resolve_blocks(b.spans, res_waves_));
         std::fprintf(stderr, "resolve blocks, us: scan's last block end -> first start %.2f  starts spread %.2f  "
                              "first start -> first end %.2f  -> last end %.2f  longest block %.2f  mean block %.2f\n",
                      ((double)s0 - (double)d[6]) / 100.0, (s1 - s0) / 100.0, (e0 - s0) / 100.0, (e1 - s0) / 100.0,
                      d[4] / 100.0, d[5] / 100.0 / (blocks ? blocks : 1.0));
     } else if (fp_.diag & 128) {
         const double waves = b.ovl && !ovl_std_ ? (double)p3::ovl::resolve_blocks(b.spans) * 4
-                                                : (double)p3::resolve_blocks(b.spans) * 8;
+                                                : (double)p3::resolve_blocks(b.spans, res_waves_) * res_waves_;
         std::fprintf(stderr, (fp_.diag & 8192) ? "resolve link passes, us per wave (records: issue trunc link; "
                                                  "virtual: issue trunc link; -; -):"
                                                : "resolve phases, us per wave (meta recs settle+wait virtual-links "
diff --git a/chunkfs_amd/csrc/engine.hpp b/chunkfs_amd/csrc/engine.hpp
--- a/chunkfs_amd/csrc/engine.hpp
+++ b/chunkfs_amd/csrc/engine.hpp
@@ -154,6 +154,8 @@
     FastParams fp_{};
     uint32_t span_log2_ = 16;
     uint32_t small_span_log2_ = 16;
+    int res_waves_ = 8;
+    int res_warm_ = 2;
     static constexpr uint64_t kSmallBatch = uint64_t(8) << 20;
     static constexpr size_t kZeroCopyStreams = 64;
     uint32_t cap_ = 0, smax_ = 0;
diff --git a/chunkfs_amd/csrc/fastcdc.hip b/chunkfs_amd/csrc/fastcdc.hip
--- a/chunkfs_amd/csrc/fastcdc.hip
+++ b/chunkfs_amd/csrc/fastcdc.hip
@@ -837,16 +837,9 @@
 
 
 
-#ifndef CDC_RES_WAVES
-#define CDC_RES_WAVES 8
-#endif
 #ifndef CDC_WALK_SPANS
 #define CDC_WALK_SPANS 8
 #endif
-#ifndef CDC_WIN_RECS
-#define CDC_WIN_RECS 768
-#endif
-constexpr int kResWaves = CDC_RES_WAVES;
 #ifndef CDC_RES_LINK_DIAG
 #define CDC_RES_LINK_DIAG 0
 #endif
@@ -859,8 +852,8 @@
 #ifndef CDC_RES_FASTTRUNC
 #define CDC_RES_FASTTRUNC 1
 #endif
-constexpr int kResThreads = kResWaves * 64;
-
+
+template <bool kLean>
 __device__ __forceinline__ uint32_t trunc_words(const uint8_t *data, uint64_t w0, uint32_t len, uint64_t a0,
                                                 uint64_t ce, uint64_t mask_s, uint64_t mask_l, lds_u64 *tab) {
     const uint64_t al = w0 & ~3ull;
@@ -870,6 +863,30 @@
     for (int i = 0; i < 13; ++i) w[i] = *(g_u32 *)(data + al + 4 * i);
     uint64_t h = 0;
     uint32_t t = kTruncNone;
+    if constexpr (kLean) {
+        const uint32_t ns = ce > a0 ? (uint32_t)min(ce - a0, (uint64_t)64) : 0u;
+#pragma unroll
+        for (int k0 = 0; k0 < 12; k0 += 3) {
+            uint64_t g[12];
+#pragma unroll
+            for (int k = 0; k < 3; ++k) {
+                const uint32_t a = __builtin_amdgcn_alignbyte(w[k0 + k + 1], w[k0 + k], sh);
+#pragma unroll
+                for (int j = 0; j < 4; ++j) g[4 * k + j] = tab[(a >> (8 * j)) & 255];
+            }
+#pragma unroll
+            for (int i = 0; i < 12; ++i) {
+                const uint32_t d = 4 * k0 + i;
+                if (d >= kTruncMax) break;
+                h = shl1_add(h, g[i]);
+                const bool hit = d < len && !(h & (d < ns ? mask_s : mask_l));
+                t = (hit && t == kTruncNone) ? d : t;
+            }
+            asm volatile("" : "+v"(h), "+v"(t));
+            __builtin_amdgcn_sched_barrier(0);
+        }
+        return t;
+    }
 #pragma unroll
     for (int k = 0; k < 12; ++k) {
         const uint32_t a = __builtin_amdgcn_alignbyte(w[k + 1], w[k], sh);
@@ -888,6 +905,7 @@
 #ifndef CDC_RES_CALLS
 #define CDC_RES_CALLS __forceinline__
 #endif
+template <bool kLean>
 __device__ CDC_RES_CALLS uint32_t trunc_at(const uint8_t *data, uint64_t n, uint64_t c, uint64_t mask_s,
                                           uint64_t mask_l, uint32_t mn, uint32_t avg, uint32_t mx, uint32_t trunc,
                                           lds_u64 *tab) {
@@ -899,7 +917,7 @@
     if (tl <= a0) return kTruncNone;
     const uint32_t len = (uint32_t)(tl - a0);
     const uint64_t w0 = c + a0;
-    if ((w0 & ~3ull) + 52 <= n) return trunc_words(data, w0, len, a0, ce, mask_s, mask_l, tab);
+    if ((w0 & ~3ull) + 52 <= n) return trunc_words<kLean>(data, w0, len, a0, ce, mask_s, mask_l, tab);
     uint64_t h = 0;
     for (uint32_t d = 0; d < len; ++d) {
         h = (h << 1) + tab[as_global1(data)[w0 + d]];
@@ -908,9 +926,10 @@
     return kTruncNone;
 }
 
+template <bool kLean>
 __device__ __forceinline__ uint32_t trunc_call(const uint8_t *data, uint64_t n, uint64_t c, const FastParams &fp,
                                                const uint64_t *tab) {
-    return trunc_at(data, n, c, fp.mask_s, fp.mask_l, fp.min, fp.avg, fp.max, fp.trunc, (lds_u64 *)tab);
+    return trunc_at<kLean>(data, n, c, fp.mask_s, fp.mask_l, fp.min, fp.avg, fp.max, fp.trunc, (lds_u64 *)tab);
 }
 
 __device__ CDC_RES_CALLS uint64_t coop_next_bytes(uint32_t mn, uint32_t avg, uint32_t mx, uint64_t mask_s,
@@ -948,12 +967,13 @@
     return v;
 }
 
+template <bool kLean>
 __device__ __forceinline__ uint64_t lane_next_global(const StreamTable &st, const FastParams &fp,
                                                      const Candidates &cand, const uint64_t *tab,
                                                      const uint8_t *data, uint64_t n, uint64_t gbase, uint64_t s) {
     if (n - s <= fp.min) return n;
     const Regime R = regime(fp, s, n);
-    const uint32_t t = trunc_call(data, n, s, fp, tab);
+    const uint32_t t = trunc_call<kLean>(data, n, s, fp, tab);
     if (t != kTruncNone) return s + R.a0 + t;
     if (R.tl >= R.re) return s + R.rem;
     const uint64_t lo = s + R.tl, hi = s + R.re;
@@ -986,13 +1006,16 @@
     const uint8_t *data;
 };
 
+template <class G>
 struct ChainWin;
-__device__ __forceinline__ void emit_start(ChainWin &W, const Chains &ch, const LaneSpan &L, uint32_t l, uint64_t s,
+template <class G>
+__device__ __forceinline__ void emit_start(ChainWin<G> &W, const Chains &ch, const LaneSpan &L, uint32_t l, uint64_t s,
                                            uint32_t &cnt, uint64_t &entry);
+template <class G>
 __device__ __forceinline__ void walk_lanes(const StreamTable &st, const FastParams &fp, const Candidates &cand,
-                                           const uint64_t *tab, ChainWin &W, const Chains &ch, const LaneSpan &L,
+                                           const uint64_t *tab, ChainWin<G> &W, const Chains &ch, const LaneSpan &L,
                                            uint32_t lane, bool go, uint64_t s, uint32_t &cnt, uint64_t &entry,
-                                           uint64_t &exit, uint64_t &steps) {
+                                           uint64_t &exit, uint32_t &steps) {
     cnt = 0;
     entry = ~0ull;
     go = go && s < L.span_end;
@@ -1001,7 +1024,7 @@
         if (go) {
             emit_start(W, ch, L, lane, s, cnt, entry);
             ++steps;
-            const uint64_t nx = lane_next_global(st, fp, cand, tab, L.data, L.n, L.gbase, s);
+            const uint64_t nx = lane_next_global<G::kLean>(st, fp, cand, tab, L.data, L.n, L.gbase, s);
             if (nx == ~0ull) need = true; else s = nx;
             go = !need && s < L.span_end;
         }
@@ -1022,15 +1045,20 @@
 }
 
 constexpr int kWalkSpans = CDC_WALK_SPANS;
-#ifndef CDC_WARM_SPANS
-#define CDC_WARM_SPANS 2
-#endif
-constexpr int kWarmSpans = CDC_WARM_SPANS;
-constexpr int kWinSlots = kWarmSpans + kWalkSpans + 1;
-constexpr int kReach = kWarmSpans + kWalkSpans;
-constexpr uint32_t kWinRecs = CDC_WIN_RECS;
 constexpr uint32_t kVirt = 128;
-constexpr int kBlockSpans = kResWaves * kWalkSpans;
+
+template <int kWaves_, uint32_t kRecs_, int kWarm_, bool kDiag_>
+struct ResGeo {
+    static constexpr int kWaves = kWaves_;
+    static constexpr int kThreads = kWaves_ * 64;
+    static constexpr int kWarm = kWarm_;
+    static constexpr int kWinSlots = kWarm_ + kWalkSpans + 1;
+    static constexpr int kReach = kWarm_ + kWalkSpans;
+    static constexpr uint32_t kRecs = kRecs_;
+    static constexpr int kBlockSpans = kWaves_ * kWalkSpans;
+    static constexpr bool kDiag = kDiag_;
+    static constexpr bool kLean = kWaves_ > 8;
+};
 constexpr uint64_t kNoDep = ~0ull;
 constexpr uint64_t kAgg = 1, kInc = 2;
 constexpr uint32_t kSpinMax = 1u << 26;
@@ -1039,7 +1067,10 @@
 constexpr int kKeyShift = 40;
 constexpr uint64_t kKeyPos = (1ull << kKeyShift) - 1;
 
+template <class G>
 struct ChainWin {
+    static constexpr uint32_t kWinRecs = G::kRecs;
+    static constexpr int kWinSlots = G::kWinSlots;
     uint64_t key[kWinRecs];
     uint32_t rec[kWinRecs];
     uint32_t link[kWinRecs + kVirt];
@@ -1058,21 +1089,23 @@
     uint32_t nrec, nvirt;
 };
 
+template <class G>
 struct BlockState {
-    uint64_t E[kBlockSpans];
-    uint64_t X[kBlockSpans];
-    uint32_t N[kBlockSpans];
-    uint8_t F[kBlockSpans];
+    uint64_t E[G::kBlockSpans];
+    uint64_t X[G::kBlockSpans];
+    uint32_t N[G::kBlockSpans];
+    uint8_t F[G::kBlockSpans];
     uint64_t b, base, pred;
     uint64_t t0;
     uint32_t rewalk;
-    uint64_t stat[kResWaves][3];
-    uint64_t diag[kResWaves][kStatDiagN];
+    uint64_t stat[G::kWaves][3];
+    uint64_t diag[G::kWaves][G::kDiag ? kStatDiagN : 1];
 };
 
 __device__ __forceinline__ uint64_t skey(uint32_t si) { return (uint64_t)si << kKeyShift; }
 
-__device__ __forceinline__ uint32_t win_lower(const ChainWin &W, uint64_t k) {
+template <class G>
+__device__ __forceinline__ uint32_t win_lower(const ChainWin<G> &W, uint64_t k) {
     uint32_t a = 0, b = W.nrec;
     while (a < b) {
         const uint32_t m = (a + b) >> 1;
@@ -1081,16 +1114,18 @@
     return a;
 }
 
-__device__ __forceinline__ uint32_t win_entry_at(const ChainWin &W, uint32_t si, uint64_t p) {
+template <class G>
+__device__ __forceinline__ uint32_t win_entry_at(const ChainWin<G> &W, uint32_t si, uint64_t p) {
     const uint64_t k = skey(si) | p;
     const uint32_t f = win_lower(W, k);
     if (f < W.nrec && W.key[f] == k) return f + 1;
     for (uint32_t v = 0; v < W.nvirt; ++v)
-        if (W.vpos[v] == p && W.ssi[W.vslot[v]] == si) return kWinRecs + v + 1;
+        if (W.vpos[v] == p && W.ssi[W.vslot[v]] == si) return G::kRecs + v + 1;
     return 0;
 }
 
-__device__ __forceinline__ uint64_t win_search(const ChainWin &W, uint32_t si, uint64_t c, const Regime &R,
+template <class G>
+__device__ __forceinline__ uint64_t win_search(const ChainWin<G> &W, uint32_t si, uint64_t c, const Regime &R,
                                                uint32_t i0, uint32_t *lr) {
     *lr = 0;
     const uint64_t s = skey(si);
@@ -1106,15 +1141,15 @@
     return c + R.rem;
 }
 
-template <bool kTrKnown>
-__device__ __forceinline__ uint64_t win_next(const ChainWin &W, const FastParams &fp, const uint64_t *tab,
+template <bool kTrKnown, class G>
+__device__ __forceinline__ uint64_t win_next(const ChainWin<G> &W, const FastParams &fp, const uint64_t *tab,
                                              const uint8_t *data, uint64_t n, uint32_t si, uint64_t c,
                                              uint32_t i0, uint32_t tr, uint32_t *lr) {
     *lr = 0;
     if (n - c <= fp.min) return n;
     const Regime R = regime(fp, c, n);
     if (R.tl > R.a0) {
-        const uint32_t t = kTrKnown ? tr : trunc_call(data, n, c, fp, tab);
+        const uint32_t t = kTrKnown ? tr : trunc_call<G::kLean>(data, n, c, fp, tab);
         if (t != kTruncNone) return c + R.a0 + t;
     }
     if (R.tl >= R.re) return c + R.rem;
@@ -1130,7 +1165,8 @@
     return v < kVirt ? v : kVirt;
 }
 
-__device__ __forceinline__ void emit_start(ChainWin &W, const Chains &ch, const LaneSpan &L, uint32_t l, uint64_t s,
+template <class G>
+__device__ __forceinline__ void emit_start(ChainWin<G> &W, const Chains &ch, const LaneSpan &L, uint32_t l, uint64_t s,
                                            uint32_t &cnt, uint64_t &entry) {
     if (s >= L.off) {
         if (cnt < kLdsStarts) W.st[l][cnt] = (uint32_t)(s - L.off);
@@ -1140,10 +1176,11 @@
     }
 }
 
-__device__ __forceinline__ void walk_window(ChainWin &W, const FastParams &fp, const uint64_t *tab,
+template <class G>
+__device__ __forceinline__ void walk_window(ChainWin<G> &W, const FastParams &fp, const uint64_t *tab,
                                             const LaneSpan &L, const Chains &ch, uint32_t lane, bool go, uint64_t s,
                                             uint32_t wr, uint32_t &cnt, uint64_t &entry, uint64_t &exit,
-                                            uint64_t &steps) {
+                                            uint32_t &steps) {
     cnt = 0;
     entry = ~0ull;
     go = go && s < L.span_end;
@@ -1207,10 +1244,11 @@
     exit = s;
 }
 
+template <class G>
 __device__ __forceinline__ void wave_settle(const StreamTable &st, const FastParams &fp, const Candidates &cand,
-                                            const uint64_t *tab, const Chains &ch, ChainWin &W, bool dense,
+                                            const uint64_t *tab, const Chains &ch, ChainWin<G> &W, bool dense,
                                             const LaneSpan &L, uint32_t lane, uint32_t k0, bool has0,
-                                            uint64_t pred0, BlockState &B, uint64_t &rewalks, uint64_t &steps) {
+                                            uint64_t pred0, BlockState<G> &B, uint32_t &rewalks, uint32_t &steps) {
     const bool mine = lane < kWalkSpans && L.act;
     uint64_t E = mine ? B.E[k0 + lane] : 0, X = mine ? B.X[k0 + lane] : 0;
     for (;;) {
@@ -1239,20 +1277,22 @@
 struct LinkItem {
     bool act, fast;
     int j;
-    uint32_t e, i0, si, len;
+    uint32_t e, i0, len;
     uint32_t known;
-    uint64_t c, n, a0, ce, w0;
-    const uint8_t *data;
+    uint32_t ce;
+    uint64_t c;
 };
-
-__device__ __forceinline__ LinkItem link_item(const ChainWin &W, const FastParams &fp, bool virt, uint32_t x,
+__device__ __forceinline__ uint64_t item_a0(const FastParams &fp) { return (fp.min / 2) * 2; }
+
+template <class G>
+__device__ __forceinline__ LinkItem link_item(const ChainWin<G> &W, const FastParams &fp, bool virt, uint32_t x,
                                               uint32_t e1) {
     LinkItem it{};
     it.known = kTruncUnknown;
     it.act = x < e1;
     if (!it.act) return it;
     if (virt) {
-        it.e = kWinRecs + x;
+        it.e = G::kRecs + x;
         it.j = W.vslot[x];
         it.c = W.vpos[x];
         it.i0 = win_lower(W, skey(W.ssi[it.j]) | it.c);
@@ -1263,36 +1303,36 @@
         it.i0 = x + 1;
         it.known = (W.rec[x] >> kRecTShift) & 63u;
     }
-    it.si = W.ssi[it.j];
-    it.n = W.slen[it.j];
-    it.data = W.sptr[it.j];
-    if (it.n - it.c > fp.min) {
-        const Regime R = regime(fp, it.c, it.n);
+    const uint64_t n = W.slen[it.j];
+    if (n - it.c > fp.min) {
+        const Regime R = regime(fp, it.c, n);
         if (R.tl > R.a0) {
             it.len = (uint32_t)(R.tl - R.a0);
-            it.a0 = R.a0;
-            it.ce = R.ce;
-            it.w0 = it.c + R.a0;
-            it.fast = (it.w0 & ~3ull) + 52 <= it.n && it.known == kTruncUnknown;
+            it.ce = (uint32_t)R.ce;
+            it.fast = ((it.c + R.a0) & ~3ull) + 52 <= n && it.known == kTruncUnknown;
         }
     }
     return it;
 }
 
-__device__ __forceinline__ void item_load(const LinkItem &it, const void *safe, uint32_t (&w)[13]) {
+template <class G>
+__device__ __forceinline__ void item_load(const ChainWin<G> &W, const FastParams &fp, const LinkItem &it,
+                                          const void *safe, uint32_t (&w)[13]) {
     if (!__ballot(it.fast)) return;
-    const uint8_t *src = it.fast ? it.data + (it.w0 & ~3ull) : static_cast<const uint8_t *>(safe);
+    const uint8_t *src = it.fast ? W.sptr[it.j] + ((it.c + item_a0(fp)) & ~3ull) : static_cast<const uint8_t *>(safe);
 #pragma unroll
     for (int i = 0; i < 13; ++i) w[i] = *(g_u32 *)(src + 4 * i);
 }
 
-__device__ __forceinline__ uint32_t item_trunc(const LinkItem &it, const uint32_t (&w)[13], const FastParams &fp,
-                                               const uint64_t *tab, const uint64_t *tabs) {
+template <class G>
+__device__ __forceinline__ uint32_t item_trunc(const ChainWin<G> &W, const LinkItem &it, const uint32_t (&w)[13],
+                                               const FastParams &fp, const uint64_t *tab, const uint64_t *tabs) {
     if (!it.act || it.len == 0) return kTruncNone;
     if (it.known != kTruncUnknown) return it.known;
-    if (!it.fast) return trunc_call(it.data, it.n, it.c, fp, tab);
-    const uint32_t r = (uint32_t)(it.w0 & 3);
-    const uint32_t ns = it.ce > it.a0 ? (uint32_t)min(it.ce - it.a0, (uint64_t)64) : 0u;
+    if (!it.fast) return trunc_call<G::kLean>(W.sptr[it.j], W.slen[it.j], it.c, fp, tab);
+    const uint64_t a0 = item_a0(fp);
+    const uint32_t r = (uint32_t)((it.c + a0) & 3);
+    const uint32_t ns = it.ce > a0 ? (uint32_t)min(it.ce - a0, (uint64_t)64) : 0u;
     if (CDC_RES_FASTTRUNC && fp.cm_align && it.len == kTruncMax && ns >= kTruncMax) {
         const uint32_t ms = (uint32_t)(fp.mask_s_sh >> 32);
         uint64_t h = 0;
@@ -1337,23 +1377,26 @@
     return hits ? (uint32_t)__builtin_ctzll(hits) : kTruncNone;
 }
 
-__device__ __forceinline__ void item_link(ChainWin &W, const FastParams &fp, const uint64_t *tab,
+template <class G>
+__device__ __forceinline__ void item_link(ChainWin<G> &W, const FastParams &fp, const uint64_t *tab,
                                           const LinkItem &it, uint32_t tr, uint32_t sl2, uint32_t &nv) {
     bool mk = false;
     uint64_t nx = 0;
     uint32_t lr = 0;
     int jt = 0;
     if (it.act) {
-        nx = win_next<true>(W, fp, tab, nullptr, it.n, it.si, it.c, it.i0, tr, &lr);
+        const uint64_t n = W.slen[it.j];
+        const uint32_t si = W.ssi[it.j];
+        nx = win_next<true>(W, fp, tab, nullptr, n, si, it.c, it.i0, tr, &lr);
         W.link[it.e] = (uint32_t)(nx - it.c);
         jt = it.j + (int)((nx - W.soff[it.j]) >> sl2);
-        mk = lr == 0 && nx < it.n && jt < kReach && W.ssi[jt] == it.si;
+        mk = lr == 0 && nx < n && jt < G::kReach && W.ssi[jt] == si;
     }
     const uint32_t v = virt_alloc(mk, nv);
     if (mk && v < kVirt) {
         W.vpos[v] = nx;
         W.vslot[v] = (uint8_t)jt;
-        lr = kWinRecs + v + 1;
+        lr = G::kRecs + v + 1;
     }
     if (it.act) W.lrec[it.e] = (uint16_t)lr;
 }
@@ -1494,18 +1537,40 @@
     return __builtin_nontemporal_load((const g_u64 *)p);
 }
 
+template <class G>
+__device__ __forceinline__ LaneSpan lane_span(const ChainWin<G> &W, uint64_t G0, uint32_t k0, uint32_t nsp,
+                                              uint32_t lane, uint32_t sl2) {
+    LaneSpan L{};
+    if (lane < kWalkSpans && k0 + lane < nsp) {
+        const int j = G::kWarm + (int)lane;
+        L.act = true;
+        L.g = G0 + lane;
+        L.si = W.ssi[j];
+        L.off = W.soff[j];
+        L.n = W.slen[j];
+        L.data = W.sptr[j];
+        L.gbase = L.g - (L.off >> sl2);
+        L.span_end = min(L.off + (1ull << sl2), L.n);
+        L.first = L.off == 0;
+    }
+    return L;
+}
+
 #define CDC_DIAG_T(k)                                                  \
     do {                                                               \
-        if ((fp.diag & 128) && !(CDC_RES_LINK_DIAG && (fp.diag & 8192))) { \
-            const uint64_t t_ = __builtin_amdgcn_s_memrealtime();       \
-            dt[k] += t_ - t_prev;                                      \
-            t_prev = t_;                                               \
+        if constexpr (G::kDiag) {                                      \
+            if ((fp.diag & 128) && !(CDC_RES_LINK_DIAG && (fp.diag & 8192))) { \
+                const uint64_t t_ = __builtin_amdgcn_s_memrealtime();   \
+                dt[k] += (uint32_t)(t_ - t_prev);                                 \
+                t_prev = t_;                                           \
+            }                                                          \
         }                                                              \
     } while (0)
 
 #ifndef CDC_RES_ATTR
-#define CDC_RES_ATTR __launch_bounds__(kResThreads, 2)
-#endif
+#define CDC_RES_ATTR __launch_bounds__(G::kThreads, G::kWaves > 8 ? G::kWaves / 4 : 2)
+#endif
+template <class G>
 __global__ CDC_RES_ATTR void resolve_kernel(const StreamTable st, const FastParams fp,
                                                               const uint64_t *__restrict__ gear,
                                                               const Candidates cand, const Chains ch,
@@ -1513,8 +1578,11 @@
                                                               cdc_chunk_pod *out, uint64_t out_cap) {
     __shared__ uint64_t tab[256];
     __shared__ uint64_t tabs[256];
-    __shared__ ChainWin win[kResWaves];
-    __shared__ BlockState B;
+    constexpr int kResWaves = G::kWaves, kBlockSpans = G::kBlockSpans, kWarmSpans = G::kWarm;
+    constexpr int kWinSlots = G::kWinSlots, kReach = G::kReach;
+    constexpr uint32_t kWinRecs = G::kRecs;
+    __shared__ ChainWin<G> win[kResWaves];
+    __shared__ BlockState<G> B;
     if (threadIdx.x == 0) {
         if (fp.diag & 64) B.t0 = __builtin_amdgcn_s_memrealtime();
         B.b = atomicAdd((unsigned long long *)&cp.stats[kStatOrder], 1ull);
@@ -1532,11 +1600,10 @@
     const uint32_t k0 = wave * kWalkSpans;
     const uint64_t G0 = g0 + k0;
     const uint32_t cap = cand.cap;
-    ChainWin &W = win[wave];
-    uint64_t t_prev = (fp.diag & 128) ? __builtin_amdgcn_s_memrealtime() : 0;
-    uint64_t dt[kStatDiagN] = {};
-    uint64_t steps = 0, rewalks = 0, cstat = 0;
-    LaneSpan L{};
+    ChainWin<G> &W = win[wave];
+    uint64_t t_prev = (G::kDiag && (fp.diag & 128)) ? __builtin_amdgcn_s_memrealtime() : 0;
+    uint32_t dt[kStatDiagN] = {};
+    uint32_t steps = 0, rewalks = 0;
     bool dense = false;
 
     if (k0 < nsp) {
@@ -1575,24 +1642,14 @@
         }
         wave_sync_lds();
         dense = W.nvirt != 0;
-        if (lane < kWalkSpans && k0 + lane < nsp) {
-            const int j = kWarmSpans + (int)lane;
-            L.act = true;
-            L.g = G0 + lane;
-            L.si = W.ssi[j];
-            L.off = W.soff[j];
-            L.n = W.slen[j];
-            L.data = W.sptr[j];
-            L.gbase = L.g - (L.off >> sl2);
-            L.span_end = min(L.off + span, L.n);
-            L.first = L.off == 0;
-            const uint32_t c = W.scnt[j];
-            cstat = c > cap ? 1ull : (uint64_t)c << 24;
-        }
         CDC_DIAG_T(0);
         uint32_t cnt = 0;
         uint64_t entry = 0, exit = 0;
+        bool act, first;
         if (dense) {
+            const LaneSpan L = lane_span(W, G0, k0, nsp, lane, sl2);
+            act = L.act;
+            first = L.first;
             uint64_t s0 = 0;
             if (L.act && !L.first) s0 = L.off > kWarmSpans * span ? L.off - kWarmSpans * span : 0;
             if (L.act && !L.first && (fp.diag & 1)) s0 = L.off;
@@ -1629,24 +1686,33 @@
             for (;;) {
                 LinkItem A = link_item(W, fp, virt, e0 + lane, e1);
                 uint32_t wa[13];
-                item_load(A, gear, wa);
+                item_load(W, fp, A, gear, wa);
+                if constexpr (G::kLean) {
+                    for (uint32_t base = e0; base < e1; base += 64) {
+                        const uint32_t tr = (fp.diag & 4) ? kTruncNone : item_trunc(W, A, wa, fp, tab, tabs);
+                        const LinkItem B2 = link_item(W, fp, virt, base + 64 + lane, e1);
+                        item_load(W, fp, B2, gear, wa);
+                        item_link(W, fp, tab, A, tr, sl2, nv);
+                        A = B2;
+                    }
+                } else
                 for (uint32_t base = e0; base < e1; base += 64) {
-                    constexpr bool kLinkDiag = CDC_RES_LINK_DIAG;
+                    constexpr bool kLinkDiag = CDC_RES_LINK_DIAG && G::kDiag;
                     uint64_t f0 = (kLinkDiag && (fp.diag & 8192)) ? __builtin_amdgcn_s_memrealtime() : 0;
                     const LinkItem B2 = link_item(W, fp, virt, base + 64 + lane, e1);
                     uint32_t wb[13];
-                    item_load(B2, gear, wb);
+                    item_load(W, fp, B2, gear, wb);
                     uint64_t f1 = (kLinkDiag && (fp.diag & 8192)) ? __builtin_amdgcn_s_memrealtime() : 0;
-                    const uint32_t tr = (fp.diag & 4) ? kTruncNone : item_trunc(A, wa, fp, tab, tabs);
+                    const uint32_t tr = (fp.diag & 4) ? kTruncNone : item_trunc(W, A, wa, fp, tab, tabs);
                     if (kLinkDiag && (fp.diag & 8192)) __builtin_amdgcn_s_waitcnt(0);
                     uint64_t f2 = (kLinkDiag && (fp.diag & 8192)) ? __builtin_amdgcn_s_memrealtime() : 0;
                     item_link(W, fp, tab, A, tr, sl2, nv);
                     if (kLinkDiag && (fp.diag & 8192)) {
                         const uint64_t f3 = __builtin_amdgcn_s_memrealtime();
                         const int o = virt ? 3 : 0;
-                        dt[o] += f1 - f0;
-                        dt[o + 1] += f2 - f1;
-                        dt[o + 2] += f3 - f2;
+                        dt[o] += (uint32_t)(f1 - f0);
+                        dt[o + 1] += (uint32_t)(f2 - f1);
+                        dt[o + 2] += (uint32_t)(f3 - f2);
                     }
                     A = B2;
 #pragma unroll
@@ -1663,6 +1729,9 @@
             if (lane == 0) W.nvirt = min(nv, kVirt);
             wave_sync_lds();
             CDC_DIAG_T(3);
+            const LaneSpan L = lane_span(W, G0, k0, nsp, lane, sl2);
+            act = L.act;
+            first = L.first;
             uint64_t s = 0;
             uint32_t wr = 0;
             if (L.act && !L.first && L.off >= kWarmSpans * span) {
@@ -1680,11 +1749,11 @@
             }
             walk_window(W, fp, tab, L, ch, lane, L.act, s, wr, cnt, entry, exit, steps);
         }
-        if (L.act) {
+        if (act) {
             B.E[k0 + lane] = entry;
             B.X[k0 + lane] = exit;
             B.N[k0 + lane] = cnt;
-            B.F[k0 + lane] = L.first ? 1 : 0;
+            B.F[k0 + lane] = first ? 1 : 0;
         }
         CDC_DIAG_T(5);
     }
@@ -1722,6 +1791,7 @@
             need = B.rewalk != 0;
         }
         if (need) {
+            const LaneSpan L = lane_span(W, G0, k0, nsp, lane, sl2);
             for (uint32_t w2 = 0; w2 < (uint32_t)kResWaves; ++w2) {
                 if (wave == w2 && k0 < nsp)
                     wave_settle(st, fp, cand, tab, ch, W, dense, L, lane, k0, w2 > 0 || round > 0,
@@ -1735,10 +1805,17 @@
         uint64_t C = 0;
         for (uint32_t k = lane; k < nsp; k += 64) C += B.N[k];
         C = wave_sum(C);
-        publish(rs, b, kInc, B.base + C, 0, B.X[nsp - 1], lane);
+        publish(rs, B.b, kInc, B.base + C, 0, B.X[nsp - 1], lane);
     }
 
     if (k0 < nsp) {
+        const uint64_t Gw = B.b * kBlockSpans + k0;
+        const LaneSpan L = lane_span(W, Gw, k0, nsp, lane, sl2);
+        uint64_t cstat = 0;
+        if (L.act) {
+            const uint32_t c = W.scnt[kWarmSpans + lane];
+            cstat = c > cap ? 1ull : (uint64_t)c << 24;
+        }
         uint32_t wpre0 = 0;
         for (uint32_t k = 0; k < k0; ++k) wpre0 += B.N[k];
         const uint32_t myN = L.act ? B.N[k0 + lane] : 0;
@@ -1760,7 +1837,7 @@
                 int k = 0;
                 while (k + 1 < kWalkSpans && W.wpre[k + 1] <= i) ++k;
                 const uint32_t r = i - W.wpre[k];
-                const uint64_t *list = ch.starts + (G0 + k) * ch.smax;
+                const uint64_t *list = ch.starts + (Gw + k) * ch.smax;
                 const uint64_t off_k = W.soff[kWarmSpans + k];
                 const uint64_t s0 = r < kLdsStarts ? off_k + W.st[k][r] : ld_nt(list + r);
                 const uint64_t nx = r + 1 >= B.N[k0 + k] ? B.X[k0 + k]
@@ -1772,7 +1849,7 @@
                 if (L.g + 1 == st.total_spans) cp.h_first[st.n] = obase + x;
             }
         }
-        const uint64_t cs = wave_sum(cstat), rw = wave_sum(rewalks), sp = wave_sum(steps);
+        const uint64_t cs = wave_sum(cstat), rw = wave_sum((uint64_t)rewalks), sp = wave_sum((uint64_t)steps);
         if (lane == 0) {
             B.stat[wave][0] = cs;
             B.stat[wave][1] = rw;
@@ -1782,8 +1859,9 @@
     } else if (lane == 0) {
         B.stat[wave][0] = B.stat[wave][1] = B.stat[wave][2] = 0;
     }
-    if ((fp.diag & 128) && lane == 0)
-        for (int k = 0; k < kStatDiagN; ++k) B.diag[wave][k] = dt[k];
+    if constexpr (G::kDiag)
+        if ((fp.diag & 128) && lane == 0)
+            for (int k = 0; k < kStatDiagN; ++k) B.diag[wave][k] = dt[k];
 #if CDC_RES_HOSTREL >= 3
     __threadfence_system();
 #elif CDC_RES_HOSTREL >= 1
@@ -1806,7 +1884,7 @@
             atomicMax(d + 3, (unsigned long long)~t1);
             atomicMax(d + 4, (unsigned long long)(t1 - t0));
             atomicAdd(d + 5, (unsigned long long)(t1 - t0));
-        } else if (fp.diag & 128)
+        } else if (G::kDiag && (fp.diag & 128))
             for (int k = 0; k < kStatDiagN; ++k) {
                 uint64_t d = 0;
                 for (int w = 0; w < kResWaves; ++w) d += B.diag[w][k];
@@ -1896,16 +1974,59 @@
     return e != hipSuccess ? e : hipGetLastError();
 }
 
-uint64_t resolve_blocks(uint64_t spans) { return (spans + kBlockSpans - 1) / kBlockSpans; }
+template <class G>
+static hipError_t resolve_launch(const StreamTable &st, const FastParams &fp, const uint64_t *d_gear,
+                                 const Candidates &cand, const Chains &ch, const Compact &cp, const Resolve &rs,
+                                 void *d_out, uint64_t out_cap, hipStream_t s) {
+    const uint64_t blocks = (st.total_spans + G::kBlockSpans - 1) / G::kBlockSpans;
+    resolve_kernel<G><<<(unsigned)blocks, G::kThreads, 0, s>>>(
+        st, fp, d_gear, cand, ch, cp, rs, reinterpret_cast<cdc_chunk_pod *>(d_out), out_cap);
+    return hipGetLastError();
+}
+
+#ifdef CDC_OVL
+using OvlGeo = ResGeo<CDC_RES_WAVES, CDC_WIN_RECS, 2, true>;
+
+uint64_t resolve_blocks(uint64_t spans) { return (spans + OvlGeo::kBlockSpans - 1) / OvlGeo::kBlockSpans; }
 
 hipError_t launch_resolve(const StreamTable &st, const FastParams &fp, const uint64_t *d_gear,
                           const Candidates &cand, const Chains &ch, const Compact &cp, const Resolve &rs,
                           void *d_out, uint64_t out_cap, hipStream_t s) {
     if (!st.total_spans) return hipSuccess;
-    resolve_kernel<<<(unsigned)resolve_blocks(st.total_spans), kResThreads, 0, s>>>(
-        st, fp, d_gear, cand, ch, cp, rs, reinterpret_cast<cdc_chunk_pod *>(d_out), out_cap);
-    return hipGetLastError();
-}
+    return resolve_launch<OvlGeo>(st, fp, d_gear, cand, ch, cp, rs, d_out, out_cap, s);
+}
+#else
+constexpr uint32_t kRecs8 = 768, kRecs12 = 512;
+
+uint32_t resolve_win_recs(int waves) { return waves == 12 ? kRecs12 : kRecs8; }
+
+uint64_t resolve_blocks(uint64_t spans, int waves) {
+    const uint64_t bs = (uint64_t)(waves == 12 ? 12 : 8) * kWalkSpans;
+    return (spans + bs - 1) / bs;
+}
+
+int resolve_warm_spans(uint32_t span_log2) { return span_log2 >= 17 ? 1 : 2; }
+
+hipError_t launch_resolve(const StreamTable &st, const FastParams &fp, const uint64_t *d_gear,
+                          const Candidates &cand, const Chains &ch, const Compact &cp, const Resolve &rs,
+                          void *d_out, uint64_t out_cap, int waves, int warm, hipStream_t s) {
+    if (!st.total_spans) return hipSuccess;
+    const bool diag = (fp.diag & 128) != 0;
+#define CDC_RES_CASE(WV, RC, WM, DG)                                                                     \
+    if (waves == WV && warm == WM && diag == DG)                                                         \
+        return resolve_launch<ResGeo<WV, RC, WM, DG>>(st, fp, d_gear, cand, ch, cp, rs, d_out, out_cap, s)
+    CDC_RES_CASE(8, kRecs8, 2, false);
+    CDC_RES_CASE(8, kRecs8, 1, false);
+    CDC_RES_CASE(12, kRecs12, 2, false);
+    CDC_RES_CASE(12, kRecs12, 1, false);
+    CDC_RES_CASE(8, kRecs8, 2, true);
+    CDC_RES_CASE(8, kRecs8, 1, true);
+    CDC_RES_CASE(12, kRecs12, 2, true);
+    CDC_RES_CASE(12, kRecs12, 1, true);
+#undef CDC_RES_CASE
+    return hipErrorInvalidValue;
+}
+#endif
 
 #ifdef CDC_OVL
 }
diff --git a/chunkfs_amd/csrc/fastcdc.hpp b/chunkfs_amd/csrc/fastcdc.hpp
--- a/chunkfs_amd/csrc/fastcdc.hpp
+++ b/chunkfs_amd/csrc/fastcdc.hpp
@@ -37,14 +37,16 @@
 constexpr int kStatDiagN = 8;
 constexpr int kStatWords = kStatDiag0 + kStatDiagN;
 
-uint64_t resolve_blocks(uint64_t spans);
+uint32_t resolve_win_recs(int waves);
+uint64_t resolve_blocks(uint64_t spans, int waves);
+int resolve_warm_spans(uint32_t span_log2);
 
 hipError_t launch_scan(const StreamTable &st, const FastParams &fp, const uint64_t *d_gear,
                        const Candidates &cand, const Compact &cp, const uint64_t *d_tails, uint32_t n_tails,
                        int num_cus, hipStream_t s);
 hipError_t launch_resolve(const StreamTable &st, const FastParams &fp, const uint64_t *d_gear,
                           const Candidates &cand, const Chains &ch, const Compact &cp, const Resolve &rs,
-                          void *d_out, uint64_t out_cap, hipStream_t s);
+                          void *d_out, uint64_t out_cap, int waves, int warm, hipStream_t s);
 
 namespace ovl {
 uint64_t resolve_blocks(uint64_t spans);
```

Measured after the change: 4316, median of 6. About the same (+0.3%).
